# tanishqkumar/ssd

Hardware: NVIDIA H100
Metric: decode tokens/sec (sync speculative decoding, accept-len reported) (higher is better)
Workload: dtype bf16

## Files before the change

### include/ssdk.h

```cpp
#ifndef SSDK_H_
#define SSDK_H_

#include <stdint.h>

#ifdef __cplusplus
extern "C" {
#endif

#define SSDK_ABI_VERSION 1

typedef struct ssdk_engine* ssdk_handle;

enum { SSDK_TARGET = 0, SSDK_DRAFT = 1 };

enum {
  SSDK_W_EMBED      = 0,
  SSDK_W_LM_HEAD    = 1,
  SSDK_W_FINAL_NORM = 2,
  SSDK_W_INPUT_NORM = 3,
  SSDK_W_QKV        = 4,
  SSDK_W_Q_NORM     = 5,
  SSDK_W_K_NORM     = 6,
  SSDK_W_O          = 7,
  SSDK_W_POST_NORM  = 8,
  SSDK_W_GATE_UP    = 9,
  SSDK_W_DOWN       = 10,
  SSDK_W_ROPE_TABLE = 11,
  SSDK_W_KIND_COUNT = 12
};

typedef struct ssdk_model_cfg {
  int32_t hidden;
  int32_t layers;
  int32_t heads;
  int32_t kv_heads;
  int32_t head_dim;
  int32_t ffn;
  int32_t vocab;
  int32_t qk_norm;
  float   rms_eps;
  int32_t max_pos;
  int32_t tp_size;
  int32_t tp_rank;
} ssdk_model_cfg;

typedef struct ssdk_runtime_cfg {
  int32_t spec_k;
  int32_t max_batch;
  int32_t block_size;
  int32_t max_blocks_per_seq;
  int32_t use_graph;
  int32_t use_pdl;
  int32_t jit_speculate;
  int32_t reserved;
} ssdk_runtime_cfg;

int  ssdk_abi_version(void);
const char* ssdk_last_error(void);

int ssdk_create(const ssdk_model_cfg* target, const ssdk_model_cfg* draft,
                const ssdk_runtime_cfg* rt, ssdk_handle* out);
int ssdk_destroy(ssdk_handle h);

int ssdk_bind_weight(ssdk_handle h, int which, int kind, int layer,
                     const void* dev_ptr, int64_t rows, int64_t cols);

int ssdk_bind_kv_cache(ssdk_handle h, int which, void* kv_base, int64_t num_blocks);

int64_t ssdk_workspace_bytes(ssdk_handle h);
int ssdk_bind_workspace(ssdk_handle h, void* dev_ptr, int64_t bytes);

int ssdk_set_nccl_comm(ssdk_handle h, void* nccl_comm);
int64_t ssdk_symm_bytes(ssdk_handle h);
int ssdk_bind_symm(ssdk_handle h, void* const* peer_ptrs, int n_peers);

int ssdk_finalize(ssdk_handle h, void* stream);


int ssdk_spec_step(ssdk_handle h, int batch,
                   const int32_t* ctx_len, const int64_t* recovery,
                   const int32_t* block_tables_target, const int32_t* block_tables_draft,
                   const float* temp_t, const float* temp_q,
                   uint64_t seed, uint64_t step_id,
                   int64_t* out_tokens, int32_t* out_n_accept, int64_t* out_recovery,
                   void* stream);

int ssdk_spec_step_stage(ssdk_handle h, int batch,
                         const int32_t* ctx_len, const int64_t* recovery,
                         const int32_t* block_tables_target, const int32_t* block_tables_draft,
                         const float* temp_t, const float* temp_q,
                         uint64_t seed, uint64_t step_id, void* stream);
int ssdk_spec_step_resident(ssdk_handle h, int batch, void* stream);
int ssdk_spec_step_fetch(ssdk_handle h, int batch, int64_t* out_tokens,
                         int32_t* out_n_accept, int64_t* out_recovery, void* stream);
int ssdk_spec_step_log(ssdk_handle h, int seq, int64_t* out_tokens, int cap, void* stream);

int ssdk_forward_tokens(ssdk_handle h, int which, int batch, int q_len,
                        const int64_t* ids, const int32_t* ctx_len,
                        const int32_t* block_tables, int want_sample,
                        const float* temps, uint64_t seed, uint64_t step_id,
                        int64_t* out_tokens, void* stream);

int ssdk_forward_varlen(ssdk_handle h, int which, int n_seqs, const int32_t* q_lens,
                        const int64_t* ids, const int32_t* ctx_len,
                        const int32_t* block_tables, int want_sample,
                        const float* temps, uint64_t seed, uint64_t step_id,
                        int64_t* out_tokens, void* stream);

const void* ssdk_logits_p(ssdk_handle h);
const void* ssdk_logits_q(ssdk_handle h);
const void* ssdk_logits_last(ssdk_handle h);
int ssdk_debug_trace(void* dev_buf, int cap);
int64_t ssdk_launch_count(ssdk_handle h);


int ssdk_gemm_small_m(const void* x, const void* w, void* y, float* partials,
                      int M, int N, int K, int ldy, int split_k, void* stream);

int ssdk_gemm_gate_up_silu(const void* x, const void* w_gate_up, void* h,
                           int M, int ffn, int K, void* stream);

int ssdk_rmsnorm(const void* x, const void* residual_in, const void* w, float eps,
                 void* y, void* residual_out, int M, int d, void* stream);

int ssdk_rope_store_kv(const void* qkv, const int64_t* positions, const int32_t* slot_mapping,
                       const float* rope_table, const void* q_norm_w, const void* k_norm_w,
                       float norm_eps, void* q_out, void* k_cache, void* v_cache,
                       int M, int heads, int kv_heads, int head_dim, void* stream);

int ssdk_silu_mul(const void* gate_up, void* out, int M, int ffn, void* stream);

int64_t ssdk_paged_attn_scratch_bytes(int batch, int q_len, int heads, int head_dim, int max_ctx);
int ssdk_paged_attn(const void* q, const void* k_cache, const void* v_cache,
                    const int32_t* block_tables, const int32_t* context_lens,
                    void* out, void* scratch,
                    int batch, int q_len, int heads, int kv_heads, int head_dim,
                    int block_size, int max_blocks_per_seq, float scale, void* stream);
int ssdk_paged_attn_plan(int heads, int kv_heads, int batch, int q_len, int max_ctx, int* out4);
int ssdk_paged_attn_varlen(const void* q, const void* k_cache, const void* v_cache,
                           const int32_t* block_tables, const int32_t* context_lens,
                           const int32_t* q_lens, void* out, void* scratch,
                           int batch, int heads, int kv_heads, int head_dim,
                           int block_size, int max_blocks_per_seq, float scale, void* stream);
int ssdk_paged_attn_varlen_plan(int heads, int kv_heads, int batch, const int32_t* q_lens, int max_ctx, int* out5);

int ssdk_sample(const void* logits, int64_t ld, const float* temps, int B, int V,
                uint64_t seed, uint64_t step_id, int64_t* out_tokens, void* stream);

int64_t ssdk_verify_scratch_bytes(int B, int K);
int ssdk_verify(const void* logits_p, const void* logits_q, const int64_t* speculations,
                const float* temps_t, const float* temps_q, const int32_t* cache_hits,
                int jit_speculate, int B, int K, int V, uint64_t seed, uint64_t step_id,
                int32_t* n_accept, int64_t* recovery, void* scratch, void* stream);

#ifdef __cplusplus
}
#endif
#endif
```

### ssd_b200/csrc/draft_stream.cuh

```cuda
#pragma once
#include "common.cuh"
#include "sampling.cuh"

namespace ssdk {

constexpr int kDsConsumers = 256;
constexpr int kDsWarps = kDsConsumers / 32;
constexpr int kDsThreads = kDsConsumers + 32;
constexpr int kDsMaxLayers = 32;
constexpr int kDsSplits = 16;
constexpr int kDsShortSplits = 8;
constexpr int kDsLongCtx = 256;
constexpr int kDsSlotBytes = 32768;
constexpr int kDsMaxSlots = 6;
constexpr int kDsMaxSteps = 8;
constexpr int kDsBtSmem = 32;

struct DsLayer {
  const __nv_bfloat16 *qkv, *o, *gate_up, *down, *in_norm, *post_norm, *q_norm, *k_norm;
};

struct DsParams {
  int d, L, H, KV, ffn, vocab, qk_norm;
  float eps, scale_log2;
  const __nv_bfloat16 *embed, *final_norm, *lm_head;
  const float* rope;
  __nv_bfloat16 *k_cache, *v_cache;
  long long cache_layer_stride;
  int block_size, max_blocks;
  int64_t* tok_buf;
  int n_fwd;
  int skip_last_head;
  const int32_t* ctx0;
  const int32_t* block_table;
  __nv_bfloat16 *vec_qkv, *vec_attn, *vec_o, *vec_act, *vec_down, *resid0, *resid1;
  float* attn_part;
  __nv_bfloat16* logits;
  long long logits_ld;
  const float* temp;
  const uint64_t* dyn;
  uint64_t seed, call_base;
  ArgMax* samp_partial;
  unsigned* bar_state;
  unsigned* attn_ticket;
  int n_slots;
  DsLayer layers[kDsMaxLayers];
};

SSDK_DEVINL void ds_sync() {
#ifdef SSDK_HOST_EMU
  ::emu::named_barrier(1, kDsConsumers);
#else
  asm volatile("bar.sync 1, 256;" ::: "memory");
#endif
}

struct DsGridBar {
  unsigned long long* counter;
  unsigned long long target;
  __device__ void init() {
    if (threadIdx.x == 0) {
      const unsigned long long c = ld_relaxed_gpu_u64(counter);
      target = c - c % (unsigned long long)gridDim.x;
    }
  }
  __device__ void sync() {
    ds_sync();
    if (threadIdx.x == 0) {
      target += (unsigned long long)gridDim.x;
      red_add_release_gpu_u64(counter, 1ull);
      const long long t0 = clock64();
      while (ld_relaxed_gpu_u64(counter) < target) {
        if (clock64() - t0 > 4000000000LL) __trap();
      }
      fence_acq_rel_gpu();
    }
    ds_sync();
  }
};

SSDK_DEVINL uint4 ds_ldcg16(const void* p) { return __ldcg(reinterpret_cast<const uint4*>(p)); }
SSDK_DEVINL float2 ds_bf2(uint32_t w) { return __bfloat1622float2(*reinterpret_cast<const __nv_bfloat162*>(&w)); }

SSDK_DEVINL void ds_mark(int f, int point) {
  if (f == 1 && threadIdx.x == 0) trace_mark(64 + point);
}

enum { DS_QKV = 0, DS_O = 1, DS_GU = 2, DS_DOWN = 3, DS_HEAD = 4 };
enum { DS_PLAIN = 0, DS_PAIR = 1, DS_SPLIT = 2 };
struct DsGeom {
  int K;
  int rows;
  int kind;
  int rpj;
  int segs;
  int nj;
};
__host__ SSDK_DEVINL bool ds_geometry(int K, int rows, bool pair, DsGeom* g) {
  g->K = K; g->rows = rows; g->segs = 1;
  if (K < 256 || K > 8192 || (K % 256) != 0) return false;
  if (pair) {
    if (K > 2048) return false;
    g->kind = DS_PAIR; g->rpj = 8;
  } else if (K <= 2048) {
    g->kind = DS_PLAIN; g->rpj = 8;
  } else {
    g->kind = DS_SPLIT; g->rpj = K <= 4096 ? 4 : 2; g->segs = kDsWarps / g->rpj;
    if ((K % (256 * g->segs)) != 0) return false;
  }
  g->nj = (rows + g->rpj - 1) / g->rpj;
  return true;
}
SSDK_DEVINL bool ds_has_head(const DsParams& p, int f) { return !(p.skip_last_head && f == p.n_fwd - 1); }
SSDK_DEVINL const __nv_bfloat16* ds_weight(const DsParams& p, int l, int m) {
  const DsLayer& lw = p.layers[l < p.L ? l : 0];
  return m == DS_QKV ? lw.qkv : (m == DS_O ? lw.o : (m == DS_GU ? lw.gate_up : (m == DS_DOWN ? lw.down : p.lm_head)));
}

struct DsCursor {
  int f, l, m, s;
  bool valid;
};
SSDK_DEVINL void ds_cursor_settle(const DsParams& p, const DsGeom* geom, DsCursor& c) {
  while (c.valid && c.s >= geom[c.m].nj) {
    c.s = (int)blockIdx.x;
    if (c.m == DS_HEAD) {
      c.f++; c.l = 0; c.m = DS_QKV;
    } else if (c.m == DS_DOWN) {
      c.l++; c.m = DS_QKV;
      if (c.l == p.L) {
        if (ds_has_head(p, c.f)) c.m = DS_HEAD;
        else { c.f++; c.l = 0; }
      }
    } else {
      c.m++;
    }
    if (c.f >= p.n_fwd) c.valid = false;
  }
}

SSDK_DEVINL void ds_cursor_next(const DsParams& p, const DsGeom* geom, DsCursor& c) {
  c.s += (int)gridDim.x;
  if (c.s >= geom[c.m].nj) ds_cursor_settle(p, geom, c);
}
SSDK_DEVINL void ds_producer(const DsParams& p, const DsGeom* geom, uint8_t* ring, uint64_t* full, uint64_t* empty) {
  DsCursor c;
  c.f = 0; c.l = 0; c.m = DS_QKV; c.s = (int)blockIdx.x; c.valid = p.n_fwd > 0;
  ds_cursor_settle(p, geom, c);
  unsigned n = 0;
  const unsigned S = (unsigned)p.n_slots;
  while (c.valid) {
    const DsGeom g = geom[c.m];
    const __nv_bfloat16* w = ds_weight(p, c.l, c.m);
    const int rows = min(g.rpj, g.rows - c.s * g.rpj);
    const unsigned bytes = (unsigned)rows * (unsigned)g.K * 2u;
    const int parts = g.kind == DS_PAIR ? 2 : 1;
    for (int q = 0; q < parts; ++q) {
      const unsigned slot = n % S, round = n / S;
      mbar_wait(&empty[slot], (round & 1u) ^ 1u);
      mbar_arrive_expect_tx(&full[slot], bytes);
      const __nv_bfloat16* src = w + ((size_t)(q ? g.rows : 0) + (size_t)c.s * g.rpj) * g.K;
      bulk_load_g2s(ring + (size_t)slot * kDsSlotBytes, src, bytes, &full[slot]);
      ++n;
    }
    ds_cursor_next(p, geom, c);
  }
}

struct DsRing {
  uint8_t* base;
  uint64_t *full, *empty;
  unsigned n_slots;
  unsigned taken;
};
SSDK_DEVINL const uint8_t* ds_acquire(DsRing& r, unsigned k) {
  const unsigned n = r.taken + k, slot = n % r.n_slots;
  mbar_wait(&r.full[slot], (n / r.n_slots) & 1u);
  return r.base + (size_t)slot * kDsSlotBytes;
}
SSDK_DEVINL void ds_release(DsRing& r, unsigned k, int lane) {
  __syncwarp();
  if (lane == 0) mbar_arrive(&r.empty[(r.taken + k) % r.n_slots]);
}

SSDK_DEVINL void ds_load_x(const float* xseg, int steps, int lane, float (&xr)[kDsMaxSteps][8]) {
#pragma unroll
  for (int j = 0; j < kDsMaxSteps; ++j) {
    if (j < steps) {
      const float4 a = *reinterpret_cast<const float4*>(xseg + j * 256 + lane * 8);
      const float4 b = *reinterpret_cast<const float4*>(xseg + j * 256 + lane * 8 + 4);
      xr[j][0] = a.x; xr[j][1] = a.y; xr[j][2] = a.z; xr[j][3] = a.w;
      xr[j][4] = b.x; xr[j][5] = b.y; xr[j][6] = b.z; xr[j][7] = b.w;
    } else {
#pragma unroll
      for (int e = 0; e < 8; ++e) xr[j][e] = 0.f;
    }
  }
}
SSDK_DEVINL float ds_dot_seg(const uint8_t* wseg, int steps, int lane, const float (&xr)[kDsMaxSteps][8]) {
  const uint4* wp = reinterpret_cast<const uint4*>(wseg) + lane;
  float a0 = 0.f, a1 = 0.f, a2 = 0.f, a3 = 0.f;
#pragma unroll
  for (int j = 0; j < kDsMaxSteps; ++j) {
    if (j < steps) {
      const uint4 w = wp[j * 32];
      float2 f = ds_bf2(w.x);
      a0 = fmaf(f.x, xr[j][0], a0); a1 = fmaf(f.y, xr[j][1], a1);
      f = ds_bf2(w.y);
      a2 = fmaf(f.x, xr[j][2], a2); a3 = fmaf(f.y, xr[j][3], a3);
      f = ds_bf2(w.z);
      a0 = fmaf(f.x, xr[j][4], a0); a1 = fmaf(f.y, xr[j][5], a1);
      f = ds_bf2(w.w);
      a2 = fmaf(f.x, xr[j][6], a2); a3 = fmaf(f.y, xr[j][7], a3);
    }
  }
  return warp_sum((a0 + a1) + (a2 + a3));
}

struct DsSample {
  bool greedy;
  float invT;
  uint64_t seed, call_id;
  ArgMax best;
};
SSDK_DEVINL float ds_score(const DsSample& s, float logit, int idx) {
  if (s.greedy) return logit;
  const uint4 rnd = philox_draw((uint32_t)(idx >> 2), 0u, s.call_id, TAG_SAMPLE, s.seed);
  const float e = u32_to_exp1(u4_word(rnd, idx & 3)) + 1e-10f;
  return logit * s.invT - __logf(e);
}

template <bool HEAD>
SSDK_DEVINL void ds_consume_plain(DsRing& ring, const DsGeom& g, const float* xs, __nv_bfloat16* y, DsSample* smp) {
  if ((int)blockIdx.x >= g.nj) return;
  const int warp = threadIdx.x >> 5, lane = threadIdx.x & 31;
  const int steps = g.K >> 8;
  float xr[kDsMaxSteps][8];
  ds_load_x(xs, steps, lane, xr);
  for (int s = (int)blockIdx.x; s < g.nj; s += (int)gridDim.x) {
    const uint8_t* st = ds_acquire(ring, 0);
    const float acc = ds_dot_seg(st + (size_t)warp * g.K * 2, steps, lane, xr);
    ds_release(ring, 0, lane);
    ring.taken += 1u;
    const int row = s * 8 + warp;
    if (lane == 0 && row < g.rows) {
      const __nv_bfloat16 o = f2bf(acc);
      if (!HEAD) {
        y[row] = o;
      } else {
        if (y) y[row] = o;
        smp->best = argmax_better(smp->best, ArgMax{ds_score(*smp, bf2f(o), row), row});
      }
    }
  }
}
SSDK_DEVINL void ds_consume_pair(DsRing& ring, const DsGeom& g, const float* xs, __nv_bfloat16* act) {
  if ((int)blockIdx.x >= g.nj) return;
  const int warp = threadIdx.x >> 5, lane = threadIdx.x & 31;
  const int steps = g.K >> 8;
  float xr[kDsMaxSteps][8];
  ds_load_x(xs, steps, lane, xr);
  for (int s = (int)blockIdx.x; s < g.nj; s += (int)gridDim.x) {
    const uint8_t* sg = ds_acquire(ring, 0);
    float gate = ds_dot_seg(sg + (size_t)warp * g.K * 2, steps, lane, xr);
    ds_release(ring, 0, lane);
    const uint8_t* su = ds_acquire(ring, 1);
    float up = ds_dot_seg(su + (size_t)warp * g.K * 2, steps, lane, xr);
    ds_release(ring, 1, lane);
    ring.taken += 2u;
    const int i = s * 8 + warp;
    if (lane == 0 && i < g.rows) {
      gate = bf16_round(gate);
      up = bf16_round(up);
      act[i] = f2bf((gate / (1.0f + __expf(-gate))) * up);
    }
  }
}
SSDK_DEVINL void ds_consume_split(DsRing& ring, const DsGeom& g, const float* xs, float* res, __nv_bfloat16* y) {
  if ((int)blockIdx.x >= g.nj) return;
  const int warp = threadIdx.x >> 5, lane = threadIdx.x & 31;
  const int row_in_job = warp / g.segs, seg = warp - row_in_job * g.segs;
  const int seg_len = g.K / g.segs, steps = seg_len >> 8;
  float xr[kDsMaxSteps][8];
  ds_load_x(xs + seg * seg_len, steps, lane, xr);
  const size_t w_off = ((size_t)row_in_job * g.K + (size_t)seg * seg_len) * 2;
  unsigned it = 0;
  for (int s = (int)blockIdx.x; s < g.nj; s += (int)gridDim.x, ++it) {
    const uint8_t* st = ds_acquire(ring, 0);
    const float acc = ds_dot_seg(st + w_off, steps, lane, xr);
    ds_release(ring, 0, lane);
    ring.taken += 1u;
    float* rb = res + (it & 1u) * kDsWarps;
    if (lane == 0) rb[warp] = acc;
    ds_sync();
    if ((int)threadIdx.x < g.rpj) {
      const int row = s * g.rpj + (int)threadIdx.x;
      if (row < g.rows) {
        float v = 0.f;
        for (int q = 0; q < g.segs; ++q) v += rb[(int)threadIdx.x * g.segs + q];
        y[row] = f2bf(v);
      }
    }
  }
}
SSDK_DEVINL void ds_consume(DsRing& ring, const DsGeom& g, const float* xs, float* res, __nv_bfloat16* y) {
  if (g.kind == DS_PLAIN) ds_consume_plain<false>(ring, g, xs, y, nullptr);
  else ds_consume_split(ring, g, xs, res, y);
}

SSDK_DEVINL float ds_block_sum(float v, float* red) {
  const int lane = threadIdx.x & 31, wid = threadIdx.x >> 5;
  v = warp_sum(v);
  ds_sync();
  if (lane == 0) red[wid] = v;
  ds_sync();
  float t = (lane < kDsWarps) ? red[lane] : 0.f;
  return warp_sum(t);
}

struct DsPre {
  uint4 w, b;
};
SSDK_DEVINL DsPre ds_preload(const __nv_bfloat16* b, const __nv_bfloat16* w, int d) {
  DsPre r;
  const int i = threadIdx.x * 8;
  r.w = r.b = make_uint4(0u, 0u, 0u, 0u);
  if (i < d) {
    r.w = *reinterpret_cast<const uint4*>(w + i);
    if (b) r.b = ds_ldcg16(b + i);
  }
  return r;
}
SSDK_DEVINL void ds_norm_prologue(const __nv_bfloat16* a, const __nv_bfloat16* b, __nv_bfloat16* resid_out,
                                  const __nv_bfloat16* w, float eps, int d, float* xs, float* red, const DsPre* pre) {
  float ss = 0.f;
  const int i0 = threadIdx.x * 8;
  for (int i = i0; i < d; i += kDsConsumers * 8) {
    float x[8];
    unpack_bf16x8(ds_ldcg16(a + i), x);
    if (b) {
      float y[8];
      unpack_bf16x8((pre && i == i0) ? pre->b : ds_ldcg16(b + i), y);
#pragma unroll
      for (int j = 0; j < 8; ++j) x[j] += y[j];
    }
    if (resid_out && blockIdx.x == 0) *reinterpret_cast<uint4*>(resid_out + i) = pack_bf16x8(x);
#pragma unroll
    for (int j = 0; j < 8; ++j) {
      xs[i + j] = x[j];
      ss += x[j] * x[j];
    }
  }
  ss = ds_block_sum(ss, red);
  const float rstd = rsqrtf(ss / (float)d + eps);
  for (int i = i0; i < d; i += kDsConsumers * 8) {
    float wv[8];
    unpack_bf16x8((pre && i == i0) ? pre->w : *reinterpret_cast<const uint4*>(w + i), wv);
#pragma unroll
    for (int j = 0; j < 8; ++j) xs[i + j] = bf16_round(xs[i + j] * rstd * wv[j]);
  }
  ds_sync();
}
SSDK_DEVINL void ds_load_vec(const __nv_bfloat16* v, int n, float* xs) {
  for (int i = threadIdx.x * 8; i < n; i += kDsConsumers * 8) {
    float x[8];
    unpack_bf16x8(ds_ldcg16(v + i), x);
#pragma unroll
    for (int j = 0; j < 8; ++j) xs[i + j] = x[j];
  }
  ds_sync();
}

SSDK_DEVINL int ds_num_splits(int ctx) {
  return ctx > kDsLongCtx ? kDsSplits : min(kDsShortSplits, max(1, (ctx + 7) >> 3));
}
SSDK_DEVINL int ds_page_of(const DsParams& p, const int* bt_s, int t) {
  const int i = t / p.block_size;
  return p.max_blocks <= kDsBtSmem ? bt_s[i] : p.block_table[i];
}
template <int HD, int TB>
SSDK_DEVINL void ds_load_kv(const DsParams& p, const int* bt_s, const __nv_bfloat16* kbase, const __nv_bfloat16* vbase, int h,
                            int tb, int t1, int pos, int lane, float (&kv)[TB][HD / 32], float (&vv)[TB][HD / 32]) {
  constexpr int EPL = HD / 32;
  static_assert(EPL == 2 || EPL == 4, "head_dim 64 or 128");
#pragma unroll
  for (int u = 0; u < TB; ++u) {
    const int t = tb + u * kDsWarps;
#pragma unroll
    for (int e = 0; e < EPL; ++e) kv[u][e] = vv[u][e] = 0.f;
    if (t < t1 && t != pos) {
      const int blk = ds_page_of(p, bt_s, t);
      const size_t off = (((size_t)blk * p.block_size + t % p.block_size) * p.KV + h) * HD + lane * EPL;
      if constexpr (EPL == 2) {
        const float2 a = ds_bf2(__ldcg(reinterpret_cast<const uint32_t*>(kbase + off)));
        const float2 b = ds_bf2(__ldcg(reinterpret_cast<const uint32_t*>(vbase + off)));
        kv[u][0] = a.x; kv[u][1] = a.y; vv[u][0] = b.x; vv[u][1] = b.y;
      } else {
        const uint2 a = __ldcg(reinterpret_cast<const uint2*>(kbase + off));
        const uint2 b = __ldcg(reinterpret_cast<const uint2*>(vbase + off));
        float2 f = ds_bf2(a.x); kv[u][0] = f.x; kv[u][1] = f.y;
        f = ds_bf2(a.y); kv[u][EPL - 2] = f.x; kv[u][EPL - 1] = f.y;
        f = ds_bf2(b.x); vv[u][0] = f.x; vv[u][1] = f.y;
        f = ds_bf2(b.y); vv[u][EPL - 2] = f.x; vv[u][EPL - 1] = f.y;
      }
    }
  }
}
template <int HD, int GMAX, int TB>
SSDK_DEVINL void ds_attention_unit(const DsParams& p, int layer, int h, int s, int ns, int ctx, float* sm, int* flag,
                                   const int* bt_s) {
  constexpr int HALF = HD / 2;
  constexpr int EPL = HD / 32;
  const int warp = threadIdx.x >> 5, lane = threadIdx.x & 31;
  const int G = p.H / p.KV;
  const int pos = ctx - 1;
  float* sq = sm;
  float* sk = sq + GMAX * HD;
  float* sv = sk + HD;
  float* sred = sv + HD;

  const int per = (ctx + ns - 1) / ns;
  const int t0 = s * per, t1 = min(ctx, t0 + per);
  const __nv_bfloat16* kbase = p.k_cache + (size_t)layer * p.cache_layer_stride;
  const __nv_bfloat16* vbase = p.v_cache + (size_t)layer * p.cache_layer_stride;
  float kv[TB][EPL], vv[TB][EPL];
  ds_load_kv<HD, TB>(p, bt_s, kbase, vbase, h, t0 + warp, t1, pos, lane, kv, vv);

  const float* cs = p.rope + (size_t)pos * HD;
  for (int row = warp; row < G + 2; row += kDsWarps) {
    const int kind = row < G ? 0 : (row == G ? 1 : 2);
    const int col0 = (kind == 0 ? (h * G + row) : (kind == 1 ? p.H + h : p.H + p.KV + h)) * HD;
    float x1[(HALF + 31) / 32], x2[(HALF + 31) / 32];
    float ss = 0.f;
#pragma unroll
    for (int t = 0; t < (HALF + 31) / 32; ++t) {
      const int i = lane + 32 * t;
      x1[t] = x2[t] = 0.f;
      if (i < HALF) {
        const unsigned short a = __ldcg(reinterpret_cast<const unsigned short*>(p.vec_qkv + col0 + i));
        const unsigned short b = __ldcg(reinterpret_cast<const unsigned short*>(p.vec_qkv + col0 + HALF + i));
        x1[t] = __bfloat162float(__ushort_as_bfloat16(a));
        x2[t] = __bfloat162float(__ushort_as_bfloat16(b));
        ss += x1[t] * x1[t] + x2[t] * x2[t];
      }
    }
    float* dst = kind == 0 ? sq + row * HD : (kind == 1 ? sk : sv);
    if (kind == 2) {
#pragma unroll
      for (int t = 0; t < (HALF + 31) / 32; ++t) {
        const int i = lane + 32 * t;
        if (i < HALF) {
          dst[i] = x1[t];
          dst[HALF + i] = x2[t];
        }
      }
      continue;
    }
    const __nv_bfloat16* nw = p.qk_norm ? (kind == 0 ? p.layers[layer].q_norm : p.layers[layer].k_norm) : nullptr;
    if (nw) {
      ss = warp_sum(ss);
      const float rstd = rsqrtf(ss / (float)HD + p.eps);
#pragma unroll
      for (int t = 0; t < (HALF + 31) / 32; ++t) {
        const int i = lane + 32 * t;
        if (i < HALF) {
          x1[t] = bf16_round(x1[t] * rstd * bf2f(nw[i]));
          x2[t] = bf16_round(x2[t] * rstd * bf2f(nw[HALF + i]));
        }
      }
    }
#pragma unroll
    for (int t = 0; t < (HALF + 31) / 32; ++t) {
      const int i = lane + 32 * t;
      if (i < HALF) {
        const float c = cs[i], sn = cs[HALF + i];
        dst[i] = bf16_round(x1[t] * c - x2[t] * sn);
        dst[HALF + i] = bf16_round(x2[t] * c + x1[t] * sn);
      }
    }
  }
  ds_sync();

  const int blk_new = ds_page_of(p, bt_s, pos);
  if (s == 0 && blk_new >= 0) {
    const size_t slot = (size_t)blk_new * p.block_size + pos % p.block_size;
    __nv_bfloat16* kc = p.k_cache + (size_t)layer * p.cache_layer_stride + (slot * p.KV + h) * HD;
    __nv_bfloat16* vc = p.v_cache + (size_t)layer * p.cache_layer_stride + (slot * p.KV + h) * HD;
    for (int i = threadIdx.x; i < HD; i += kDsConsumers) {
      kc[i] = f2bf(sk[i]);
      vc[i] = f2bf(sv[i]);
    }
  }

  float qreg[GMAX][EPL];
#pragma unroll
  for (int g = 0; g < GMAX; ++g)
#pragma unroll
    for (int e = 0; e < EPL; ++e) qreg[g][e] = (g < G) ? sq[g * HD + lane * EPL + e] : 0.f;
  float m[GMAX], l[GMAX], acc[GMAX][EPL];
#pragma unroll
  for (int g = 0; g < GMAX; ++g) {
    m[g] = -INFINITY;
    l[g] = 0.f;
#pragma unroll
    for (int e = 0; e < EPL; ++e) acc[g][e] = 0.f;
  }
  for (int tb = t0 + warp; tb < t1; tb += TB * kDsWarps) {
    if (tb != t0 + warp) ds_load_kv<HD, TB>(p, bt_s, kbase, vbase, h, tb, t1, pos, lane, kv, vv);
#pragma unroll
    for (int u = 0; u < TB; ++u) {
      const int t = tb + u * kDsWarps;
      if (t < t1) {
        if (t == pos) {
#pragma unroll
          for (int e = 0; e < EPL; ++e) {
            kv[u][e] = sk[lane * EPL + e];
            vv[u][e] = sv[lane * EPL + e];
          }
        }
#pragma unroll
        for (int g = 0; g < GMAX; ++g) {
          if (g < G) {
            float sc = 0.f;
#pragma unroll
            for (int e = 0; e < EPL; ++e) sc = fmaf(qreg[g][e], kv[u][e], sc);
            sc = warp_sum(sc) * p.scale_log2;
            const float mn = fmaxf(m[g], sc);
            const float corr = exp2f(m[g] - mn);
            const float pr = exp2f(sc - mn);
            l[g] = l[g] * corr + pr;
#pragma unroll
            for (int e = 0; e < EPL; ++e) acc[g][e] = acc[g][e] * corr + pr * vv[u][e];
            m[g] = mn;
          }
        }
      }
    }
  }
  constexpr int LDR = HD + 2;
#pragma unroll
  for (int g = 0; g < GMAX; ++g) {
    if (g < G) {
      float* w = sred + ((size_t)warp * G + g) * LDR;
#pragma unroll
      for (int e = 0; e < EPL; ++e) w[lane * EPL + e] = acc[g][e];
      if (lane == 0) {
        w[HD] = m[g];
        w[HD + 1] = l[g];
      }
    }
  }
  ds_sync();
  for (int idx = threadIdx.x; idx < G * HD; idx += kDsConsumers) {
    const int g = idx / HD, dim = idx - g * HD;
    float mx = -INFINITY;
    for (int w = 0; w < kDsWarps; ++w) mx = fmaxf(mx, sred[((size_t)w * G + g) * LDR + HD]);
    float o = 0.f, ll = 0.f;
    if (mx != -INFINITY) {
      for (int w = 0; w < kDsWarps; ++w) {
        const float* r = sred + ((size_t)w * G + g) * LDR;
        const float wt = exp2f(r[HD] - mx);
        o += r[dim] * wt;
        ll += r[HD + 1] * wt;
      }
    }
    if (ns == 1) {
      p.vec_attn[(size_t)(h * G + g) * HD + dim] = f2bf(ll > 0.f ? o / ll : 0.f);
    } else {
      float* out = p.attn_part + ((size_t)(h * G + g) * kDsSplits + s) * LDR;
      out[dim] = o;
      if (dim == 0) {
        out[HD] = mx;
        out[HD + 1] = ll;
      }
    }
  }
  if (ns == 1) {
    ds_sync();
    return;
  }
  ds_sync();
  if (threadIdx.x == 0) *flag = (atom_add_acq_rel_gpu(p.attn_ticket + h, 1u) == (unsigned)ns - 1u) ? 1 : 0;
  ds_sync();
  if (*flag) {
    if (threadIdx.x == 0) st_relaxed_gpu_u32(p.attn_ticket + h, 0u);
    for (int idx = threadIdx.x; idx < G * HD; idx += kDsConsumers) {
      const int g = idx / HD, dim = idx - g * HD;
      const float* base = p.attn_part + (size_t)(h * G + g) * kDsSplits * LDR;
      float ms[kDsSplits], ls[kDsSplits], os[kDsSplits];
      float mx = -INFINITY;
#pragma unroll
      for (int q = 0; q < kDsSplits; ++q) {
        const bool on = q < ns;
        ms[q] = on ? __ldcg(base + q * LDR + HD) : -INFINITY;
        ls[q] = on ? __ldcg(base + q * LDR + HD + 1) : 0.f;
        os[q] = on ? __ldcg(base + q * LDR + dim) : 0.f;
        mx = fmaxf(mx, ms[q]);
      }
      float o = 0.f, l = 0.f;
#pragma unroll
      for (int q = 0; q < kDsSplits; ++q) {
        const float wt = (ms[q] == -INFINITY) ? 0.f : exp2f(ms[q] - mx);
        o += os[q] * wt;
        l += ls[q] * wt;
      }
      p.vec_attn[(size_t)(h * G + g) * HD + dim] = f2bf(l > 0.f ? o / l : 0.f);
    }
  }
  ds_sync();
}


template <int HD, int GMAX>
__global__ void __launch_bounds__(kDsThreads, 1) draft_stream_kernel(const __grid_constant__ DsParams p) {
  SSDK_DYN_SMEM(uint8_t, ds_smem);
  SSDK_STATIC_SMEM(uint64_t, full_bar, kDsMaxSlots);
  SSDK_STATIC_SMEM(uint64_t, empty_bar, kDsMaxSlots);
  SSDK_STATIC_SMEM(DsGeom, geom, 5);
  SSDK_STATIC_SMEM(float, red, 32);
  SSDK_STATIC_SMEM(float, res, 2 * kDsWarps);
  SSDK_STATIC_SMEM(ArgMax, ared, 32);
  SSDK_SHARED_VAR(int, tok_s);
  SSDK_SHARED_VAR(int, flag_s);
  SSDK_STATIC_SMEM(int, bt_s, kDsBtSmem);
  float* xs = reinterpret_cast<float*>(ds_smem + (size_t)p.n_slots * kDsSlotBytes);
  float* scratch = xs + max(max(p.d, p.ffn), p.H * HD);
  if (threadIdx.x < kDsBtSmem && (int)threadIdx.x < p.max_blocks) bt_s[threadIdx.x] = p.block_table[threadIdx.x];
  if (threadIdx.x == 0) {
    trace_mark(TR_MISC);
    ds_geometry(p.d, (p.H + 2 * p.KV) * HD, false, &geom[DS_QKV]);
    ds_geometry(p.H * HD, p.d, false, &geom[DS_O]);
    ds_geometry(p.d, p.ffn, true, &geom[DS_GU]);
    ds_geometry(p.ffn, p.d, false, &geom[DS_DOWN]);
    ds_geometry(p.d, p.vocab, false, &geom[DS_HEAD]);
    for (int s = 0; s < p.n_slots; ++s) {
      mbar_init(&full_bar[s], 1);
      mbar_init(&empty_bar[s], kDsWarps);
    }
    fence_mbar_init();
  }
  __syncthreads();

  if (threadIdx.x >= kDsConsumers) {
    if (threadIdx.x == kDsConsumers) ds_producer(p, geom, ds_smem, full_bar, empty_bar);
    return;
  }

  DsRing ring;
  ring.base = ds_smem;
  ring.full = full_bar;
  ring.empty = empty_bar;
  ring.n_slots = (unsigned)p.n_slots;
  ring.taken = 0u;
  DsGridBar bar;
  bar.counter = reinterpret_cast<unsigned long long*>(p.bar_state);
  bar.target = 0;
  bar.init();

  const int ctx_base = p.ctx0[0];
  const float T = p.temp ? p.temp[0] : 0.f;
  const uint64_t seed = p.dyn ? p.dyn[0] : p.seed;
  const uint64_t call0 = p.dyn ? p.dyn[1] * 16ull : p.call_base;
  __nv_bfloat16* resid[2] = {p.resid0, p.resid1};
  long long tok = p.tok_buf[0];

  for (int f = 0; f < p.n_fwd; ++f) {
    if (threadIdx.x == 0 && f > 0) trace_mark(TR_MISC);
    const int ctx = ctx_base + f + 1;
    const __nv_bfloat16* emb = p.embed + (size_t)tok * p.d;
    int cur = 0;
    DsPre pre;
    for (int l = 0; l < p.L; ++l) {
      const DsLayer& lw = p.layers[l];
      if (l == 0) {
        ds_norm_prologue(emb, nullptr, resid[cur ^ 1], lw.in_norm, p.eps, p.d, xs, red, nullptr);
      } else {
        ds_norm_prologue(p.vec_down, resid[cur], resid[cur ^ 1], lw.in_norm, p.eps, p.d, xs, red, &pre);
      }
      cur ^= 1;
      ds_mark(f, 0);
      ds_consume(ring, geom[DS_QKV], xs, res, p.vec_qkv);
      ds_mark(f, 1);
      bar.sync();
      ds_mark(f, 2);
#ifdef SSDK_TRACE_FINE
      bar.sync();
      ds_mark(f, 12);
#endif
      const int ns = ds_num_splits(ctx);
      for (int u = blockIdx.x; u < p.KV * ns; u += gridDim.x) {
        if (ns == kDsSplits) ds_attention_unit<HD, GMAX, 8>(p, l, u / ns, u % ns, ns, ctx, scratch, &flag_s, bt_s);
        else ds_attention_unit<HD, GMAX, 4>(p, l, u / ns, u % ns, ns, ctx, scratch, &flag_s, bt_s);
      }
      ds_mark(f, 3);
      bar.sync();
      ds_mark(f, 4);
      ds_load_vec(p.vec_attn, p.H * HD, xs);
      ds_consume(ring, geom[DS_O], xs, res, p.vec_o);
      ds_mark(f, 5);
      pre = ds_preload(resid[cur], lw.post_norm, p.d);
      bar.sync();
      ds_mark(f, 6);
      ds_norm_prologue(p.vec_o, resid[cur], resid[cur ^ 1], lw.post_norm, p.eps, p.d, xs, red, &pre);
      cur ^= 1;
      ds_mark(f, 7);
      ds_consume_pair(ring, geom[DS_GU], xs, p.vec_act);
      ds_mark(f, 8);
      bar.sync();
      ds_mark(f, 9);
      ds_load_vec(p.vec_act, p.ffn, xs);
      ds_consume(ring, geom[DS_DOWN], xs, res, p.vec_down);
      ds_mark(f, 10);
      pre = ds_preload(resid[cur], l + 1 < p.L ? p.layers[l + 1].in_norm : p.final_norm, p.d);
      bar.sync();
      ds_mark(f, 11);
    }
    if (!ds_has_head(p, f)) break;
    ds_norm_prologue(p.vec_down, resid[cur], nullptr, p.final_norm, p.eps, p.d, xs, red, &pre);
    DsSample smp;
    smp.greedy = (T == 0.f);
    smp.invT = smp.greedy ? 1.f : 1.f / T;
    smp.seed = seed;
    smp.call_id = call0 + (uint64_t)f;
    smp.best = ArgMax{-INFINITY, 0x7fffffff};
    ds_consume_plain<true>(ring, geom[DS_HEAD], xs, p.logits ? p.logits + (size_t)f * p.logits_ld : nullptr, &smp);
    if ((threadIdx.x & 31) == 0) ared[threadIdx.x >> 5] = smp.best;
    ds_sync();
    if (threadIdx.x == 0) {
      ArgMax b = ared[0];
      for (int w = 1; w < kDsWarps; ++w) b = argmax_better(b, ared[w]);
      p.samp_partial[blockIdx.x] = b;
    }
    bar.sync();
    {
      ArgMax a{-INFINITY, 0x7fffffff};
      for (int i = threadIdx.x; i < (int)gridDim.x; i += kDsConsumers) {
        ArgMax q;
        q.v = __ldcg(&p.samp_partial[i].v);
        q.i = __ldcg(&p.samp_partial[i].i);
        a = argmax_better(a, q);
      }
      a = warp_argmax(a);
      ds_sync();
      if ((threadIdx.x & 31) == 0) ared[threadIdx.x >> 5] = a;
      ds_sync();
      if (threadIdx.x == 0) {
        ArgMax b = ared[0];
        for (int w = 1; w < kDsWarps; ++w) b = argmax_better(b, ared[w]);
        tok_s = b.i;
      }
      ds_sync();
      tok = tok_s;
      if (blockIdx.x == 0 && threadIdx.x == 0) p.tok_buf[f + 1] = tok;
    }
  }
}

}
```

### ssd_b200/csrc/elementwise.cuh

```cuda
#pragma once
#include "common.cuh"

namespace ssdk {

struct GemmOut {
  const __nv_bfloat16* dense;
  const float* partial;
  int S;
  int M;
  int N;
};

SSDK_DEVINL float gemm_out_at(const GemmOut& g, int m, int n) {
  if (g.S == 0) return bf2f(g.dense[(size_t)m * g.N + n]);
  const float* base = g.partial + (size_t)m * g.N + n;
  const size_t stride = (size_t)g.M * g.N;
  float acc = 0.f;
  for (int s0 = 0; s0 < g.S; s0 += 8) {
    float v[8];
#pragma unroll
    for (int u = 0; u < 8; ++u) v[u] = (s0 + u < g.S) ? __ldcg(base + (size_t)(s0 + u) * stride) : 0.f;
#pragma unroll
    for (int u = 0; u < 8; ++u) acc += v[u];
  }
  return bf16_round(acc);
}
template <int NB = 8>
SSDK_DEVINL void gemm_out_at8(const GemmOut& g, int m, int n, float* f) {
  if (g.S == 0) {
    uint4 v = *reinterpret_cast<const uint4*>(g.dense + (size_t)m * g.N + n);
    unpack_bf16x8(v, f);
    return;
  }
#pragma unroll
  for (int i = 0; i < 8; ++i) f[i] = 0.f;
  const float* base = g.partial + (size_t)m * g.N + n;
  const size_t stride = (size_t)g.M * g.N;
  for (int s0 = 0; s0 < g.S; s0 += NB) {
    float4 a[NB], b[NB];
#pragma unroll
    for (int u = 0; u < NB; ++u) {
      if (s0 + u < g.S) {
        const float4* p = reinterpret_cast<const float4*>(base + (size_t)(s0 + u) * stride);
        a[u] = __ldcg(p);
        b[u] = __ldcg(p + 1);
      } else {
        a[u] = make_float4(0.f, 0.f, 0.f, 0.f);
        b[u] = a[u];
      }
    }
#pragma unroll
    for (int u = 0; u < NB; ++u) {
      f[0] += a[u].x; f[1] += a[u].y; f[2] += a[u].z; f[3] += a[u].w;
      f[4] += b[u].x; f[5] += b[u].y; f[6] += b[u].z; f[7] += b[u].w;
    }
  }
#pragma unroll
  for (int i = 0; i < 8; ++i) f[i] = bf16_round(f[i]);
}

SSDK_DEVINL void gemm_out_at2x2(const GemmOut& g, int m, int a, int b, float* fa, float* fb) {
  if (g.S == 0) {
    const float2 va = __bfloat1622float2(*reinterpret_cast<const __nv_bfloat162*>(g.dense + (size_t)m * g.N + a));
    const float2 vb = __bfloat1622float2(*reinterpret_cast<const __nv_bfloat162*>(g.dense + (size_t)m * g.N + b));
    fa[0] = va.x; fa[1] = va.y; fb[0] = vb.x; fb[1] = vb.y;
    return;
  }
  fa[0] = fa[1] = fb[0] = fb[1] = 0.f;
  const float* base = g.partial + (size_t)m * g.N;
  const size_t stride = (size_t)g.M * g.N;
  for (int s0 = 0; s0 < g.S; s0 += 8) {
    float2 va[8], vb[8];
#pragma unroll
    for (int u = 0; u < 8; ++u) {
      const float* row = base + (size_t)min(s0 + u, g.S - 1) * stride;
      va[u] = __ldcg(reinterpret_cast<const float2*>(row + a));
      vb[u] = __ldcg(reinterpret_cast<const float2*>(row + b));
    }
#pragma unroll
    for (int u = 0; u < 8; ++u) {
      const bool in = s0 + u < g.S;
      fa[0] += in ? va[u].x : 0.f; fa[1] += in ? va[u].y : 0.f;
      fb[0] += in ? vb[u].x : 0.f; fb[1] += in ? vb[u].y : 0.f;
    }
  }
  fa[0] = bf16_round(fa[0]); fa[1] = bf16_round(fa[1]); fb[0] = bf16_round(fb[0]); fb[1] = bf16_round(fb[1]);
}

__global__ void prep_kernel(const int32_t* __restrict__ ctx0, const int32_t* __restrict__ block_tables,
                            int max_blocks, int block_size, int batch, int q_len, int pos_offset,
                            int64_t* __restrict__ positions, int32_t* __restrict__ slot_mapping,
                            int32_t* __restrict__ context_lens, unsigned* __restrict__ fwd_seq) {
  pdl_launch_dependents();
  pdl_wait();
  if (threadIdx.x == 0) trace_mark(TR_PREP);
  const int i = blockIdx.x * blockDim.x + threadIdx.x;
  if (i < batch * q_len) {
    const int b = i / q_len, j = i - b * q_len;
    const int pos = ctx0[b] + pos_offset + j;
    positions[i] = pos;
    const int blk = block_tables[(size_t)b * max_blocks + pos / block_size];
    slot_mapping[i] = (blk < 0) ? -1 : blk * block_size + pos % block_size;
  }
  if (i < batch) context_lens[i] = ctx0[i] + pos_offset + q_len;
  if (fwd_seq && i == 0) *fwd_seq += 1u;
}

__global__ void prep_varlen_kernel(const int32_t* __restrict__ ctx0, const int32_t* __restrict__ cu_q,
                                   const int32_t* __restrict__ block_tables, int max_blocks, int block_size, int batch,
                                   int64_t* __restrict__ positions, int32_t* __restrict__ slot_mapping,
                                   int32_t* __restrict__ context_lens, unsigned* __restrict__ fwd_seq) {
  pdl_launch_dependents();
  pdl_wait();
  if (threadIdx.x == 0) trace_mark(TR_PREP);
  const int i = blockIdx.x * blockDim.x + threadIdx.x;
  if (i < cu_q[batch]) {
    int b = 0;
    while (cu_q[b + 1] <= i) ++b;
    const int pos = ctx0[b] + i - cu_q[b];
    positions[i] = pos;
    const int blk = block_tables[(size_t)b * max_blocks + pos / block_size];
    slot_mapping[i] = (blk < 0) ? -1 : blk * block_size + pos % block_size;
  }
  if (i < batch) context_lens[i] = ctx0[i] + cu_q[i + 1] - cu_q[i];
  if (fwd_seq && i == 0) *fwd_seq += 1u;
}

struct SymmIn {
  const uint8_t* base;
  const unsigned* fwd_seq;
  int no_dep_wait;
  int call_idx;
  int n_calls;
  int n_ranks;
  unsigned slot_bytes;
};
constexpr int kSymmMaxRanks = 8;
SSDK_DEVINL size_t symm_slot_off(unsigned parity, int rank, unsigned slot_bytes) {
  return ((size_t)parity * kSymmMaxRanks + rank) * slot_bytes;
}

struct NormParams {
  GemmOut x;
  SymmIn symm;
  const int64_t* ids;
  int ids_stride;
  const __nv_bfloat16* embed;
  int vocab_start, vocab_rows;
  const __nv_bfloat16* residual_in;
  const __nv_bfloat16* w;
  float eps;
  __nv_bfloat16* y;
  __nv_bfloat16* residual_out;
  int d;
};

template <int NB>
SSDK_DEVINL void norm_slice(const NormParams& p, int m, int i, const uint8_t* symm_slots, unsigned symm_e,
                            const __nv_bfloat16* erow, bool zero_row, float* x) {
  const int d = p.d;
  uint4 res = make_uint4(0, 0, 0, 0);
  if (p.residual_in && !symm_slots) res = *reinterpret_cast<const uint4*>(p.residual_in + (size_t)m * d + i);
  if (symm_slots) {
#pragma unroll
    for (int j = 0; j < 8; ++j) x[j] = 0.f;
    const size_t word0 = ((size_t)m * d + i) / 2;
    uint4 lo[kSymmMaxRanks], hi[kSymmMaxRanks];
    const long long t0 = clock64();
    bool ready = false;
    while (!ready) {
#pragma unroll
      for (int r = 0; r < kSymmMaxRanks; ++r) {
        if (r < p.symm.n_ranks) {
          const uint4* src = reinterpret_cast<const uint4*>(symm_slots + (size_t)r * p.symm.slot_bytes) + word0 / 2;
          lo[r] = ld_volatile_v4(src);
          hi[r] = ld_volatile_v4(src + 1);
        }
      }
      ready = true;
#pragma unroll
      for (int r = 0; r < kSymmMaxRanks; ++r)
        if (r < p.symm.n_ranks)
          ready = ready && lo[r].y == symm_e && lo[r].w == symm_e && hi[r].y == symm_e && hi[r].w == symm_e;
      if (!ready && clock64() - t0 > 8000000000LL) __trap();
    }
#pragma unroll
    for (int r = 0; r < kSymmMaxRanks; ++r) {
      if (r < p.symm.n_ranks) {
        const uint32_t w4[4] = {lo[r].x, lo[r].z, hi[r].x, hi[r].z};
#pragma unroll
        for (int q = 0; q < 4; ++q) {
          const float2 c = __bfloat1622float2(*reinterpret_cast<const __nv_bfloat162*>(&w4[q]));
          x[2 * q] += c.x;
          x[2 * q + 1] += c.y;
        }
      }
    }
#pragma unroll
    for (int j = 0; j < 8; ++j) x[j] = bf16_round(x[j]);
    asm volatile("" ::: "memory");
    if (p.residual_in) res = *reinterpret_cast<const uint4*>(p.residual_in + (size_t)m * d + i);
  } else if (p.ids) {
    if (zero_row) {
#pragma unroll
      for (int j = 0; j < 8; ++j) x[j] = 0.f;
    } else {
      unpack_bf16x8(*reinterpret_cast<const uint4*>(erow + i), x);
    }
  } else {
    gemm_out_at8<NB>(p.x, m, i, x);
  }
  if (p.residual_in) {
    float r[8];
    unpack_bf16x8(res, r);
#pragma unroll
    for (int j = 0; j < 8; ++j) x[j] += r[j];
  }
  if (p.residual_out) *reinterpret_cast<uint4*>(p.residual_out + (size_t)m * d + i) = pack_bf16x8(x);
}

template <int SLICES>
__global__ void __launch_bounds__(512) add_rmsnorm_kernel(NormParams p) {
  SSDK_DYN_SMEM(float, rbuf);
  SSDK_STATIC_SMEM(float, red, 32);
  pdl_launch_dependents();
  if (!(p.symm.base && p.symm.no_dep_wait)) pdl_wait();
  if (threadIdx.x == 0) trace_mark(TR_NORM);
  const int m = blockIdx.x;
  const int d = p.d;
  const uint8_t* symm_slots = nullptr;
  unsigned symm_e = 0;
  if (p.symm.base) {
    const unsigned seq = __ldcg(p.symm.fwd_seq);
    symm_e = symm_epoch_of(seq, p.symm.call_idx);
    symm_slots = p.symm.base + symm_slot_off(symm_parity_of(seq, p.symm.call_idx, p.symm.n_calls), 0, p.symm.slot_bytes);
  }
  const __nv_bfloat16* erow = nullptr;
  bool zero_row = false;
  if (p.ids) {
    const long long id = p.ids[(size_t)m * p.ids_stride] - p.vocab_start;
    if (id < 0 || id >= p.vocab_rows) zero_row = true;
    else erow = p.embed + (size_t)id * d;
  }
  float ss = 0.f;
  if constexpr (SLICES > 0) {
    constexpr int NB = (SLICES == 1) ? 8 : 4;
    float xreg[SLICES][8];
    uint4 wpk[SLICES];
#pragma unroll
    for (int c = 0; c < SLICES; ++c) {
      const int i = (c * blockDim.x + threadIdx.x) * 8;
      if (i < d && p.y) wpk[c] = *reinterpret_cast<const uint4*>(p.w + i);
    }
#pragma unroll
    for (int c = 0; c < SLICES; ++c) {
      const int i = (c * blockDim.x + threadIdx.x) * 8;
      if (i < d) {
        norm_slice<NB>(p, m, i, symm_slots, symm_e, erow, zero_row, xreg[c]);
#pragma unroll
        for (int j = 0; j < 8; ++j) ss += xreg[c][j] * xreg[c][j];
      }
    }
    if (threadIdx.x == 0) trace_fine(TRF_NORM + 0);
    ss = block_sum(ss, red);
    if (threadIdx.x == 0) trace_fine(TRF_NORM + 1);
    const float rstd = rsqrtf(ss / (float)d + p.eps);
    if (p.y) {
#pragma unroll
      for (int c = 0; c < SLICES; ++c) {
        const int i = (c * blockDim.x + threadIdx.x) * 8;
        if (i < d) {
          float w[8], o[8];
          unpack_bf16x8(wpk[c], w);
#pragma unroll
          for (int j = 0; j < 8; ++j) o[j] = xreg[c][j] * rstd * w[j];
          *reinterpret_cast<uint4*>(p.y + (size_t)m * d + i) = pack_bf16x8(o);
        }
      }
    }
  } else {
    for (int i = threadIdx.x * 8; i < d; i += blockDim.x * 8) {
      float x[8];
      norm_slice<4>(p, m, i, symm_slots, symm_e, erow, zero_row, x);
#pragma unroll
      for (int j = 0; j < 8; ++j) {
        rbuf[i + j] = x[j];
        ss += x[j] * x[j];
      }
    }
    ss = block_sum(ss, red);
    const float rstd = rsqrtf(ss / (float)d + p.eps);
    if (p.y) {
      for (int i = threadIdx.x * 8; i < d; i += blockDim.x * 8) {
        float w[8], o[8];
        unpack_bf16x8(*reinterpret_cast<const uint4*>(p.w + i), w);
#pragma unroll
        for (int j = 0; j < 8; ++j) o[j] = rbuf[i + j] * rstd * w[j];
        *reinterpret_cast<uint4*>(p.y + (size_t)m * d + i) = pack_bf16x8(o);
      }
    }
  }
  if (threadIdx.x == 0) trace_fine(TRF_NORM + 2);
}

struct ArPublishParams {
  GemmOut x;
  const int64_t* ids;
  int ids_stride;
  const __nv_bfloat16* embed;
  int vocab_start, vocab_rows;
  int M, d, n_ranks, rank;
  uint8_t* peer[kSymmMaxRanks];
  unsigned slot_bytes;
  const unsigned* fwd_seq;
  int call_idx, n_calls;
};

__global__ void __launch_bounds__(256) ar_publish_kernel(ArPublishParams p) {
  pdl_launch_dependents();
  pdl_wait();
  if (threadIdx.x == 0) trace_mark(TR_MISC);
  const unsigned seq = __ldcg(p.fwd_seq);
  const unsigned e = symm_epoch_of(seq, p.call_idx);
  const size_t slot_off = symm_slot_off(symm_parity_of(seq, p.call_idx, p.n_calls), p.rank, p.slot_bytes);
  const int total = p.M * p.d;
  for (int idx = (blockIdx.x * blockDim.x + threadIdx.x) * 8; idx < total; idx += gridDim.x * blockDim.x * 8) {
    const int m = idx / p.d, i = idx - m * p.d;
    float x[8];
    if (p.ids) {
      const long long id = p.ids[(size_t)m * p.ids_stride] - p.vocab_start;
      if (id < 0 || id >= p.vocab_rows) {
#pragma unroll
        for (int j = 0; j < 8; ++j) x[j] = 0.f;
      } else {
        unpack_bf16x8(*reinterpret_cast<const uint4*>(p.embed + (size_t)id * p.d + i), x);
      }
    } else {
      gemm_out_at8(p.x, m, i, x);
    }
    const uint4 v = pack_bf16x8(x);
    const uint4 lo = make_uint4(v.x, e, v.y, e), hi = make_uint4(v.z, e, v.w, e);
    const int r_lo = gridDim.y > 1 ? (int)blockIdx.y : 0, r_hi = gridDim.y > 1 ? (int)blockIdx.y + 1 : p.n_ranks;
#pragma unroll
    for (int r = 0; r < kSymmMaxRanks; ++r) {
      if (r >= r_lo && r < r_hi) {
        uint4* dst = reinterpret_cast<uint4*>(p.peer[r] + slot_off) + idx / 4;
        dst[0] = lo;
        dst[1] = hi;
      }
    }
  }
}

struct RopeParams {
  GemmOut qkv;
  const int64_t* positions;
  const int32_t* slot_mapping;
  const float* rope_table;
  const __nv_bfloat16* q_norm_w;
  const __nv_bfloat16* k_norm_w;
  float norm_eps;
  __nv_bfloat16* q_out;
  __nv_bfloat16* k_cache;
  __nv_bfloat16* v_cache;
  int heads, kv_heads, head_dim;
};

template <int HD>
__global__ void __launch_bounds__(128) rope_store_kernel(RopeParams p) {
  constexpr int HALF = HD / 2;
  constexpr int NP = (HALF + 63) / 64;
  pdl_launch_dependents();
  pdl_wait();
  if (threadIdx.x == 0) trace_mark(TR_ROPE);
  const int m = blockIdx.x;
  const int head = blockIdx.y * 4 + (threadIdx.x >> 5);
  const int lane = threadIdx.x & 31;
  const int H = p.heads, KV = p.kv_heads;
  if (head >= H + 2 * KV) return;
  const int kind = head < H ? 0 : (head < H + KV ? 1 : 2);
  const int col0 = head * HD;
  const int slot = p.slot_mapping[m];
  const long long pos = p.positions[m];

  float x1[NP][2], x2[NP][2];
  float ss = 0.f;
#pragma unroll
  for (int t = 0; t < NP; ++t) {
    const int i = 2 * lane + 64 * t;
    if (i < HALF) {
      gemm_out_at2x2(p.qkv, m, col0 + i, col0 + HALF + i, x1[t], x2[t]);
      ss += x1[t][0] * x1[t][0] + x1[t][1] * x1[t][1] + x2[t][0] * x2[t][0] + x2[t][1] * x2[t][1];
    } else {
      x1[t][0] = x1[t][1] = x2[t][0] = x2[t][1] = 0.f;
    }
  }
  if (kind != 0 && slot < 0) return;
  if (kind == 2) {
    __nv_bfloat16* dst = p.v_cache + ((size_t)slot * KV + (head - H - KV)) * HD;
#pragma unroll
    for (int t = 0; t < NP; ++t) {
      const int i = 2 * lane + 64 * t;
      if (i < HALF) {
        *reinterpret_cast<__nv_bfloat162*>(dst + i) = __floats2bfloat162_rn(x1[t][0], x1[t][1]);
        *reinterpret_cast<__nv_bfloat162*>(dst + HALF + i) = __floats2bfloat162_rn(x2[t][0], x2[t][1]);
// ... 77 lines not shown
```

### ssd_b200/csrc/engine.cu

```cuda
#include <cuda.h>
#include <cuda_runtime.h>
#include <cudaTypedefs.h>
#include <nccl.h>

#include <algorithm>
#include <cstdarg>
#include <cstdio>
#include <cstdlib>
#include <cstring>
#include <map>
#include <string>
#include <tuple>
#include <vector>

#include "../../include/ssdk.h"
#include "attention.cuh"
#include "common.cuh"
#include "elementwise.cuh"
#include "gemm.cuh"
#include "sampling.cuh"
#include "draft_stream.cuh"

using namespace ssdk;
typedef __nv_bfloat16 bf16;

static thread_local std::string g_err;
static int fail(const char* fmt, ...) {
  char buf[1024];
  va_list ap;
  va_start(ap, fmt);
  vsnprintf(buf, sizeof(buf), fmt, ap);
  va_end(ap);
  g_err = buf;
  return -1;
}
#define CK(expr)                                                                              \
  do {                                                                                        \
    cudaError_t _e = (expr);                                                                  \
    if (_e != cudaSuccess) return fail("%s:%d %s -> %s", __FILE__, __LINE__, #expr, cudaGetErrorString(_e)); \
  } while (0)
#define CKN(expr)                                                                             \
  do {                                                                                        \
    ncclResult_t _e = (expr);                                                                 \
    if (_e != ncclSuccess) return fail("%s:%d %s -> nccl error %d", __FILE__, __LINE__, #expr, (int)_e); \
  } while (0)
#define CKI(expr)                 \
  do {                            \
    int _r = (expr);              \
    if (_r != 0) return _r;       \
  } while (0)

static int env_int(const char* name, int dflt) {
  const char* s = getenv(name);
  return (s && *s) ? atoi(s) : dflt;
}

struct Launcher {
  cudaStream_t st = nullptr;
  bool pdl = false;
  bool prev_kernel = false;
  int64_t count = 0;

  template <typename... KArgs, typename... Args>
  int go(void (*kernel)(KArgs...), dim3 grid, dim3 block, size_t smem, Args... args) {
    cudaLaunchConfig_t cfg = {};
    cfg.gridDim = grid;
    cfg.blockDim = block;
    cfg.dynamicSmemBytes = smem;
    cfg.stream = st;
    cudaLaunchAttribute attr[1];
    attr[0].id = cudaLaunchAttributeProgrammaticStreamSerialization;
    attr[0].val.programmaticStreamSerializationAllowed = 1;
    cfg.attrs = attr;
    cfg.numAttrs = (pdl && prev_kernel) ? 1 : 0;
    cudaError_t e = cudaLaunchKernelEx(&cfg, kernel, KArgs(args)...);
    if (e != cudaSuccess) return fail("kernel launch failed: %s", cudaGetErrorString(e));
    prev_kernel = true;
    ++count;
    return 0;
  }
  void barrier_op() { prev_kernel = false; }
};

static PFN_cuTensorMapEncodeTiled_v12000 g_encode = nullptr;
static int get_encode() {
  if (g_encode) return 0;
  void* fn = nullptr;
  cudaDriverEntryPointQueryResult qres;
  cudaError_t e = cudaGetDriverEntryPoint("cuTensorMapEncodeTiled", &fn, cudaEnableDefault, &qres);
  if (e != cudaSuccess || qres != cudaDriverEntryPointSuccess || !fn)
    return fail("cuTensorMapEncodeTiled unavailable (%s)", cudaGetErrorString(e));
  g_encode = reinterpret_cast<PFN_cuTensorMapEncodeTiled_v12000>(fn);
  return 0;
}
static int make_tmap(CUtensorMap* tm, const void* ptr, int64_t rows, int64_t cols, int box_rows) {
  CKI(get_encode());
  if (cols % 8 != 0) return fail("TMA: row length %lld not a multiple of 8 elements", (long long)cols);
  if (((uintptr_t)ptr & 15) != 0) return fail("TMA: base pointer not 16-byte aligned");
  cuuint64_t gdim[2] = {(cuuint64_t)cols, (cuuint64_t)rows};
  cuuint64_t gstride[1] = {(cuuint64_t)cols * 2};
  cuuint32_t box[2] = {(cuuint32_t)kBlockK, (cuuint32_t)box_rows};
  cuuint32_t estr[2] = {1, 1};
  CUresult r = g_encode(tm, CU_TENSOR_MAP_DATA_TYPE_BFLOAT16, 2, const_cast<void*>(ptr), gdim, gstride, box, estr,
                        CU_TENSOR_MAP_INTERLEAVE_NONE, CU_TENSOR_MAP_SWIZZLE_128B, CU_TENSOR_MAP_L2_PROMOTION_L2_256B,
                        CU_TENSOR_MAP_FLOAT_OOB_FILL_NONE);
  if (r != CUDA_SUCCESS) return fail("cuTensorMapEncodeTiled failed (%d) rows=%lld cols=%lld box_rows=%d", (int)r,
                                     (long long)rows, (long long)cols, box_rows);
  return 0;
}

static int g_num_sms = 0;
static int num_sms() {
  if (!g_num_sms) {
    int dev = 0;
    cudaGetDevice(&dev);
    cudaDeviceGetAttribute(&g_num_sms, cudaDevAttrMultiProcessorCount, dev);
    if (g_num_sms <= 0) g_num_sms = 132;
  }
  return g_num_sms;
}
static int norm_threads(int d) { return std::max(32, std::min(512, ((d / 8 + 31) / 32) * 32)); }
static int launch_norm(Launcher& L, int M, int d, const NormParams& np) {
  const int threads = norm_threads(d);
  const int slices = (d + 8 * threads - 1) / (8 * threads);
  if (slices == 1) return L.go(add_rmsnorm_kernel<1>, dim3(M), dim3(threads), 0, np);
  if (slices == 2) return L.go(add_rmsnorm_kernel<2>, dim3(M), dim3(threads), 0, np);
  return L.go(add_rmsnorm_kernel<0>, dim3(M), dim3(threads), (size_t)d * 4, np);
}
static int launch_rope(Launcher& L, int M, const RopeParams& rp) {
  const dim3 grid(M, (rp.heads + 2 * rp.kv_heads + 3) / 4), block(128);
  switch (rp.head_dim) {
    case 64: return L.go(rope_store_kernel<64>, grid, block, 0, rp);
    case 128: return L.go(rope_store_kernel<128>, grid, block, 0, rp);
    case 256: return L.go(rope_store_kernel<256>, grid, block, 0, rp);
    default: return fail("unsupported head_dim %d for RoPE (64, 128 and 256 are built)", rp.head_dim);
  }
}
static int umma_n_for(int M) { return M <= 16 ? 16 : (M <= 32 ? 32 : (M <= 64 ? 64 : (M <= 128 ? 128 : 256))); }

static int auto_splits(int tiles, int num_kb, int ctas_per_sm = 2) {
  const int slots = ctas_per_sm * num_sms();
  int S = std::max(1, slots / tiles);
  S = std::min(S, std::max(1, num_kb / 4));
  S = std::min(S, 8);
  const int per = (num_kb + S - 1) / S;
  return (num_kb + per - 1) / per;
}

template <int UN, int EPI>
static int launch_gemm_inst(Launcher& L, const CUtensorMap& tmW, const CUtensorMap& tmX, const GemmParams& p, int tiles,
                            int splits) {
  using Cfg = GemmCfg<UN>;
  static bool attr_set = false;
  if (!attr_set) {
    CK(cudaFuncSetAttribute(gemm_ws_kernel<UN, EPI>, cudaFuncAttributeMaxDynamicSharedMemorySize, Cfg::kSmemBytes));
    attr_set = true;
  }
  return L.go(gemm_ws_kernel<UN, EPI>, dim3(tiles, splits), dim3(kGemmThreads), (size_t)Cfg::kSmemBytes, tmW, tmX, p);
}
static int launch_gemm(Launcher& L, int umma_n, int epi, const CUtensorMap& tmW, const CUtensorMap& tmX,
                       const GemmParams& p, int tiles, int splits) {
#define SSDK_GEMM_CASE(UN, EP) \
  if (umma_n == UN && epi == EP) return launch_gemm_inst<UN, EP>(L, tmW, tmX, p, tiles, splits);
  SSDK_GEMM_CASE(16, EPI_BF16) SSDK_GEMM_CASE(16, EPI_PARTIAL) SSDK_GEMM_CASE(16, EPI_SILU) SSDK_GEMM_CASE(16, EPI_PUBLISH)
  SSDK_GEMM_CASE(32, EPI_BF16) SSDK_GEMM_CASE(32, EPI_PARTIAL) SSDK_GEMM_CASE(32, EPI_SILU) SSDK_GEMM_CASE(32, EPI_PUBLISH)
  SSDK_GEMM_CASE(64, EPI_BF16) SSDK_GEMM_CASE(64, EPI_PARTIAL) SSDK_GEMM_CASE(64, EPI_SILU) SSDK_GEMM_CASE(64, EPI_PUBLISH)
  SSDK_GEMM_CASE(128, EPI_BF16) SSDK_GEMM_CASE(128, EPI_PARTIAL) SSDK_GEMM_CASE(128, EPI_SILU)
  SSDK_GEMM_CASE(256, EPI_BF16) SSDK_GEMM_CASE(256, EPI_PARTIAL) SSDK_GEMM_CASE(256, EPI_SILU)
#undef SSDK_GEMM_CASE
  return fail("no GEMM instance for umma_n=%d epi=%d", umma_n, epi);
}

struct WeightMat {
  const bf16* ptr = nullptr;
  int64_t rows = 0, cols = 0;
  CUtensorMap tm;
  bool has_tm = false;
};
static int weight_tmap(WeightMat& w) {
  if (w.has_tm) return 0;
  if (!w.ptr) return fail("weight not bound");
  CKI(make_tmap(&w.tm, w.ptr, w.rows, w.cols, 64));
  w.has_tm = true;
  return 0;
}

constexpr int kMaxTokens = 256;
struct XMapCache {
  std::map<std::tuple<const void*, int, int>, CUtensorMap> maps;
  int get(const void* ptr, int K, int umma_n, const CUtensorMap** out) {
    auto key = std::make_tuple(ptr, K, umma_n);
    auto it = maps.find(key);
    if (it == maps.end()) {
      CUtensorMap tm;
      CKI(make_tmap(&tm, ptr, kMaxTokens, K, umma_n));
      it = maps.emplace(key, tm).first;
    }
    *out = &it->second;
    return 0;
  }
};

struct LayerW {
  const bf16* input_norm = nullptr;
  const bf16* post_norm = nullptr;
  const bf16* q_norm = nullptr;
  const bf16* k_norm = nullptr;
  WeightMat qkv, o, gate_up, down;
};
struct Model {
  ssdk_model_cfg cfg;
  bool present = false;
  WeightMat embed, lm_head;
  const bf16* final_norm = nullptr;
  const float* rope = nullptr;
  int64_t rope_rows = 0;
  std::vector<LayerW> layers;
  bf16* k_cache = nullptr;
  bf16* v_cache = nullptr;
  int64_t num_blocks = 0;
  int H, KV, hd, d, ffn, qkv_dim, vocab_local;
};

struct Workspace {
  bf16 *hidden, *residual, *q, *attn_out, *act, *last_hidden, *dense_tmp;
  float* partials;
  float *att_o, *att_lse;
  unsigned* att_counters;
  unsigned* ar_state;
  unsigned* pub_counters;
  int64_t* positions;
  int32_t *slot_mapping, *context_lens;
  uint8_t* out_dev;
  int64_t* tok_buf;
  int64_t* ids_in;
  int32_t* var_cu_q;
  AttnTile* var_tiles;
  int64_t* out_tok;
  bf16 *logits_q, *logits_p, *logits_last;
  bf16 *logits_shard, *logits_gather;
  uint8_t* step_dev;
  int32_t* n_accept;
  int64_t* recovery;
  int64_t* log_tokens;
  int32_t* log_len;
  ArgMax* samp_partial;
  unsigned* samp_counters;
  RowPart* ver_rows;
  RecPart* ver_rec;
  unsigned* ver_counters;
  size_t partial_floats = 0;
  bf16* ds_vec;
  float* ds_attn;
  unsigned* ds_sync;
};

constexpr int kSampleChunks = 64;
constexpr size_t kFwInCuOff = (size_t)kMaxTokens * 8;
constexpr size_t kFwInTileOff = kFwInCuOff + ((size_t)(kMaxTokens + 1) * 4 + 15) / 16 * 16;
constexpr size_t kFwInBytes = kFwInTileOff + (size_t)kMaxTokens * sizeof(AttnTile);
constexpr int kLogCap = 16384;
constexpr int kVerifyCtas = 128;

struct ssdk_engine {
  ssdk_runtime_cfg rt;
  Model model[2];
  Workspace ws;
  void* ws_base = nullptr;
  int64_t ws_bytes = 0;
  XMapCache xmaps;
  ncclComm_t comm = nullptr;
  bool finalized = false;
  int64_t launches = 0;
  uint8_t* pin_in = nullptr;
  uint8_t* pin_out = nullptr;
  static constexpr int kFwSlots = 4;
  uint8_t* pin_fw = nullptr;
  size_t fw_slot_bytes = 0;
  cudaEvent_t fw_ev[kFwSlots] = {nullptr};
  bool fw_ev_pending[kFwSlots] = {false};
  unsigned fw_next = 0;
  size_t step_bytes = 0;
  size_t out_bytes = 0;
  size_t off_ctx, off_rec, off_tt, off_tq, off_seed, off_btt, off_btd;
  size_t off_out_nacc, off_out_rec;
  std::map<int, cudaGraphExec_t> spec_graphs;
  std::map<int, int64_t> spec_graph_launches;
  std::map<int, cudaGraphExec_t> spec_graphs_resident;
  int resident_ctx_bound = 0;
  int max_ctx_hint = 0;
  cudaStream_t cap_stream = nullptr;
  int symm_n = 0;
  uint8_t* symm_peer[kSymmMaxRanks] = {nullptr};
  unsigned symm_slot_bytes = 0;
};

static size_t align_up(size_t x, size_t a) { return (x + a - 1) / a * a; }

static void derive(Model& m) {
  const auto& c = m.cfg;
  m.H = c.heads / c.tp_size;
  m.KV = c.kv_heads / c.tp_size;
  m.hd = c.head_dim;
  m.d = c.hidden;
  m.ffn = c.ffn / c.tp_size;
  m.qkv_dim = (m.H + 2 * m.KV) * m.hd;
  m.vocab_local = c.vocab / c.tp_size;
}

static int64_t carve(ssdk_engine* e, uint8_t* base) {
  size_t off = 0;
  auto take = [&](size_t bytes) -> uint8_t* {
    off = align_up(off, 1024);
    uint8_t* p = base ? base + off : nullptr;
    off += bytes;
    return p;
  };
  int dmax = 0, qmax = 0, fmax = 0, vmax = 0, Hmax = 0, hdmax = 0;
  size_t part = 0;
  for (int w = 0; w < 2; ++w) {
    Model& m = e->model[w];
    if (!m.present) continue;
    dmax = std::max(dmax, m.d);
    qmax = std::max(qmax, m.qkv_dim);
    fmax = std::max(fmax, m.ffn);
    vmax = std::max(vmax, m.cfg.vocab);
    Hmax = std::max(Hmax, m.H);
    hdmax = std::max(hdmax, m.hd);
    auto need = [&](int N, int K) {
      const int tiles = (N + kTileRows - 1) / kTileRows;
      const int S = auto_splits(tiles, K / kBlockK);
      return (size_t)S * kMaxTokens * N;
    };
    part = std::max(part, need(m.qkv_dim, m.d));
    part = std::max(part, need(m.d, m.H * m.hd));
    part = std::max(part, need(2 * m.ffn, m.d));
    part = std::max(part, need(m.d, m.ffn));
  }
  Workspace scratch_ws;
  Workspace& w = base ? e->ws : scratch_ws;
  const int K = e->rt.spec_k, MB = e->rt.max_batch;
  w.hidden = (bf16*)take((size_t)kMaxTokens * dmax * 2);
  w.residual = (bf16*)take((size_t)kMaxTokens * dmax * 2);
  w.q = (bf16*)take((size_t)kMaxTokens * Hmax * hdmax * 2);
  w.attn_out = (bf16*)take((size_t)kMaxTokens * Hmax * hdmax * 2);
  w.act = (bf16*)take((size_t)kMaxTokens * fmax * 2);
  w.last_hidden = (bf16*)take((size_t)kMaxTokens * dmax * 2);
  w.dense_tmp = (bf16*)take((size_t)kMaxTokens * std::max(dmax, qmax) * 2);
  w.partials = (float*)take(part * 4);
  w.partial_floats = part;
  w.att_o = (float*)take((size_t)kMaxTokens * Hmax * kAttnMaxSplit * hdmax * 4);
  w.att_lse = (float*)take((size_t)kMaxTokens * Hmax * kAttnMaxSplit * 4);
  w.att_counters = (unsigned*)take((size_t)kMaxTokens * 64 * 4);
  w.ar_state = (unsigned*)take(64);
  w.pub_counters = (unsigned*)take(512 * 4);
  w.positions = (int64_t*)take(kMaxTokens * 8);
  w.slot_mapping = (int32_t*)take(kMaxTokens * 4);
  w.context_lens = (int32_t*)take(kMaxTokens * 4);
  w.out_dev = take(e->out_bytes);
  w.tok_buf = (int64_t*)w.out_dev;
  w.n_accept = (int32_t*)(w.out_dev ? w.out_dev + e->off_out_nacc : nullptr);
  w.recovery = (int64_t*)(w.out_dev ? w.out_dev + e->off_out_rec : nullptr);
  w.log_tokens = (int64_t*)take((size_t)MB * kLogCap * 8);
  w.log_len = (int32_t*)take((size_t)MB * 4);
  w.ids_in = (int64_t*)take(kFwInBytes);
  w.var_cu_q = (int32_t*)(w.ids_in ? (uint8_t*)w.ids_in + kFwInCuOff : nullptr);
  w.var_tiles = (AttnTile*)(w.ids_in ? (uint8_t*)w.ids_in + kFwInTileOff : nullptr);
  w.out_tok = (int64_t*)take(kMaxTokens * 8);
  w.logits_q = (bf16*)take((size_t)MB * std::max(K, 1) * vmax * 2);
  w.logits_p = (bf16*)take((size_t)MB * (K + 1) * vmax * 2);
  w.logits_last = (bf16*)take((size_t)kMaxTokens * vmax * 2);
  w.logits_shard = (bf16*)take((size_t)kMaxTokens * vmax * 2);
  w.logits_gather = (bf16*)take((size_t)kMaxTokens * vmax * 2);
  w.step_dev = take(e->step_bytes);
  w.samp_partial = (ArgMax*)take((size_t)kMaxTokens * kSampleChunks * sizeof(ArgMax));
  w.samp_counters = (unsigned*)take(kMaxTokens * 4);
  w.ver_rows = (RowPart*)take((size_t)kVerifyMaxRows * kVerifyCtas * sizeof(RowPart));
  w.ver_rec = (RecPart*)take((size_t)kVerifyMaxBatch * kVerifyCtas * sizeof(RecPart));
  w.ver_counters = (unsigned*)take(64);
  w.ds_vec = (bf16*)take((size_t)(qmax + 4 * dmax + fmax + Hmax * hdmax + 64) * 2);
  w.ds_attn = (float*)take((size_t)Hmax * kDsSplits * (hdmax + 2) * 4);
  w.ds_sync = (unsigned*)take(256);
  return (int64_t)align_up(off, 1024);
}

struct VarlenFwd {
  AttnVarlen attn;
  AttnPlan plan;
  int n_tiles;
  int M;
};
struct Fwd {
  int which;
  int B, Q;
  const int64_t* ids;
  int ids_stride;
  const int32_t* ctx0;
  const int32_t* block_tables;
  int pos_offset;
  int logits_mode;
  bf16* logits_out;
  int64_t logits_ld;
  const VarlenFwd* var = nullptr;
};

static int attn_plan_raw(int H, int KV, int B, int Q, int max_ctx, int* TQ, int* MT, int* nqt, int* nsplit) {
  AttnPlan pl;
  const int rc = attn_make_plan(H, KV, B, Q, max_ctx, num_sms(), &pl);
  if (rc == 1) return fail("unsupported GQA ratio %d/%d", H, KV);
  if (rc != 0) return fail("attention tile too large");
  *TQ = pl.TQ;
  *MT = pl.MT;
  *nqt = pl.n_qtiles;
  *nsplit = pl.n_split;
  return 0;
}
static int attn_plan(const Model& m, int B, int Q, int* TQ, int* MT, int* nqt, int* nsplit, int max_ctx) {
  return attn_plan_raw(m.H, m.KV, B, Q, max_ctx, TQ, MT, nqt, nsplit);
}

template <int HD, int MT>
static int launch_attn_inst(Launcher& L, const AttnParams& p, const AttnVarlen* var, dim3 grid) {
  const size_t smem = (size_t)2 * 2 * kAttChunk * (HD + 8) * 2;
  static bool attr_set = false;
  if (!attr_set) {
    CK(cudaFuncSetAttribute(paged_attn_kernel<HD, MT>, cudaFuncAttributeMaxDynamicSharedMemorySize, (int)smem));
    CK(cudaFuncSetAttribute(paged_attn_varlen_kernel<HD, MT>, cudaFuncAttributeMaxDynamicSharedMemorySize, (int)smem));
    attr_set = true;
  }
  if (var) return L.go(paged_attn_varlen_kernel<HD, MT>, grid, dim3(attn_warps(MT) * 32), smem, p, *var);
  return L.go(paged_attn_kernel<HD, MT>, grid, dim3(attn_warps(MT) * 32), smem, p);
}
static int launch_attn(Launcher& L, const AttnParams& p, const AttnVarlen* var, int hd, int MT, dim3 grid) {
  if (hd == 128 && MT == 1) return launch_attn_inst<128, 1>(L, p, var, grid);
  if (hd == 128 && MT == 2) return launch_attn_inst<128, 2>(L, p, var, grid);
  if (hd == 128 && MT == 4) return launch_attn_inst<128, 4>(L, p, var, grid);
  if (hd == 64 && MT == 1) return launch_attn_inst<64, 1>(L, p, var, grid);
  if (hd == 64 && MT == 2) return launch_attn_inst<64, 2>(L, p, var, grid);
  if (hd == 64 && MT == 4) return launch_attn_inst<64, 4>(L, p, var, grid);
  return fail("unsupported head_dim %d (64 and 128 are built)", hd);
}

static int enqueue_attention(Launcher& L, const bf16* q, const bf16* kc, const bf16* vc, const int32_t* bt,
                             const int32_t* ctx_lens, bf16* out, float* part_o, float* part_lse, unsigned* counters,
                             int B, int Q, int H,
                             int KV, int hd, int block_size, int max_blocks, float scale, int TQ, int MT, int nqt,
                             int nsplit, const VarlenFwd* var = nullptr) {
  AttnParams a;
  a.q = q; a.k_cache = kc; a.v_cache = vc; a.block_tables = bt; a.context_lens = ctx_lens; a.out = out;
  a.part_o = part_o; a.part_lse = part_lse;
  (void)counters;
  a.B = B; a.Q = Q; a.H = H; a.KV = KV; a.block_size = block_size; a.max_blocks = max_blocks;
  a.n_split = nsplit; a.TQ = TQ; a.n_qtiles = nqt;
  a.g_shift = attn_g_shift(H, KV);
  a.scale_log2 = scale * 1.4426950408889634f;
  if (var) {
    CKI(launch_attn(L, a, &var->attn, hd, MT, dim3(KV, nsplit, var->n_tiles)));
    if (nsplit > 1) CKI(L.go(attn_combine_kernel<true>, dim3(var->M * H), dim3(32), 0, a, hd, var->attn));
    return 0;
  }
  CKI(launch_attn(L, a, nullptr, hd, MT, dim3(KV, nsplit, B * nqt)));
  if (nsplit > 1) CKI(L.go(attn_combine_kernel<false>, dim3(B * Q * H), dim3(32), 0, a, hd, AttnVarlen{}));
  return 0;
}

static int enqueue_gemm(ssdk_engine* e, Launcher& L, const bf16* x, WeightMat& w, int M, int epi, void* out, int ldo,
                        int N_out, int* splits_out, const PublishParams* pub = nullptr) {
  CKI(weight_tmap(w));
  const int K = (int)w.cols;
  if (K % kBlockK) return fail("GEMM K=%d not a multiple of 64", K);
  const int un = umma_n_for(M);
  const CUtensorMap* tmX;
  CKI(e->xmaps.get(x, K, un, &tmX));
  GemmParams p;
  p.out = out; p.M = M; p.N = N_out; p.ldo = ldo; p.num_kb = K / kBlockK;
  int tiles, splits;
  p.sk_partials = nullptr; p.sk_counters = nullptr; p.sk_width = 0;
  if (epi == EPI_SILU) {
    tiles = (N_out + 63) / 64;
    splits = (un <= 64 && tiles < num_sms() && out != nullptr && e->ws.partials) ? auto_splits(tiles, p.num_kb) : 1;
    if (splits > 1 && (tiles > 512 || (size_t)splits * M * 2 * N_out > e->ws.partial_floats)) splits = 1;
    p.tile_rows = 64;
    p.hi_row_offset = N_out;
    if (splits > 1) {
      p.sk_partials = e->ws.partials; p.sk_counters = e->ws.pub_counters; p.sk_width = 2 * N_out;
    }
  } else {
    tiles = (N_out + kTileRows - 1) / kTileRows;
    splits = (epi == EPI_PARTIAL || epi == EPI_PUBLISH) ? auto_splits(tiles, p.num_kb, un <= 64 ? 2 : 1) : 1;
    p.tile_rows = kTileRows;
    p.hi_row_offset = 64;
  }
  if (epi == EPI_PUBLISH) {
    if (!pub) return fail("EPI_PUBLISH without publish parameters");
    if (un > 64) return fail("EPI_PUBLISH is planned for <= 64 tokens");
    if (tiles > 512) return fail("EPI_PUBLISH: %d tiles > 512 ticket counters", tiles);
    if ((size_t)splits * M * N_out > e->ws.partial_floats) return fail("split-K partial buffer too small");
    p.pub = *pub;
    p.sk_partials = e->ws.partials; p.sk_counters = e->ws.pub_counters; p.sk_width = N_out;
  }
  p.kb_per_split = (p.num_kb + splits - 1) / splits;
  if (epi == EPI_PARTIAL && (size_t)splits * M * N_out > e->ws.partial_floats && out == e->ws.partials)
    return fail("split-K partial buffer too small");
  if (splits_out) *splits_out = splits;
  return launch_gemm(L, un, epi, w.tm, *tmX, p, tiles, splits);
}

static SymmIn symm_in(ssdk_engine* e, int call_idx, bool no_dep_wait = false) {
  SymmIn s;
  s.no_dep_wait = no_dep_wait ? 1 : 0;
  s.base = e->symm_peer[e->model[SSDK_TARGET].cfg.tp_rank];
  s.fwd_seq = e->ws.ar_state;
  s.call_idx = call_idx;
  s.n_calls = 2 * e->model[SSDK_TARGET].cfg.layers + 1;
  s.n_ranks = e->symm_n;
  s.slot_bytes = e->symm_slot_bytes;
  return s;
}
static int enqueue_ar_publish(ssdk_engine* e, Launcher& L, const GemmOut* x, const NormParams* embed_src, int M, int d,
                              int call_idx) {
  Model& m = e->model[SSDK_TARGET];
  ArPublishParams ap;
  memset(&ap, 0, sizeof(ap));
  if (x) ap.x = *x;
  if (embed_src) {
    ap.ids = embed_src->ids; ap.ids_stride = embed_src->ids_stride; ap.embed = embed_src->embed;
    ap.vocab_start = embed_src->vocab_start; ap.vocab_rows = embed_src->vocab_rows;
  }
  ap.M = M; ap.d = d; ap.n_ranks = e->symm_n; ap.rank = m.cfg.tp_rank;
  for (int r = 0; r < e->symm_n; ++r) ap.peer[r] = e->symm_peer[r];
  ap.slot_bytes = e->symm_slot_bytes;
  ap.fwd_seq = e->ws.ar_state; ap.call_idx = call_idx; ap.n_calls = 2 * m.cfg.layers + 1;
  const int n8 = M * d / 8;
  static int per_peer = -1;
  if (per_peer < 0) per_peer = env_int("SSDK_PUBLISH_PER_PEER", e->symm_n >= 8 ? 1 : 0) != 0 ? 1 : 0;
  const int gx = std::max(1, std::min((n8 + 255) / 256, num_sms()));
  return L.go(ar_publish_kernel, dim3(gx, per_peer ? e->symm_n : 1), dim3(256), 0, ap);
}

static PublishParams publish_params(ssdk_engine* e, int call_idx) {
  Model& m = e->model[SSDK_TARGET];
  PublishParams pb;
  memset(&pb, 0, sizeof(pb));
  for (int r = 0; r < e->symm_n; ++r) pb.peer[r] = e->symm_peer[r];
  pb.fwd_seq = e->ws.ar_state;
  pb.slot_bytes = e->symm_slot_bytes;
  pb.call_idx = call_idx;
  pb.n_calls = 2 * m.cfg.layers + 1;
  pb.n_ranks = e->symm_n;
  pb.rank = m.cfg.tp_rank;
  return pb;
}
static bool fused_publish_enabled() {
  static int v = -1;
  if (v < 0) {
    const char* s = getenv("SSDK_FUSED_PUBLISH");
    v = (s && *s) ? (atoi(s) != 0 ? 1 : 0) : 0;
  }
  return v == 1;
}

static int enqueue_tp_allreduce(ssdk_engine* e, Launcher& L, int S, int M, int N, GemmOut* out) {
  Workspace& w = e->ws;
  const int n = M * N;
  CKI(L.go(splitk_reduce_kernel, dim3((n + 255) / 256), dim3(256), 0, (const float*)w.partials, w.dense_tmp, S, M, N, N));
  CKN(ncclAllReduce(w.dense_tmp, w.dense_tmp, (size_t)n, ncclBfloat16, ncclSum, e->comm, L.st));
  L.barrier_op();
  out->dense = w.dense_tmp; out->partial = nullptr; out->S = 0; out->M = M; out->N = N;
  return 0;
}

__global__ void unshard_logits_kernel(const bf16* __restrict__ gathered, bf16* __restrict__ out, int tp, int rows, int Vs,
                                      int64_t ld) {
  pdl_launch_dependents();
  pdl_wait();
  const int64_t n8 = (int64_t)tp * rows * (Vs / 8);
  for (int64_t i = (int64_t)blockIdx.x * blockDim.x + threadIdx.x; i < n8; i += (int64_t)gridDim.x * blockDim.x) {
    const int v8 = (int)(i % (Vs / 8));
    const int64_t t = i / (Vs / 8);
    const int m = (int)(t % rows), r = (int)(t / rows);
    const uint4 val = *reinterpret_cast<const uint4*>(gathered + ((size_t)r * rows + m) * Vs + (size_t)v8 * 8);
    *reinterpret_cast<uint4*>(out + (size_t)m * ld + (size_t)r * Vs + (size_t)v8 * 8) = val;
  }
}

static int enqueue_forward(ssdk_engine* e, Launcher& L, const Fwd& f) {
  Model& m = e->model[f.which];
  Workspace& w = e->ws;
  const int M = f.var ? f.var->M : f.B * f.Q;
  if (M < 1 || M > kMaxTokens) return fail("forward: %d tokens (max %d)", M, kMaxTokens);
  const int tp = m.cfg.tp_size;
  if (tp > 1 && !e->comm) return fail("tensor parallel forward without a NCCL communicator");
  const int bs = e->rt.block_size, mb = e->rt.max_blocks_per_seq;
  const int64_t cache_layer_stride = m.num_blocks * bs * m.KV * m.hd;

  unsigned* fwd_seq = (f.which == SSDK_TARGET && tp > 1 && e->symm_n == tp) ? w.ar_state : (unsigned*)nullptr;
  int TQ = 1, MT = 1, nqt = 1, nsplit = 1;
  if (f.var) {
    CKI(L.go(prep_varlen_kernel, dim3(1), dim3(kMaxTokens), 0, f.ctx0, f.var->attn.cu_q, f.block_tables, mb, bs, f.B,
             w.positions, w.slot_mapping, w.context_lens, fwd_seq));
    TQ = f.var->plan.TQ; MT = f.var->plan.MT; nqt = f.var->plan.n_qtiles; nsplit = f.var->plan.n_split;
  } else {
    CKI(L.go(prep_kernel, dim3(1), dim3(kMaxTokens), 0, f.ctx0, f.block_tables, mb, bs, f.B, f.Q, f.pos_offset,
             w.positions, w.slot_mapping, w.context_lens, fwd_seq));
    CKI(attn_plan(m, f.B, f.Q, &TQ, &MT, &nqt, &nsplit, e->max_ctx_hint));
  }
  const float scale = 1.0f / sqrtf((float)m.hd);

  const bool use_symm = tp > 1 && e->symm_n == tp;
  bool prev_symm = false;
  int ar_idx = 0, prev_idx = 0;
  GemmOut prev;
  prev.dense = nullptr; prev.partial = nullptr; prev.S = 0; prev.M = M; prev.N = m.d;

  for (int l = 0; l < m.cfg.layers; ++l) {
    LayerW& lw = m.layers[l];
    NormParams np;
    memset(&np, 0, sizeof(np));
    np.eps = m.cfg.rms_eps; np.d = m.d; np.w = lw.input_norm; np.y = w.hidden; np.residual_out = w.residual;
    if (l == 0) {
      if (tp == 1) {
        np.ids = f.ids; np.ids_stride = f.ids_stride; np.embed = m.embed.ptr;
        np.vocab_start = 0; np.vocab_rows = m.vocab_local;
      } else {
        NormParams ep;
        memset(&ep, 0, sizeof(ep));
        ep.ids = f.ids; ep.ids_stride = f.ids_stride; ep.embed = m.embed.ptr;
        ep.vocab_start = m.cfg.tp_rank * m.vocab_local; ep.vocab_rows = m.vocab_local;
        if (use_symm) {
          CKI(enqueue_ar_publish(e, L, nullptr, &ep, M, m.d, ar_idx));
          np.symm = symm_in(e, ar_idx++);
        } else {
          ep.eps = m.cfg.rms_eps; ep.d = m.d; ep.residual_out = w.dense_tmp;
          CKI(launch_norm(L, M, m.d, ep));
          CKN(ncclAllReduce(w.dense_tmp, w.dense_tmp, (size_t)M * m.d, ncclBfloat16, ncclSum, e->comm, L.st));
          L.barrier_op();
          np.x.dense = w.dense_tmp; np.x.S = 0; np.x.M = M; np.x.N = m.d;
        }
      }
    } else {
      np.x = prev;
      if (prev_symm) np.symm = symm_in(e, prev_idx, true);
      np.residual_in = w.residual;
    }
    CKI(launch_norm(L, M, m.d, np));

    int S = 1;
    CKI(enqueue_gemm(e, L, w.hidden, lw.qkv, M, EPI_PARTIAL, w.partials, 0, m.qkv_dim, &S));
    RopeParams rp;
    rp.qkv.dense = nullptr; rp.qkv.partial = w.partials; rp.qkv.S = S; rp.qkv.M = M; rp.qkv.N = m.qkv_dim;
    rp.positions = w.positions; rp.slot_mapping = w.slot_mapping; rp.rope_table = m.rope;
    rp.q_norm_w = m.cfg.qk_norm ? lw.q_norm : nullptr;
    rp.k_norm_w = m.cfg.qk_norm ? lw.k_norm : nullptr;
    rp.norm_eps = m.cfg.rms_eps;
    rp.q_out = w.q;
    rp.k_cache = m.k_cache + (size_t)l * cache_layer_stride;
    rp.v_cache = m.v_cache + (size_t)l * cache_layer_stride;
    rp.heads = m.H; rp.kv_heads = m.KV; rp.head_dim = m.hd;
    CKI(launch_rope(L, M, rp));

    CKI(enqueue_attention(L, w.q, rp.k_cache, rp.v_cache, f.block_tables, w.context_lens, w.attn_out, w.att_o,
                          w.att_lse, w.att_counters, f.B, f.Q, m.H, m.KV, m.hd, bs, mb, scale, TQ, MT, nqt, nsplit,
                          f.var));

    const bool fuse_pub = use_symm && fused_publish_enabled() && M <= 64;
    GemmOut oproj;
    bool oproj_symm = false;
    int oproj_idx = 0;
    if (fuse_pub) {
      const PublishParams pb = publish_params(e, ar_idx);
      CKI(enqueue_gemm(e, L, w.attn_out, lw.o, M, EPI_PUBLISH, w.partials, 0, m.d, &S, &pb));
      oproj_idx = ar_idx++;
      oproj_symm = true;
    } else {
      CKI(enqueue_gemm(e, L, w.attn_out, lw.o, M, EPI_PARTIAL, w.partials, 0, m.d, &S));
    }
    oproj.dense = nullptr; oproj.partial = w.partials; oproj.S = S; oproj.M = M; oproj.N = m.d;
    if (tp > 1 && !fuse_pub) {
      if (use_symm) {
        CKI(enqueue_ar_publish(e, L, &oproj, nullptr, M, m.d, ar_idx));
        oproj_idx = ar_idx++;
        oproj_symm = true;
      } else {
        CKI(enqueue_tp_allreduce(e, L, S, M, m.d, &oproj));
      }
    }

    NormParams pn;
    memset(&pn, 0, sizeof(pn));
    pn.x = oproj; pn.residual_in = w.residual; pn.w = lw.post_norm; pn.eps = m.cfg.rms_eps;
    if (oproj_symm) pn.symm = symm_in(e, oproj_idx, true);
    pn.y = w.hidden; pn.residual_out = w.residual; pn.d = m.d;
    CKI(launch_norm(L, M, m.d, pn));

    CKI(enqueue_gemm(e, L, w.hidden, lw.gate_up, M, EPI_SILU, w.act, m.ffn, m.ffn, nullptr));
    if (fuse_pub) {
      const PublishParams pb = publish_params(e, ar_idx);
      CKI(enqueue_gemm(e, L, w.act, lw.down, M, EPI_PUBLISH, w.partials, 0, m.d, &S, &pb));
      prev_idx = ar_idx++;
      prev_symm = true;
    } else {
      CKI(enqueue_gemm(e, L, w.act, lw.down, M, EPI_PARTIAL, w.partials, 0, m.d, &S));
    }
    prev.dense = nullptr; prev.partial = w.partials; prev.S = S; prev.M = M; prev.N = m.d;
    if (tp > 1 && !fuse_pub) {
      if (use_symm) {
        CKI(enqueue_ar_publish(e, L, &prev, nullptr, M, m.d, ar_idx));
        prev_idx = ar_idx++;
        prev_symm = true;
      } else {
        CKI(enqueue_tp_allreduce(e, L, S, M, m.d, &prev));
      }
    }
  }
  NormParams fn;
  memset(&fn, 0, sizeof(fn));
  fn.x = prev; fn.residual_in = w.residual; fn.w = m.final_norm; fn.eps = m.cfg.rms_eps; fn.y = w.hidden;
  if (prev_symm) fn.symm = symm_in(e, prev_idx, true);
  fn.residual_out = nullptr; fn.d = m.d;
  CKI(launch_norm(L, M, m.d, fn));

  if (f.logits_mode != 0) {
    const bf16* x = w.hidden;
    int rows = M;
    if (f.logits_mode == 2 && f.var) {
      if (M > f.B) {
        CKI(L.go(gather_last_rows_varlen_kernel, dim3(f.B), dim3(256), 0, (const bf16*)w.hidden, w.last_hidden,
                 f.var->attn.cu_q, m.d));
        x = w.last_hidden;
      }
      rows = f.B;
    } else if (f.logits_mode == 2 && f.Q > 1) {
      CKI(L.go(gather_last_rows_kernel, dim3(f.B), dim3(256), 0, (const bf16*)w.hidden, w.last_hidden, f.B, f.Q, m.d));
      x = w.last_hidden;
      rows = f.B;
    } else if (f.logits_mode == 2) {
      rows = f.B;
    }
    if (tp == 1) {
      CKI(enqueue_gemm(e, L, x, m.lm_head, rows, EPI_BF16, f.logits_out, (int)f.logits_ld, m.vocab_local, nullptr));
    } else {
      const int Vs = m.vocab_local;
      if (Vs % 8) return fail("tensor-parallel lm_head: vocab shard %d not a multiple of 8", Vs);
      CKI(enqueue_gemm(e, L, x, m.lm_head, rows, EPI_BF16, w.logits_shard, Vs, Vs, nullptr));
      CKN(ncclAllGather(w.logits_shard, w.logits_gather, (size_t)rows * Vs, ncclBfloat16, e->comm, L.st));
      L.barrier_op();
      if (m.cfg.tp_rank == 0 && f.logits_out)
        CKI(L.go(unshard_logits_kernel, dim3(num_sms()), dim3(256), 0, (const bf16*)w.logits_gather, f.logits_out, tp, rows,
                 Vs, f.logits_ld));
    }
  }
  return 0;
}

static void layout_step(ssdk_engine* e) {
  const int MB = e->rt.max_batch, mbk = e->rt.max_blocks_per_seq;
  size_t off = 0;
  auto take = [&](size_t n) { size_t o = off; off = align_up(off + n, 16); return o; };
  e->off_ctx = take((size_t)MB * 4);
  e->off_rec = take((size_t)MB * 8);
  e->off_tt = take((size_t)MB * 4);
  e->off_tq = take((size_t)MB * 4);
  e->off_seed = take(16);
  e->off_btt = take((size_t)MB * mbk * 4);
  e->off_btd = take((size_t)MB * mbk * 4);
  e->step_bytes = off;
  e->off_out_nacc = align_up((size_t)MB * (e->rt.spec_k + 1) * 8, 16);
  e->off_out_rec = e->off_out_nacc + align_up((size_t)MB * 4, 16);
  e->out_bytes = align_up(e->off_out_rec + (size_t)MB * 8, 16);
}



__global__ void init_tokens_kernel(const int64_t* __restrict__ recovery, int64_t* __restrict__ tok_buf, int B, int Kp1) {
  pdl_launch_dependents();
  pdl_wait();
  const int b = threadIdx.x;
  if (b < B) tok_buf[(size_t)b * Kp1] = recovery[b];
}

__global__ void advance_kernel(int32_t* __restrict__ ctx, int64_t* __restrict__ recovery_in, uint64_t* __restrict__ seed_step,
                               const int64_t* __restrict__ tok_buf, const int32_t* __restrict__ n_accept,
                               const int64_t* __restrict__ recovery_out, int64_t* __restrict__ log_tokens,
                               int32_t* __restrict__ log_len, int B, int Kp1, int log_cap) {
  pdl_launch_dependents();
  pdl_wait();
  const int b = threadIdx.x;
  if (b < B) {
    const int n = n_accept[b] + 1;
    int len = log_len[b];
    for (int j = 0; j < n && len < log_cap; ++j) log_tokens[(size_t)b * log_cap + len++] = tok_buf[(size_t)b * Kp1 + j];
    log_len[b] = len;
    ctx[b] += n;
    recovery_in[b] = recovery_out[b];
  }
  if (threadIdx.x == 0) seed_step[1] += 1;
}

static bool draft_stream_enabled() {
  static int v = -1;
  if (v < 0) v = env_int("SSDK_DRAFT_STREAM", 1) != 0 ? 1 : 0;
  return v == 1;
}
constexpr int kMaxDynSmem = 227 * 1024 - 2048;
static size_t ds_fixed_smem(const Model& m) {
  const int G = m.H / m.KV, gmax = G <= 4 ? 4 : 8;
  const size_t xs = (size_t)std::max(std::max(m.d, m.ffn), m.H * m.hd);
  const size_t scratch = (size_t)gmax * m.hd + 2 * m.hd + (size_t)kDsWarps * gmax * (m.hd + 2);
  return (xs + scratch) * 4 + 256;
}
static int ds_ring_slots(const Model& m) {
  const size_t fixed = ds_fixed_smem(m);
  if (fixed + 3 * (size_t)kDsSlotBytes > (size_t)kMaxDynSmem) return 0;
  return (int)std::min<size_t>(kDsMaxSlots, ((size_t)kMaxDynSmem - fixed) / kDsSlotBytes);
}
static bool draft_stream_supported(const Model& m, int B) {
  const int G = m.KV ? m.H / m.KV : 0;
  DsGeom g;
  return B == 1 && m.cfg.tp_size == 1 && m.cfg.layers <= kDsMaxLayers && (m.hd == 64 || m.hd == 128) && G >= 1 && G <= 8 &&
         m.H % m.KV == 0 && m.KV <= 32 && m.d % 8 == 0 && (m.H * m.hd) % 8 == 0 && m.ffn % 8 == 0 &&
         ds_geometry(m.d, m.qkv_dim, false, &g) && ds_geometry(m.H * m.hd, m.d, false, &g) &&
         ds_geometry(m.d, m.ffn, true, &g) && ds_geometry(m.ffn, m.d, false, &g) && ds_geometry(m.d, m.cfg.vocab, false, &g) &&
         ds_ring_slots(m) >= 3;
}
static int draft_stream_max_ctx() {
  static int v = -1;
  if (v < 0) v = std::max(0, env_int("SSDK_DRAFT_STREAM_MAX_CTX", 1024));
  return v;
}
static bool use_draft_stream(ssdk_engine* e, int B, int ctx_bound) {
  const Model& drf = e->model[SSDK_DRAFT];
  return drf.present && draft_stream_enabled() && draft_stream_supported(drf, B) &&
         ctx_bound + e->rt.spec_k + 1 <= draft_stream_max_ctx();
}
template <int HD, int GMAX>
static int launch_draft_stream(Launcher& L, const DsParams& p, size_t smem) {
  static bool attr_set = false;
  if (!attr_set) {
    CK(cudaFuncSetAttribute(draft_stream_kernel<HD, GMAX>, cudaFuncAttributeMaxDynamicSharedMemorySize, (int)smem));
    attr_set = true;
  }
  cudaLaunchConfig_t cfg = {};
  cfg.gridDim = dim3(num_sms());
  cfg.blockDim = dim3(kDsThreads);
  cfg.dynamicSmemBytes = smem;
  cfg.stream = L.st;
  cudaLaunchAttribute attr[1];
  attr[0].id = cudaLaunchAttributeCooperative;
  attr[0].val.cooperative = 1;
  cfg.attrs = attr;
  cfg.numAttrs = 1;
  cudaError_t err = cudaLaunchKernelEx(&cfg, draft_stream_kernel<HD, GMAX>, p);
  if (err != cudaSuccess) return fail("draft stream launch failed: %s", cudaGetErrorString(err));
  L.barrier_op();
  ++L.count;
  return 0;
}
static int enqueue_draft_stream(ssdk_engine* e, Launcher& L, int64_t* tok_buf, int n_fwd, bool skip_last_head,
                                const int32_t* ctx0, const int32_t* block_table, const float* temp, const uint64_t* dyn,
                                bf16* logits, int64_t logits_ld) {
  Model& m = e->model[SSDK_DRAFT];
  Workspace& w = e->ws;
  DsParams p;
  memset(&p, 0, sizeof(p));
  p.d = m.d; p.L = m.cfg.layers; p.H = m.H; p.KV = m.KV; p.ffn = m.ffn; p.vocab = m.cfg.vocab; p.qk_norm = m.cfg.qk_norm;
  p.eps = m.cfg.rms_eps;
  p.scale_log2 = (1.0f / sqrtf((float)m.hd)) * 1.4426950408889634f;
  p.embed = m.embed.ptr; p.final_norm = m.final_norm; p.lm_head = m.lm_head.ptr; p.rope = m.rope;
  p.k_cache = m.k_cache; p.v_cache = m.v_cache;
  p.cache_layer_stride = (long long)m.num_blocks * e->rt.block_size * m.KV * m.hd;
  p.block_size = e->rt.block_size; p.max_blocks = e->rt.max_blocks_per_seq;
  p.tok_buf = tok_buf; p.n_fwd = n_fwd; p.skip_last_head = skip_last_head ? 1 : 0;
  p.ctx0 = ctx0; p.block_table = block_table;
  bf16* v = w.ds_vec;
  p.vec_qkv = v; v += align_up((size_t)m.qkv_dim, 8);
  p.vec_attn = v; v += (size_t)m.H * m.hd;
  p.vec_o = v; v += m.d;
  p.vec_down = v; v += m.d;
  p.resid0 = v; v += m.d;
  p.resid1 = v; v += m.d;
  p.vec_act = v;
  p.attn_part = w.ds_attn;
  p.logits = logits; p.logits_ld = logits_ld;
  p.temp = temp; p.dyn = dyn;
  p.samp_partial = w.samp_partial;
  p.bar_state = w.ds_sync;
  p.attn_ticket = w.ds_sync + 8;
  p.n_slots = ds_ring_slots(m);
  for (int l = 0; l < p.L; ++l) {
    const LayerW& lw = m.layers[l];
    p.layers[l] = DsLayer{lw.qkv.ptr, lw.o.ptr, lw.gate_up.ptr, lw.down.ptr, lw.input_norm, lw.post_norm, lw.q_norm, lw.k_norm};
  }
  const int G = m.H / m.KV, gmax = G <= 4 ? 4 : 8;
  const size_t smem = ds_fixed_smem(m) + (size_t)p.n_slots * kDsSlotBytes;
  if (m.hd == 64 && gmax == 4) return launch_draft_stream<64, 4>(L, p, smem);
  if (m.hd == 64 && gmax == 8) return launch_draft_stream<64, 8>(L, p, smem);
  if (m.hd == 128 && gmax == 4) return launch_draft_stream<128, 4>(L, p, smem);
  return launch_draft_stream<128, 8>(L, p, smem);
}

static int enqueue_spec_step(ssdk_engine* e, Launcher& L, int B, bool host_io, bool advance, bool stream_draft) {
  Workspace& w = e->ws;
  const int K = e->rt.spec_k;
  Model& tgt = e->model[SSDK_TARGET];
  Model& drf = e->model[SSDK_DRAFT];
  const int V = tgt.cfg.vocab;
  if (host_io) {
    CK(cudaMemcpyAsync(w.step_dev, e->pin_in, e->step_bytes, cudaMemcpyHostToDevice, L.st));
    L.barrier_op();
  }
  int32_t* ctx = (int32_t*)(w.step_dev + e->off_ctx);
  int64_t* rec_in = (int64_t*)(w.step_dev + e->off_rec);
  const float* tt = (const float*)(w.step_dev + e->off_tt);
  const float* tq = (const float*)(w.step_dev + e->off_tq);
  uint64_t* seed_step = (uint64_t*)(w.step_dev + e->off_seed);
  const int32_t* btt = (const int32_t*)(w.step_dev + e->off_btt);
  const int32_t* btd = (const int32_t*)(w.step_dev + e->off_btd);

  const int tp = tgt.cfg.tp_size, tp_rank = tgt.cfg.tp_rank;
  if (tp > 1 && !e->comm) return fail("tensor parallel spec step without a NCCL communicator");
  if (tp_rank == 0 && !drf.present) return fail("rank 0 needs the draft model");
  if (drf.present) CKI(L.go(init_tokens_kernel, dim3(1), dim3(64), 0, (const int64_t*)rec_in, w.tok_buf, B, K + 1));
  if (stream_draft)
    CKI(enqueue_draft_stream(e, L, w.tok_buf, K + 1, true, ctx, btd, tq, seed_step, w.logits_q, (int64_t)V));
  for (int k = 0; k <= K && drf.present && !stream_draft; ++k) {
    Fwd f;
    f.which = SSDK_DRAFT; f.B = B; f.Q = 1; f.ids = w.tok_buf + k; f.ids_stride = K + 1;
    f.ctx0 = ctx; f.block_tables = btd; f.pos_offset = k;
    f.logits_mode = (k < K) ? 1 : 0;
    f.logits_out = w.logits_q + (size_t)k * V;
    f.logits_ld = (int64_t)K * V;
    CKI(enqueue_forward(e, L, f));
    if (k < K) {
      SampleParams sp;
      sp.logits = w.logits_q + (size_t)k * V; sp.ld = (int64_t)K * V; sp.temps = tq; sp.V = drf.cfg.vocab;
      sp.seed = 0; sp.call_id = 0; sp.out = w.tok_buf + k + 1; sp.out_stride = K + 1;
      sp.partial = w.samp_partial; sp.counters = w.samp_counters; sp.dyn = seed_step; sp.sub = k;
      CKI(L.go(sample_kernel, dim3(kSampleChunks, B), dim3(256), 0, sp));
    }
  }
  if (tp > 1) {
    CKN(ncclBroadcast(w.tok_buf, w.tok_buf, (size_t)B * (K + 1), ncclInt64, 0, e->comm, L.st));
    L.barrier_op();
  }
  {
    Fwd f;
    f.which = SSDK_TARGET; f.B = B; f.Q = K + 1; f.ids = w.tok_buf; f.ids_stride = 1;
    f.ctx0 = ctx; f.block_tables = btt; f.pos_offset = 0; f.logits_mode = 1;
    f.logits_out = w.logits_p; f.logits_ld = V;
    CKI(enqueue_forward(e, L, f));
  }
  if (tp_rank == 0) {
    VerifyParams vp;
    vp.lp = w.logits_p; vp.lq = w.logits_q; vp.spec = w.tok_buf; vp.temps_t = tt; vp.temps_q = tq;
    vp.cache_hits = nullptr; vp.jit = e->rt.jit_speculate; vp.B = B; vp.K = K; vp.V = V;
    vp.seed = 0; vp.call_id = 0; vp.n_accept = w.n_accept; vp.recovery = w.recovery;
    vp.row_part = w.ver_rows; vp.rec_part = w.ver_rec; vp.counters = w.ver_counters;
    vp.dyn = seed_step; vp.sub = 15;
    CKI(L.go(verify_kernel, dim3(kVerifyCtas), dim3(kVerifyThreads), 0, vp));
  }
  if (tp > 1) {
    CKN(ncclBroadcast(w.out_dev, w.out_dev, e->out_bytes, ncclChar, 0, e->comm, L.st));
    L.barrier_op();
  }
  if (advance) {
    CKI(L.go(advance_kernel, dim3(1), dim3(64), 0, ctx, rec_in, seed_step, (const int64_t*)w.tok_buf,
             (const int32_t*)w.n_accept, (const int64_t*)w.recovery, w.log_tokens, w.log_len, B, K + 1, kLogCap));
  }
  if (host_io) {
    CK(cudaMemcpyAsync(e->pin_out, w.out_dev, e->out_bytes, cudaMemcpyDeviceToHost, L.st));
    L.barrier_op();
  }
  return 0;
}

static int get_spec_graph(ssdk_engine* e, int B, bool host_io, bool stream_draft, cudaStream_t st, cudaGraphExec_t* out,
                          int64_t* nlaunch) {
  auto& cache = host_io ? e->spec_graphs : e->spec_graphs_resident;
  const int key = B * 2 + (stream_draft ? 1 : 0);
  auto it = cache.find(key);
  if (it != cache.end()) {
    *out = it->second;
    *nlaunch = e->spec_graph_launches[key];
    return 0;
  }
  (void)st;
  if (!e->cap_stream) CK(cudaStreamCreateWithFlags(&e->cap_stream, cudaStreamNonBlocking));
  Launcher L;
  L.st = e->cap_stream;
  L.pdl = e->rt.use_pdl != 0;
  cudaGraph_t graph = nullptr;
  CK(cudaStreamBeginCapture(e->cap_stream, cudaStreamCaptureModeThreadLocal));
  const int rc = enqueue_spec_step(e, L, B, host_io, !host_io, stream_draft);
  cudaError_t ce = cudaStreamEndCapture(e->cap_stream, &graph);
  if (rc != 0) {
    if (graph) cudaGraphDestroy(graph);
    return rc;
  }
  if (ce != cudaSuccess) return fail("graph capture failed: %s", cudaGetErrorString(ce));
  cudaGraphExec_t exec = nullptr;
  ce = cudaGraphInstantiate(&exec, graph, 0);
  cudaGraphDestroy(graph);
  if (ce != cudaSuccess) return fail("graph instantiate failed: %s", cudaGetErrorString(ce));
  cache[key] = exec;
  e->spec_graph_launches[key] = L.count;
  *out = exec;
  *nlaunch = L.count;
  return 0;
}

static int init_kernel_attrs() {
#define SSDK_ATTR_G(UN, EP) \
  CK(cudaFuncSetAttribute(gemm_ws_kernel<UN, EP>, cudaFuncAttributeMaxDynamicSharedMemorySize, GemmCfg<UN>::kSmemBytes));
  SSDK_ATTR_G(16, EPI_BF16) SSDK_ATTR_G(16, EPI_PARTIAL) SSDK_ATTR_G(16, EPI_SILU) SSDK_ATTR_G(16, EPI_PUBLISH)
  SSDK_ATTR_G(32, EPI_BF16) SSDK_ATTR_G(32, EPI_PARTIAL) SSDK_ATTR_G(32, EPI_SILU) SSDK_ATTR_G(32, EPI_PUBLISH)
  SSDK_ATTR_G(64, EPI_BF16) SSDK_ATTR_G(64, EPI_PARTIAL) SSDK_ATTR_G(64, EPI_SILU) SSDK_ATTR_G(64, EPI_PUBLISH)
  SSDK_ATTR_G(128, EPI_BF16) SSDK_ATTR_G(128, EPI_PARTIAL) SSDK_ATTR_G(128, EPI_SILU)
  SSDK_ATTR_G(256, EPI_BF16) SSDK_ATTR_G(256, EPI_PARTIAL) SSDK_ATTR_G(256, EPI_SILU)
#undef SSDK_ATTR_G
#define SSDK_ATTR_A(HD, MT) \
  CK(cudaFuncSetAttribute(paged_attn_kernel<HD, MT>, cudaFuncAttributeMaxDynamicSharedMemorySize, 2 * 2 * kAttChunk * (HD + 8) * 2));
  SSDK_ATTR_A(128, 1) SSDK_ATTR_A(128, 2) SSDK_ATTR_A(128, 4) SSDK_ATTR_A(64, 1) SSDK_ATTR_A(64, 2) SSDK_ATTR_A(64, 4)
#undef SSDK_ATTR_A
#define SSDK_ATTR_AV(HD, MT) \
  CK(cudaFuncSetAttribute(paged_attn_varlen_kernel<HD, MT>, cudaFuncAttributeMaxDynamicSharedMemorySize, 2 * 2 * kAttChunk * (HD + 8) * 2));
  SSDK_ATTR_AV(128, 1) SSDK_ATTR_AV(128, 2) SSDK_ATTR_AV(128, 4) SSDK_ATTR_AV(64, 1) SSDK_ATTR_AV(64, 2) SSDK_ATTR_AV(64, 4)
#undef SSDK_ATTR_AV
  CK(cudaFuncSetAttribute(add_rmsnorm_kernel<0>, cudaFuncAttributeMaxDynamicSharedMemorySize, 64 * 1024));
  return 0;
}

static void* g_op_scratch = nullptr;
static int op_scratch(void** out, cudaStream_t st) {
  if (!g_op_scratch) {
    CK(cudaMalloc(&g_op_scratch, 1 << 20));
    CK(cudaMemsetAsync(g_op_scratch, 0, 1 << 20, st));
  }
  *out = g_op_scratch;
  return 0;
}

extern "C" {

int ssdk_abi_version(void) { return SSDK_ABI_VERSION; }
const char* ssdk_last_error(void) { return g_err.c_str(); }

int ssdk_create(const ssdk_model_cfg* target, const ssdk_model_cfg* draft, const ssdk_runtime_cfg* rt, ssdk_handle* out) {
  if (!target || !rt || !out) return fail("ssdk_create: null argument");
  int ndev = 0;
  if (cudaGetDeviceCount(&ndev) != cudaSuccess || ndev == 0) return fail("ssdk_create: no CUDA device");
  if (rt->spec_k < 0 || rt->spec_k > 7) return fail("spec_k=%d out of range [0,7]", rt->spec_k);
  if (rt->max_batch < 1 || rt->max_batch * (rt->spec_k + 1) > kMaxTokens || rt->max_batch > kVerifyMaxBatch)
    return fail("max_batch=%d: need max_batch*(K+1) <= %d and max_batch <= %d", rt->max_batch, kMaxTokens, kVerifyMaxBatch);
  if (rt->spec_k > 0 && !draft && target->tp_rank == 0) return fail("spec_k>0 needs a draft model on rank 0");
  ssdk_engine* e = new ssdk_engine();
  e->rt = *rt;
  const ssdk_model_cfg* cfgs[2] = {target, draft};
  for (int w = 0; w < 2; ++w) {
    if (!cfgs[w]) continue;
    Model& m = e->model[w];
    m.cfg = *cfgs[w];
    m.present = true;
    const ssdk_model_cfg c = m.cfg;
    if (c.tp_size < 1 || c.heads % c.tp_size || c.kv_heads % c.tp_size || c.ffn % c.tp_size || c.vocab % c.tp_size) {
      delete e;
      return fail("model %d: tp_size %d does not divide heads/kv_heads/ffn/vocab", w, c.tp_size);
    }
    if (c.head_dim != 64 && c.head_dim != 128) {
      delete e;
      return fail("model %d: head_dim %d unsupported", w, c.head_dim);
    }
    if (c.hidden % 64 || (c.ffn / c.tp_size) % 64) {
      delete e;
      return fail("model %d: hidden/ffn must be multiples of 64", w);
    }
    derive(m);
    m.layers.resize(c.layers);
  }
  if (draft && draft->vocab != target->vocab) {
    delete e;
    return fail("draft and target vocab differ (model_runner.py:49)");
  }
  layout_step(e);
  e->max_ctx_hint = rt->max_blocks_per_seq * rt->block_size;
  if (cudaHostAlloc((void**)&e->pin_in, e->step_bytes, cudaHostAllocDefault) != cudaSuccess ||
      cudaHostAlloc((void**)&e->pin_out, e->out_bytes + 64 * 8, cudaHostAllocDefault) != cudaSuccess) {
    delete e;
    return fail("pinned staging allocation failed");
  }
  memset(e->pin_in, 0, e->step_bytes);
  e->fw_slot_bytes = align_up(e->step_bytes, 64) + kFwInBytes;
  if (cudaHostAlloc((void**)&e->pin_fw, e->fw_slot_bytes * ssdk_engine::kFwSlots, cudaHostAllocDefault) != cudaSuccess) {
    cudaFreeHost(e->pin_in);
    cudaFreeHost(e->pin_out);
    delete e;
    return fail("pinned staging allocation failed");
  }
  memset(e->pin_fw, 0, e->fw_slot_bytes * ssdk_engine::kFwSlots);
  for (int i = 0; i < ssdk_engine::kFwSlots; ++i) {
    if (cudaEventCreateWithFlags(&e->fw_ev[i], cudaEventDisableTiming) != cudaSuccess) {
      delete e;
      return fail("event creation failed");
    }
  }
  *out = e;
  return 0;
}

int ssdk_destroy(ssdk_handle h) {
  if (!h) return 0;
  for (auto& kv : h->spec_graphs) cudaGraphExecDestroy(kv.second);
  for (auto& kv : h->spec_graphs_resident) cudaGraphExecDestroy(kv.second);
  if (h->cap_stream) cudaStreamDestroy(h->cap_stream);
  if (h->pin_in) cudaFreeHost(h->pin_in);
  if (h->pin_out) cudaFreeHost(h->pin_out);
  if (h->pin_fw) cudaFreeHost(h->pin_fw);
  for (int i = 0; i < ssdk_engine::kFwSlots; ++i)
    if (h->fw_ev[i]) cudaEventDestroy(h->fw_ev[i]);
  delete h;
  return 0;
}

int ssdk_bind_weight(ssdk_handle h, int which, int kind, int layer, const void* dev_ptr, int64_t rows, int64_t cols) {
  if (!h || which < 0 || which > 1 || !h->model[which].present) return fail("bind_weight: bad handle/model");
  Model& m = h->model[which];
  if (!dev_ptr) return fail("bind_weight: null pointer");
  auto mat = [&](WeightMat& w, int64_t er, int64_t ec) -> int {
    if (rows != er || cols != ec)
      return fail("bind_weight kind %d layer %d: shape [%lld,%lld], expected [%lld,%lld]", kind, layer, (long long)rows,
                  (long long)cols, (long long)er, (long long)ec);
    w.ptr = (const bf16*)dev_ptr; w.rows = rows; w.cols = cols; w.has_tm = false;
    return 0;
  };
  auto vec = [&](const bf16** dst, int64_t n) -> int {
    if (rows * std::max<int64_t>(cols, 1) != n) return fail("bind_weight kind %d: %lld elements, expected %lld", kind,
                                                            (long long)(rows * std::max<int64_t>(cols, 1)), (long long)n);
    *dst = (const bf16*)dev_ptr;
    return 0;
  };
  const bool per_layer = kind >= SSDK_W_INPUT_NORM && kind <= SSDK_W_DOWN;
  if (per_layer && (layer < 0 || layer >= m.cfg.layers)) return fail("bind_weight: layer %d out of range", layer);
  switch (kind) {
    case SSDK_W_EMBED: return mat(m.embed, m.vocab_local, m.d);
    case SSDK_W_LM_HEAD: return mat(m.lm_head, m.vocab_local, m.d);
    case SSDK_W_FINAL_NORM: return vec(&m.final_norm, m.d);
    case SSDK_W_INPUT_NORM: return vec(&m.layers[layer].input_norm, m.d);
    case SSDK_W_QKV: return mat(m.layers[layer].qkv, m.qkv_dim, m.d);
    case SSDK_W_Q_NORM: return vec(&m.layers[layer].q_norm, m.hd);
    case SSDK_W_K_NORM: return vec(&m.layers[layer].k_norm, m.hd);
    case SSDK_W_O: return mat(m.layers[layer].o, m.d, (int64_t)m.H * m.hd);
    case SSDK_W_POST_NORM: return vec(&m.layers[layer].post_norm, m.d);
    case SSDK_W_GATE_UP: return mat(m.layers[layer].gate_up, 2 * (int64_t)m.ffn, m.d);
    case SSDK_W_DOWN: return mat(m.layers[layer].down, m.d, m.ffn);
    case SSDK_W_ROPE_TABLE:
      if (cols != m.hd) return fail("rope table width %lld != head_dim %d", (long long)cols, m.hd);
      m.rope = (const float*)dev_ptr;
      m.rope_rows = rows;
      return 0;
    default: return fail("bind_weight: unknown kind %d", kind);
  }
}

int ssdk_bind_kv_cache(ssdk_handle h, int which, void* kv_base, int64_t num_blocks) {
  if (!h || which < 0 || which > 1 || !h->model[which].present) return fail("bind_kv_cache: bad handle/model");
  Model& m = h->model[which];
  if (!kv_base || num_blocks < 1) return fail("bind_kv_cache: bad arguments");
  m.num_blocks = num_blocks;
  m.k_cache = (bf16*)kv_base;
  m.v_cache = m.k_cache + (size_t)m.cfg.layers * num_blocks * h->rt.block_size * m.KV * m.hd;
  return 0;
}

int64_t ssdk_workspace_bytes(ssdk_handle h) {
  if (!h) return fail("null handle");
  return carve(h, nullptr);
}
int ssdk_bind_workspace(ssdk_handle h, void* dev_ptr, int64_t bytes) {
  if (!h || !dev_ptr) return fail("bind_workspace: null");
  const int64_t need = carve(h, nullptr);
  if (bytes < need) return fail("workspace too small: %lld < %lld", (long long)bytes, (long long)need);
  if (((uintptr_t)dev_ptr & 1023) != 0) return fail("workspace must be 1024-byte aligned");
  carve(h, (uint8_t*)dev_ptr);
  h->ws_base = dev_ptr;
  h->ws_bytes = bytes;
  h->xmaps.maps.clear();
  return 0;
}

int ssdk_set_nccl_comm(ssdk_handle h, void* nccl_comm) {
  if (!h) return fail("null handle");
  h->comm = (ncclComm_t)nccl_comm;
  return 0;
}
int64_t ssdk_symm_bytes(ssdk_handle h) {
  if (!h) return fail("null handle");
  const Model& m = h->model[SSDK_TARGET];
  if (m.cfg.tp_size <= 1) return 0;
  const int64_t slot = (int64_t)kMaxTokens * m.d * 4;
  return 2 * kSymmMaxRanks * slot;
}
int ssdk_bind_symm(ssdk_handle h, void* const* peer_ptrs, int n_peers) {
  if (!h || !peer_ptrs) return fail("bind_symm: null argument");
  const Model& m = h->model[SSDK_TARGET];
  if (n_peers != m.cfg.tp_size || n_peers > kSymmMaxRanks) return fail("bind_symm: %d peers, tp_size %d", n_peers, m.cfg.tp_size);
  for (int r = 0; r < n_peers; ++r) {
    if (!peer_ptrs[r]) return fail("bind_symm: null peer pointer %d", r);
    h->symm_peer[r] = (uint8_t*)peer_ptrs[r];
  }
  h->symm_n = n_peers;
  h->symm_slot_bytes = (unsigned)((size_t)kMaxTokens * m.d * 4);
  return 0;
}

int ssdk_finalize(ssdk_handle h, void* stream) {
  if (!h) return fail("null handle");
  if (!h->ws_base) return fail("finalize: workspace not bound");
  cudaStream_t st = (cudaStream_t)stream;
  for (int w = 0; w < 2; ++w) {
    Model& m = h->model[w];
    if (!m.present) continue;
    if (!m.embed.ptr || !m.lm_head.ptr || !m.final_norm || !m.rope) return fail("model %d: embed/lm_head/final_norm/rope not bound", w);
    if (!m.k_cache) return fail("model %d: KV cache not bound", w);
    if (m.rope_rows < h->max_ctx_hint) return fail("model %d: rope table has %lld rows < max context %d", w, (long long)m.rope_rows, h->max_ctx_hint);
    for (int l = 0; l < m.cfg.layers; ++l) {
      LayerW& lw = m.layers[l];
      if (!lw.input_norm || !lw.post_norm || !lw.qkv.ptr || !lw.o.ptr || !lw.gate_up.ptr || !lw.down.ptr)
        return fail("model %d layer %d: weights missing", w, l);
      if (m.cfg.qk_norm && (!lw.q_norm || !lw.k_norm)) return fail("model %d layer %d: q/k norm missing", w, l);
      CKI(weight_tmap(lw.qkv));
      CKI(weight_tmap(lw.o));
      CKI(weight_tmap(lw.gate_up));
      CKI(weight_tmap(lw.down));
    }
    CKI(weight_tmap(m.lm_head));
  }
  CKI(init_kernel_attrs());
  CK(cudaMemsetAsync(h->ws_base, 0, (size_t)carve(h, nullptr), st));
  CK(cudaStreamSynchronize(st));
  h->finalized = true;
  return 0;
}

static int fill_step(ssdk_handle h, int batch, const int32_t* ctx_len, const int64_t* recovery, const int32_t* btt,
                     const int32_t* btd, const float* tt, const float* tq, uint64_t seed, uint64_t step_id) {
  if (batch < 1 || batch > h->rt.max_batch) return fail("batch %d out of range", batch);
  const int mbk = h->rt.max_blocks_per_seq;
  memcpy(h->pin_in + h->off_ctx, ctx_len, (size_t)batch * 4);
  memcpy(h->pin_in + h->off_rec, recovery, (size_t)batch * 8);
  memcpy(h->pin_in + h->off_tt, tt, (size_t)batch * 4);
  memcpy(h->pin_in + h->off_tq, tq, (size_t)batch * 4);
  uint64_t ss[2] = {seed, step_id};
  memcpy(h->pin_in + h->off_seed, ss, 16);
  memcpy(h->pin_in + h->off_btt, btt, (size_t)batch * mbk * 4);
  memcpy(h->pin_in + h->off_btd, btd, (size_t)batch * mbk * 4);
  return 0;
}
static void read_step(ssdk_handle h, int batch, int64_t* out_tokens, int32_t* out_n_accept, int64_t* out_recovery) {
  const int K = h->rt.spec_k;
  if (out_tokens) memcpy(out_tokens, h->pin_out, (size_t)batch * (K + 1) * 8);
  if (out_n_accept) memcpy(out_n_accept, h->pin_out + h->off_out_nacc, (size_t)batch * 4);
  if (out_recovery) memcpy(out_recovery, h->pin_out + h->off_out_rec, (size_t)batch * 8);
}

int ssdk_spec_step(ssdk_handle h, int batch, const int32_t* ctx_len, const int64_t* recovery,
                   const int32_t* block_tables_target, const int32_t* block_tables_draft, const float* temp_t,
                   const float* temp_q, uint64_t seed, uint64_t step_id, int64_t* out_tokens, int32_t* out_n_accept,
                   int64_t* out_recovery, void* stream) {
  if (!h || !h->finalized) return fail("spec_step: engine not finalized");
  if (h->rt.spec_k < 1) return fail("spec_step: engine built without speculation");
  cudaStream_t st = (cudaStream_t)stream;
  CKI(fill_step(h, batch, ctx_len, recovery, block_tables_target, block_tables_draft, temp_t, temp_q, seed, step_id));
  const bool stream_draft = use_draft_stream(h, batch, *std::max_element(ctx_len, ctx_len + batch));
  if (h->rt.use_graph) {
    cudaGraphExec_t g;
    int64_t n;
    CKI(get_spec_graph(h, batch, true, stream_draft, st, &g, &n));
    CK(cudaGraphLaunch(g, st));
    h->launches += n;
  } else {
    Launcher L;
    L.st = st;
    L.pdl = h->rt.use_pdl != 0;
    CKI(enqueue_spec_step(h, L, batch, true, false, stream_draft));
    h->launches += L.count;
  }
  CK(cudaStreamSynchronize(st));
  read_step(h, batch, out_tokens, out_n_accept, out_recovery);
  return 0;
}

int ssdk_spec_step_stage(ssdk_handle h, int batch, const int32_t* ctx_len, const int64_t* recovery,
                         const int32_t* block_tables_target, const int32_t* block_tables_draft, const float* temp_t,
                         const float* temp_q, uint64_t seed, uint64_t step_id, void* stream) {
  if (!h || !h->finalized) return fail("spec_step_stage: engine not finalized");
  cudaStream_t st = (cudaStream_t)stream;
  CKI(fill_step(h, batch, ctx_len, recovery, block_tables_target, block_tables_draft, temp_t, temp_q, seed, step_id));
  h->resident_ctx_bound = *std::max_element(ctx_len, ctx_len + batch);
  CK(cudaMemcpyAsync(h->ws.step_dev, h->pin_in, h->step_bytes, cudaMemcpyHostToDevice, st));
  CK(cudaMemsetAsync(h->ws.log_len, 0, (size_t)h->rt.max_batch * 4, st));
  CK(cudaStreamSynchronize(st));
  return 0;
}

int ssdk_spec_step_resident(ssdk_handle h, int batch, void* stream) {
  if (!h || !h->finalized) return fail("spec_step_resident: engine not finalized");
  if (h->rt.spec_k < 1) return fail("spec_step: engine built without speculation");
  cudaStream_t st = (cudaStream_t)stream;
  const bool stream_draft = use_draft_stream(h, batch, h->resident_ctx_bound);
  h->resident_ctx_bound += h->rt.spec_k + 1;
  if (h->rt.use_graph) {
    cudaGraphExec_t g;
    int64_t n;
    CKI(get_spec_graph(h, batch, false, stream_draft, st, &g, &n));
    CK(cudaGraphLaunch(g, st));
    h->launches += n;
  } else {
    Launcher L;
    L.st = st;
    L.pdl = h->rt.use_pdl != 0;
    CKI(enqueue_spec_step(h, L, batch, false, true, stream_draft));
    h->launches += L.count;
  }
  return 0;
}

int ssdk_spec_step_fetch(ssdk_handle h, int batch, int64_t* out_tokens, int32_t* out_n_accept, int64_t* out_recovery,
                         void* stream) {
  if (!h || !h->finalized) return fail("spec_step_fetch: engine not finalized");
  cudaStream_t st = (cudaStream_t)stream;
  CK(cudaMemcpyAsync(h->pin_out, h->ws.out_dev, h->out_bytes, cudaMemcpyDeviceToHost, st));
  int32_t* lens = (int32_t*)(h->pin_out + h->out_bytes);
  CK(cudaMemcpyAsync(lens, h->ws.log_len, (size_t)batch * 4, cudaMemcpyDeviceToHost, st));
  CK(cudaStreamSynchronize(st));
  read_step(h, batch, out_tokens, nullptr, out_recovery);
  if (out_n_accept) memcpy(out_n_accept, lens, (size_t)batch * 4);
  return 0;
}

int ssdk_spec_step_log(ssdk_handle h, int seq, int64_t* out_tokens, int cap, void* stream) {
  if (!h || !h->finalized) return fail("spec_step_log: engine not finalized");
  if (seq < 0 || seq >= h->rt.max_batch || !out_tokens || cap < 0) return fail("spec_step_log: bad arguments");
  cudaStream_t st = (cudaStream_t)stream;
  int32_t len = 0;
  CK(cudaMemcpyAsync(&len, h->ws.log_len + seq, 4, cudaMemcpyDeviceToHost, st));
  CK(cudaStreamSynchronize(st));
  const int n = std::min(std::min((int)len, cap), kLogCap);
  if (n > 0) {
    CK(cudaMemcpyAsync(out_tokens, h->ws.log_tokens + (size_t)seq * kLogCap, (size_t)n * 8, cudaMemcpyDeviceToHost, st));
    CK(cudaStreamSynchronize(st));
  }
  return n;
}

static int forward_call(ssdk_handle h, int which, int batch, int q_len, const int32_t* q_lens, const int64_t* ids,
                        const int32_t* ctx_len, const int32_t* block_tables, int want_sample, const float* temps,
                        uint64_t seed, uint64_t step_id, int64_t* out_tokens, void* stream) {
  cudaStream_t st = (cudaStream_t)stream;
  Workspace& w = h->ws;
  Model& m = h->model[which];
  const int mbk = h->rt.max_blocks_per_seq;
  VarlenFwd var;
  int M = batch * q_len;
  if (q_lens) {
    int32_t n_tiles = 0;
    const int rc = attn_make_plan_varlen(m.H, m.KV, batch, q_lens, h->max_ctx_hint, num_sms(), &var.plan, &n_tiles);
    if (rc == 1) return fail("unsupported GQA ratio %d/%d", m.H, m.KV);
    if (rc != 0) return fail("attention tile too large");
    var.n_tiles = n_tiles;
    M = 0;
    for (int b = 0; b < batch; ++b) M += q_lens[b];
    var.M = M;
    var.attn.cu_q = w.var_cu_q;
    var.attn.tiles = w.var_tiles;
  }
  const int slot = (int)(h->fw_next++ % ssdk_engine::kFwSlots);
  if (h->fw_ev_pending[slot]) {
    CK(cudaEventSynchronize(h->fw_ev[slot]));
    h->fw_ev_pending[slot] = false;
  }
  uint8_t* pin = h->pin_fw + (size_t)slot * h->fw_slot_bytes;
  memcpy(pin + h->off_ctx, ctx_len, (size_t)batch * 4);
  float zero[kVerifyMaxBatch] = {0};
  memcpy(pin + h->off_tt, temps ? temps : zero, (size_t)batch * 4);
  uint64_t ss[2] = {seed, step_id};
  memcpy(pin + h->off_seed, ss, 16);
  memcpy(pin + (which == SSDK_TARGET ? h->off_btt : h->off_btd), block_tables, (size_t)batch * mbk * 4);
  CK(cudaMemcpyAsync(w.step_dev, pin, h->step_bytes, cudaMemcpyHostToDevice, st));
  uint8_t* pin_in = pin + align_up(h->step_bytes, 64);
  memcpy(pin_in, ids, (size_t)M * 8);
  size_t in_bytes = (size_t)M * 8;
  if (q_lens) {
    attn_varlen_tiles(batch, q_lens, var.plan.TQ, (AttnTile*)(pin_in + kFwInTileOff), (int32_t*)(pin_in + kFwInCuOff));
    in_bytes = kFwInTileOff + (size_t)var.n_tiles * sizeof(AttnTile);
  }
  CK(cudaMemcpyAsync(w.ids_in, pin_in, in_bytes, cudaMemcpyHostToDevice, st));
  CK(cudaEventRecord(h->fw_ev[slot], st));
  h->fw_ev_pending[slot] = true;
  int64_t* pin_ids = (int64_t*)(h->pin_out + h->out_bytes);

  Launcher L;
  L.st = st;
  L.pdl = h->rt.use_pdl != 0;
  Fwd f;
  f.which = which; f.B = batch; f.Q = q_len; f.ids = w.ids_in; f.ids_stride = 1;
  f.ctx0 = (const int32_t*)(w.step_dev + h->off_ctx);
  f.block_tables = (const int32_t*)(w.step_dev + (which == SSDK_TARGET ? h->off_btt : h->off_btd));
  f.pos_offset = 0;
  f.logits_mode = want_sample ? 2 : 0;
  f.logits_out = w.logits_last;
  f.logits_ld = m.cfg.vocab;
  f.var = q_lens ? &var : nullptr;
  CKI(enqueue_forward(h, L, f));
  const bool do_sample = want_sample && m.cfg.tp_rank == 0;
  if (do_sample) {
    SampleParams sp;
    sp.logits = w.logits_last; sp.ld = m.cfg.vocab; sp.temps = (const float*)(w.step_dev + h->off_tt);
    sp.V = m.cfg.vocab; sp.seed = seed; sp.call_id = step_id * 16ull + 14ull; sp.out = w.out_tok; sp.out_stride = 1;
    sp.partial = w.samp_partial; sp.counters = w.samp_counters; sp.dyn = nullptr; sp.sub = 0;
    CKI(L.go(sample_kernel, dim3(kSampleChunks, batch), dim3(256), 0, sp));
  }
  if (want_sample) {
    if (m.cfg.tp_size > 1) CKN(ncclBroadcast(w.out_tok, w.out_tok, (size_t)batch, ncclInt64, 0, h->comm, st));
    CK(cudaMemcpyAsync(pin_ids, w.out_tok, (size_t)batch * 8, cudaMemcpyDeviceToHost, st));
    CK(cudaStreamSynchronize(st));
    if (out_tokens) memcpy(out_tokens, pin_ids, (size_t)batch * 8);
  }
  h->launches += L.count;
  return 0;
}

int ssdk_forward_tokens(ssdk_handle h, int which, int batch, int q_len, const int64_t* ids, const int32_t* ctx_len,
                        const int32_t* block_tables, int want_sample, const float* temps, uint64_t seed,
                        uint64_t step_id, int64_t* out_tokens, void* stream) {
  if (!h || !h->finalized) return fail("forward_tokens: engine not finalized");
  if (which < 0 || which > 1 || !h->model[which].present) return fail("forward_tokens: model %d absent", which);
  if (batch < 1 || batch > h->rt.max_batch || q_len < 1 || batch * q_len > kMaxTokens)
    return fail("forward_tokens: batch=%d q_len=%d out of range", batch, q_len);
  return forward_call(h, which, batch, q_len, nullptr, ids, ctx_len, block_tables, want_sample, temps, seed, step_id,
                      out_tokens, stream);
}

int ssdk_forward_varlen(ssdk_handle h, int which, int n_seqs, const int32_t* q_lens, const int64_t* ids,
                        const int32_t* ctx_len, const int32_t* block_tables, int want_sample, const float* temps,
                        uint64_t seed, uint64_t step_id, int64_t* out_tokens, void* stream) {
  if (!h || !h->finalized) return fail("forward_varlen: engine not finalized");
  if (which < 0 || which > 1 || !h->model[which].present) return fail("forward_varlen: model %d absent", which);
  if (n_seqs < 1 || n_seqs > h->rt.max_batch)
    return fail("forward_varlen: n_seqs=%d out of range [1, %d]", n_seqs, h->rt.max_batch);
  if (!q_lens || !ids || !ctx_len || !block_tables) return fail("forward_varlen: null argument");
  int total = 0;
  for (int b = 0; b < n_seqs; ++b) {
    if (q_lens[b] < 1) return fail("forward_varlen: q_lens[%d]=%d < 1", b, q_lens[b]);
    total += q_lens[b];
    if (total > kMaxTokens) return fail("forward_varlen: more than %d tokens in one call", kMaxTokens);
  }
  return forward_call(h, which, n_seqs, 0, q_lens, ids, ctx_len, block_tables, want_sample, temps, seed, step_id,
                      out_tokens, stream);
}

int ssdk_debug_trace(void* dev_buf, int cap) {
  unsigned long long* p = (unsigned long long*)dev_buf;
  unsigned c = (unsigned)cap, zero = 0;
  CK(cudaMemcpyToSymbol(g_trace_buf, &p, sizeof(p)));
  CK(cudaMemcpyToSymbol(g_trace_cap, &c, sizeof(c)));
  CK(cudaMemcpyToSymbol(g_trace_n, &zero, sizeof(zero)));
  return 0;
}

const void* ssdk_logits_p(ssdk_handle h) { return h ? h->ws.logits_p : nullptr; }
const void* ssdk_logits_q(ssdk_handle h) { return h ? h->ws.logits_q : nullptr; }
const void* ssdk_logits_last(ssdk_handle h) { return h ? h->ws.logits_last : nullptr; }
int64_t ssdk_launch_count(ssdk_handle h) { return h ? h->launches : 0; }

int ssdk_gemm_small_m(const void* x, const void* w, void* y, float* partials, int M, int N, int K, int ldy, int split_k,
                      void* stream) {
  if (M < 1 || M > kMaxTokens) return fail("gemm_small_m: M=%d out of [1,%d]", M, kMaxTokens);
  if (K % kBlockK) return fail("gemm_small_m: K must be a multiple of 64");
  Launcher L;
  L.st = (cudaStream_t)stream;
  CUtensorMap tmW, tmX;
  CKI(make_tmap(&tmW, w, N, K, 64));
  const int un = umma_n_for(M);
  CKI(make_tmap(&tmX, x, M, K, un));
  const int tiles = (N + kTileRows - 1) / kTileRows;
  const int num_kb = K / kBlockK;
  int S = split_k > 0 ? std::min(split_k, num_kb) : auto_splits(tiles, num_kb, un <= 64 ? 2 : 1);
  if (S > 1 && !partials) return fail("gemm_small_m: split_k=%d needs a partials buffer", S);
  GemmParams p;
  p.M = M; p.N = N; p.ldo = ldy; p.num_kb = num_kb; p.tile_rows = kTileRows; p.hi_row_offset = 64;
  p.kb_per_split = (num_kb + S - 1) / S;
  S = (num_kb + p.kb_per_split - 1) / p.kb_per_split;
  if (S == 1) {
    p.out = y;
    return launch_gemm(L, un, EPI_BF16, tmW, tmX, p, tiles, 1);
  }
  p.out = partials;
  CKI(launch_gemm(L, un, EPI_PARTIAL, tmW, tmX, p, tiles, S));
  const int n = M * N;
  return L.go(splitk_reduce_kernel, dim3((n + 255) / 256), dim3(256), 0, (const float*)partials, (bf16*)y, S, M, N, ldy);
}

int ssdk_gemm_gate_up_silu(const void* x, const void* w_gate_up, void* hout, int M, int ffn, int K, void* stream) {
  if (M < 1 || M > kMaxTokens) return fail("gemm_gate_up_silu: M=%d out of range", M);
  if (K % kBlockK || ffn % 8) return fail("gemm_gate_up_silu: K %% 64 or ffn %% 8 violated");
  Launcher L;
  L.st = (cudaStream_t)stream;
  CUtensorMap tmW, tmX;
  CKI(make_tmap(&tmW, w_gate_up, 2 * (int64_t)ffn, K, 64));
  const int un = umma_n_for(M);
  CKI(make_tmap(&tmX, x, M, K, un));
  GemmParams p;
  p.out = hout; p.M = M; p.N = ffn; p.ldo = ffn; p.num_kb = K / kBlockK; p.kb_per_split = p.num_kb;
  p.tile_rows = 64; p.hi_row_offset = ffn;
  return launch_gemm(L, un, EPI_SILU, tmW, tmX, p, (ffn + 63) / 64, 1);
}

int ssdk_rmsnorm(const void* x, const void* residual_in, const void* w, float eps, void* y, void* residual_out, int M,
                 int d, void* stream) {
  if (d % 8 || d > 16384) return fail("rmsnorm: d=%d unsupported", d);
  Launcher L;
  L.st = (cudaStream_t)stream;
  CKI(init_kernel_attrs());
  NormParams np;
  memset(&np, 0, sizeof(np));
  np.x.dense = (const bf16*)x; np.x.S = 0; np.x.M = M; np.x.N = d;
  np.residual_in = (const bf16*)residual_in; np.w = (const bf16*)w; np.eps = eps;
  np.y = (bf16*)y; np.residual_out = (bf16*)residual_out; np.d = d;
  return launch_norm(L, M, d, np);
}

int ssdk_rope_store_kv(const void* qkv, const int64_t* positions, const int32_t* slot_mapping, const float* rope_table,
                       const void* q_norm_w, const void* k_norm_w, float norm_eps, void* q_out, void* k_cache,
                       void* v_cache, int M, int heads, int kv_heads, int head_dim, void* stream) {
  if (head_dim > 256 || head_dim % 2) return fail("rope: head_dim %d unsupported", head_dim);
  Launcher L;
  L.st = (cudaStream_t)stream;
  RopeParams rp;
  rp.qkv.dense = (const bf16*)qkv; rp.qkv.partial = nullptr; rp.qkv.S = 0; rp.qkv.M = M;
  rp.qkv.N = (heads + 2 * kv_heads) * head_dim;
  rp.positions = positions; rp.slot_mapping = slot_mapping; rp.rope_table = rope_table;
  rp.q_norm_w = (const bf16*)q_norm_w; rp.k_norm_w = (const bf16*)k_norm_w; rp.norm_eps = norm_eps;
  rp.q_out = (bf16*)q_out; rp.k_cache = (bf16*)k_cache; rp.v_cache = (bf16*)v_cache;
  rp.heads = heads; rp.kv_heads = kv_heads; rp.head_dim = head_dim;
  return launch_rope(L, M, rp);
}

int ssdk_silu_mul(const void* gate_up, void* out, int M, int ffn, void* stream) {
  if (ffn % 8) return fail("silu_mul: ffn %% 8 != 0");
  Launcher L;
  L.st = (cudaStream_t)stream;
  GemmOut g;
  g.dense = (const bf16*)gate_up; g.partial = nullptr; g.S = 0; g.M = M; g.N = 2 * ffn;
  return L.go(silu_mul_kernel, dim3((M * ffn / 8 + 255) / 256), dim3(256), 0, g, (bf16*)out, M, ffn);
}

int ssdk_paged_attn_plan(int heads, int kv_heads, int batch, int q_len, int max_ctx, int* out4) {
  if (batch < 1 || q_len < 1 || kv_heads < 1 || out4 == nullptr) return fail("paged_attn_plan: bad arguments");
  return attn_plan_raw(heads, kv_heads, batch, q_len, max_ctx, &out4[0], &out4[1], &out4[2], &out4[3]);
}

int64_t ssdk_paged_attn_scratch_bytes(int batch, int q_len, int heads, int head_dim, int max_ctx) {
  (void)max_ctx;
  return (int64_t)batch * q_len * heads * kAttnMaxSplit * (head_dim + 1) * 4 + 1024 + 16384;
}

int ssdk_paged_attn(const void* q, const void* k_cache, const void* v_cache, const int32_t* block_tables,
                    const int32_t* context_lens, void* out, void* scratch, int batch, int q_len, int heads, int kv_heads,
                    int head_dim, int block_size, int max_blocks_per_seq, float scale, void* stream) {
  if (batch * q_len > kMaxTokens) return fail("paged_attn: too many query tokens");
  Launcher L;
  L.st = (cudaStream_t)stream;
  CKI(init_kernel_attrs());
  int TQ, MT, nqt, nsplit;
  CKI(attn_plan_raw(heads, kv_heads, batch, q_len, block_size * max_blocks_per_seq, &TQ, &MT, &nqt, &nsplit));
  CK(cudaMemsetAsync(scratch, 0, 16384, L.st));
  float* part_o = (float*)((uint8_t*)scratch + 16384);
  float* part_lse = part_o + (size_t)batch * q_len * heads * kAttnMaxSplit * head_dim;
  return enqueue_attention(L, (const bf16*)q, (const bf16*)k_cache, (const bf16*)v_cache, block_tables, context_lens,
                           (bf16*)out, part_o, part_lse, (unsigned*)scratch, batch, q_len, heads, kv_heads, head_dim, block_size,
                           max_blocks_per_seq, scale, TQ, MT, nqt, nsplit);
}

int ssdk_paged_attn_varlen_plan(int heads, int kv_heads, int batch, const int32_t* q_lens, int max_ctx, int* out5) {
  if (batch < 1 || batch > kMaxTokens || !q_lens || kv_heads < 1 || out5 == nullptr)
    return fail("paged_attn_varlen_plan: bad arguments");
  int total = 0;
  for (int b = 0; b < batch; ++b) {
    if (q_lens[b] < 1) return fail("paged_attn_varlen_plan: q_lens[%d]=%d < 1", b, q_lens[b]);
    total += q_lens[b];
  }
  if (total > kMaxTokens) return fail("paged_attn_varlen_plan: %d query tokens (max %d)", total, kMaxTokens);
  AttnPlan pl;
  const int rc = attn_make_plan_varlen(heads, kv_heads, batch, q_lens, max_ctx, num_sms(), &pl, &out5[4]);
  if (rc == 1) return fail("unsupported GQA ratio %d/%d", heads, kv_heads);
  if (rc != 0) return fail("attention tile too large");
  out5[0] = pl.TQ; out5[1] = pl.MT; out5[2] = pl.n_qtiles; out5[3] = pl.n_split;
  return 0;
}

// ... 68 lines not shown
```

### ssd_b200/lib.py

```python
from __future__ import annotations

import ctypes as C
import os
from pathlib import Path

_LIB_PATH = Path(__file__).resolve().parent / "_lib" / "libssdk.so"

c_i32p = C.POINTER(C.c_int32)
c_i64p = C.POINTER(C.c_int64)
c_f32p = C.POINTER(C.c_float)
VP = C.c_void_p


class ModelCfg(C.Structure):

    _fields_ = [
        ("hidden", C.c_int32), ("layers", C.c_int32), ("heads", C.c_int32), ("kv_heads", C.c_int32),
        ("head_dim", C.c_int32), ("ffn", C.c_int32), ("vocab", C.c_int32), ("qk_norm", C.c_int32),
        ("rms_eps", C.c_float), ("max_pos", C.c_int32), ("tp_size", C.c_int32), ("tp_rank", C.c_int32),
    ]


class RuntimeCfg(C.Structure):

    _fields_ = [
        ("spec_k", C.c_int32), ("max_batch", C.c_int32), ("block_size", C.c_int32),
        ("max_blocks_per_seq", C.c_int32), ("use_graph", C.c_int32), ("use_pdl", C.c_int32),
        ("jit_speculate", C.c_int32), ("reserved", C.c_int32),
    ]


W_EMBED, W_LM_HEAD, W_FINAL_NORM, W_INPUT_NORM, W_QKV, W_Q_NORM, W_K_NORM, W_O, W_POST_NORM, W_GATE_UP, W_DOWN, W_ROPE_TABLE = range(12)
TARGET, DRAFT = 0, 1

SIGNATURES: dict[str, tuple] = {
    "ssdk_abi_version": (C.c_int, []),
    "ssdk_last_error": (C.c_char_p, []),
    "ssdk_create": (C.c_int, [C.POINTER(ModelCfg), C.POINTER(ModelCfg), C.POINTER(RuntimeCfg), C.POINTER(VP)]),
    "ssdk_destroy": (C.c_int, [VP]),
    "ssdk_bind_weight": (C.c_int, [VP, C.c_int, C.c_int, C.c_int, VP, C.c_int64, C.c_int64]),
    "ssdk_bind_kv_cache": (C.c_int, [VP, C.c_int, VP, C.c_int64]),
    "ssdk_workspace_bytes": (C.c_int64, [VP]),
    "ssdk_bind_workspace": (C.c_int, [VP, VP, C.c_int64]),
    "ssdk_set_nccl_comm": (C.c_int, [VP, VP]),
    "ssdk_symm_bytes": (C.c_int64, [VP]),
    "ssdk_bind_symm": (C.c_int, [VP, C.POINTER(VP), C.c_int]),
    "ssdk_finalize": (C.c_int, [VP, VP]),
    "ssdk_spec_step": (C.c_int, [VP, C.c_int, c_i32p, c_i64p, c_i32p, c_i32p, c_f32p, c_f32p, C.c_uint64, C.c_uint64,
                                 c_i64p, c_i32p, c_i64p, VP]),
    "ssdk_spec_step_stage": (C.c_int, [VP, C.c_int, c_i32p, c_i64p, c_i32p, c_i32p, c_f32p, c_f32p, C.c_uint64,
                                       C.c_uint64, VP]),
    "ssdk_spec_step_resident": (C.c_int, [VP, C.c_int, VP]),
    "ssdk_spec_step_fetch": (C.c_int, [VP, C.c_int, c_i64p, c_i32p, c_i64p, VP]),
    "ssdk_spec_step_log": (C.c_int, [VP, C.c_int, c_i64p, C.c_int, VP]),
    "ssdk_forward_tokens": (C.c_int, [VP, C.c_int, C.c_int, C.c_int, c_i64p, c_i32p, c_i32p, C.c_int, c_f32p,
                                      C.c_uint64, C.c_uint64, c_i64p, VP]),
    "ssdk_forward_varlen": (C.c_int, [VP, C.c_int, C.c_int, c_i32p, c_i64p, c_i32p, c_i32p, C.c_int, c_f32p,
                                      C.c_uint64, C.c_uint64, c_i64p, VP]),
    "ssdk_logits_p": (VP, [VP]),
    "ssdk_logits_q": (VP, [VP]),
    "ssdk_logits_last": (VP, [VP]),
    "ssdk_debug_trace": (C.c_int, [VP, C.c_int]),
    "ssdk_launch_count": (C.c_int64, [VP]),
    "ssdk_gemm_small_m": (C.c_int, [VP, VP, VP, VP, C.c_int, C.c_int, C.c_int, C.c_int, C.c_int, VP]),
    "ssdk_gemm_gate_up_silu": (C.c_int, [VP, VP, VP, C.c_int, C.c_int, C.c_int, VP]),
    "ssdk_rmsnorm": (C.c_int, [VP, VP, VP, C.c_float, VP, VP, C.c_int, C.c_int, VP]),
    "ssdk_rope_store_kv": (C.c_int, [VP, VP, VP, VP, VP, VP, C.c_float, VP, VP, VP, C.c_int, C.c_int, C.c_int,
                                     C.c_int, VP]),
    "ssdk_silu_mul": (C.c_int, [VP, VP, C.c_int, C.c_int, VP]),
    "ssdk_paged_attn_scratch_bytes": (C.c_int64, [C.c_int, C.c_int, C.c_int, C.c_int, C.c_int]),
    "ssdk_paged_attn": (C.c_int, [VP, VP, VP, VP, VP, VP, VP, C.c_int, C.c_int, C.c_int, C.c_int, C.c_int, C.c_int,
                                  C.c_int, C.c_float, VP]),
    "ssdk_paged_attn_plan": (C.c_int, [C.c_int, C.c_int, C.c_int, C.c_int, C.c_int, c_i32p]),
    "ssdk_paged_attn_varlen": (C.c_int, [VP, VP, VP, VP, VP, c_i32p, VP, VP, C.c_int, C.c_int, C.c_int, C.c_int, C.c_int,
                                         C.c_int, C.c_float, VP]),
    "ssdk_paged_attn_varlen_plan": (C.c_int, [C.c_int, C.c_int, C.c_int, c_i32p, C.c_int, c_i32p]),
    "ssdk_sample": (C.c_int, [VP, C.c_int64, VP, C.c_int, C.c_int, C.c_uint64, C.c_uint64, VP, VP]),
    "ssdk_verify_scratch_bytes": (C.c_int64, [C.c_int, C.c_int]),
    "ssdk_verify": (C.c_int, [VP, VP, VP, VP, VP, VP, C.c_int, C.c_int, C.c_int, C.c_int, C.c_uint64, C.c_uint64,
                              VP, VP, VP, VP]),
}

_lib = None


def lib_path() -> Path:
    return _LIB_PATH


def load(build_if_missing: bool = True) -> C.CDLL:
    global _lib
    if _lib is not None:
        return _lib
    if build_if_missing:
        from . import build as _build

        try:
            if _build.is_stale():
                _build.build(verbose=False)
        except Exception as exc:
            if not _LIB_PATH.exists():
                raise RuntimeError(f"libssdk.so is missing and could not be built: {exc}") from exc
    if not _LIB_PATH.exists():
        raise RuntimeError(f"{_LIB_PATH} not found — run `python -m ssd_b200.build`; there is no CPU fallback")
    path = os.environ.get("SSDK_LIB") or str(_LIB_PATH)
    lib = C.CDLL(path, mode=os.RTLD_GLOBAL if hasattr(os, "RTLD_GLOBAL") else C.DEFAULT_MODE)
    for name, (res, args) in SIGNATURES.items():
        fn = getattr(lib, name)
        fn.restype = res
        fn.argtypes = args
    if lib.ssdk_abi_version() != 1:
        raise RuntimeError("libssdk.so ABI version mismatch")
    _lib = lib
    return lib


def last_error() -> str:
    return load().ssdk_last_error().decode("utf-8", "replace")


def check(rc: int, what: str = "ssdk call") -> None:
    if rc != 0:
        raise RuntimeError(f"{what} failed: {last_error()}")
```

### ssd_b200/runner.py

```python
from __future__ import annotations

import ctypes as C
from dataclasses import dataclass

import numpy as np
import torch

from . import lib as L


@dataclass
class ModelSpec:
    hidden: int
    layers: int
    heads: int
    kv_heads: int
    head_dim: int
    ffn: int
    vocab: int
    rms_eps: float = 1e-5
    rope_theta: float = 500000.0
    qk_norm: bool = False
    tie_embed: bool = False
    max_pos: int = 8192

    @classmethod
    def from_hf(cls, cfg) -> "ModelSpec":
        hd = getattr(cfg, "head_dim", None) or cfg.hidden_size // cfg.num_attention_heads
        theta = getattr(cfg, "rope_theta", None)
        if theta is None:
            rp = getattr(cfg, "rope_parameters", None) or {}
            theta = rp.get("rope_theta", 1000000.0 if "qwen" in cfg.model_type else 500000.0)
        return cls(hidden=cfg.hidden_size, layers=cfg.num_hidden_layers, heads=cfg.num_attention_heads,
                   kv_heads=cfg.num_key_value_heads, head_dim=hd, ffn=cfg.intermediate_size, vocab=cfg.vocab_size,
                   rms_eps=cfg.rms_norm_eps, rope_theta=float(theta), qk_norm=("qwen3" in cfg.model_type),
                   tie_embed=bool(getattr(cfg, "tie_word_embeddings", False)),
                   max_pos=cfg.max_position_embeddings)


def rope_table(head_dim: int, rows: int, base: float, device) -> torch.Tensor:
    inv_freq = 1.0 / (base ** (torch.arange(0, head_dim, 2, dtype=torch.float, device=device) / head_dim))
    t = torch.arange(rows, dtype=torch.float, device=device)
    freqs = torch.einsum("i,j -> ij", t, inv_freq)
    return torch.cat((freqs.cos(), freqs.sin()), dim=-1).contiguous()


def _i32(a):
    return np.ascontiguousarray(a, dtype=np.int32)


class PairRunner:
    def __init__(self, target: ModelSpec, draft: ModelSpec | None, *, spec_k: int, max_batch: int = 1,
                 block_size: int = 256, max_model_len: int = 4096, num_blocks_target: int | None = None,
                 num_blocks_draft: int | None = None, device: str | torch.device = "cuda:0", use_graph: bool = True,
                 use_pdl: bool = False, jit_speculate: bool = True, tp_size: int = 1, tp_rank: int = 0):
        if not torch.cuda.is_available():
            raise RuntimeError("PairRunner needs a CUDA device: libssdk has no CPU path")
        self.lib = L.load()
        self.device = torch.device(device)
        torch.cuda.set_device(self.device)
        self.spec = {L.TARGET: target, L.DRAFT: draft}
        self.K, self.max_batch, self.block_size = spec_k, max_batch, block_size
        self.max_blocks = (max_model_len + block_size - 1) // block_size
        self.max_model_len = max_model_len
        self.tp_size, self.tp_rank = tp_size, tp_rank
        self._keep: list[torch.Tensor] = []
        self.weights: dict[int, dict] = {}

        def cfg(m: ModelSpec, tp: int, rank: int) -> L.ModelCfg:
            return L.ModelCfg(m.hidden, m.layers, m.heads, m.kv_heads, m.head_dim, m.ffn, m.vocab, int(m.qk_norm),
                              m.rms_eps, self.max_blocks * block_size, tp, rank)

        tcfg = cfg(target, tp_size, tp_rank)
        dcfg = cfg(draft, 1, 0) if draft is not None else None
        rt = L.RuntimeCfg(spec_k, max_batch, block_size, self.max_blocks, int(use_graph),
                          int(use_pdl), int(jit_speculate), 0)
        h = C.c_void_p()
        L.check(self.lib.ssdk_create(C.byref(tcfg), C.byref(dcfg) if dcfg is not None else None, C.byref(rt),
                                     C.byref(h)), "ssdk_create")
        self.h = h
        self.kv = {}
        for which, m, nb, tp in ((L.TARGET, target, num_blocks_target, tp_size), (L.DRAFT, draft, num_blocks_draft, 1)):
            if m is None:
                continue
            nb = nb or max_batch * self.max_blocks
            kv = torch.zeros(2, m.layers, nb, block_size, m.kv_heads // tp, m.head_dim, dtype=torch.bfloat16,
                             device=self.device)
            self.kv[which] = kv
            L.check(self.lib.ssdk_bind_kv_cache(self.h, which, kv.data_ptr(), nb), "ssdk_bind_kv_cache")
            table = rope_table(m.head_dim, self.max_blocks * block_size, m.rope_theta, self.device)
            self._keep.append(table)
            L.check(self.lib.ssdk_bind_weight(self.h, which, L.W_ROPE_TABLE, 0, table.data_ptr(), table.shape[0],
                                              table.shape[1]), "bind rope table")
        nbytes = self.lib.ssdk_workspace_bytes(self.h)
        if nbytes <= 0:
            raise RuntimeError("ssdk_workspace_bytes failed: " + L.last_error())
        self.workspace = torch.zeros(nbytes + 1024, dtype=torch.uint8, device=self.device)
        off = (-self.workspace.data_ptr()) % 1024
        L.check(self.lib.ssdk_bind_workspace(self.h, self.workspace.data_ptr() + off, nbytes), "ssdk_bind_workspace")
        self.finalized = False
        self.step_id = 0

    def bind_weights(self, which: int, w: dict) -> None:
        lib, h = self.lib, self.h

        def bind(kind, layer, t):
            if t.dtype != torch.bfloat16 or not t.is_cuda or not t.is_contiguous():
                raise ValueError("weights must be contiguous bf16 CUDA tensors")
            rows, cols = (t.shape[0], t.shape[1]) if t.dim() == 2 else (t.shape[0], 1)
            L.check(lib.ssdk_bind_weight(h, which, kind, layer, t.data_ptr(), rows, cols), f"bind kind={kind} layer={layer}")

        bind(L.W_EMBED, 0, w["embed"])
        bind(L.W_LM_HEAD, 0, w["lm_head"])
        bind(L.W_FINAL_NORM, 0, w["final_norm"])
        for l, lw in enumerate(w["layers"]):
            bind(L.W_INPUT_NORM, l, lw["input_norm"])
            bind(L.W_QKV, l, lw["qkv"])
            bind(L.W_O, l, lw["o"])
            bind(L.W_POST_NORM, l, lw["post_norm"])
            bind(L.W_GATE_UP, l, lw["gate_up"])
            bind(L.W_DOWN, l, lw["down"])
            if "q_norm" in lw:
                bind(L.W_Q_NORM, l, lw["q_norm"])
                bind(L.W_K_NORM, l, lw["k_norm"])
        self.weights[which] = w

    def set_nccl_comm(self, comm_ptr: int) -> None:
        L.check(self.lib.ssdk_set_nccl_comm(self.h, C.c_void_p(comm_ptr)), "ssdk_set_nccl_comm")

    def finalize(self) -> None:
        L.check(self.lib.ssdk_finalize(self.h, torch.cuda.current_stream().cuda_stream), "ssdk_finalize")
        self.finalized = True

    def _bt(self, block_tables) -> np.ndarray:
        B = len(block_tables)
        out = np.full((B, self.max_blocks), -1, dtype=np.int32)
        for b, t in enumerate(block_tables):
            out[b, :len(t)] = t
        return out

    def forward_tokens(self, which: int, ids: list[list[int]], ctx_len: list[int], block_tables, temps=None,
                       want_sample: bool = True, seed: int = 0) -> list[int] | None:
        if self.spec[which] is None:
            return None
        B, Q = len(ids), len(ids[0])
        assert all(len(x) == Q for x in ids)
        ids_a = np.ascontiguousarray(np.array(ids, dtype=np.int64).reshape(-1))
        ctx_a, bt_a = _i32(ctx_len), self._bt(block_tables)
        temps_a = np.ascontiguousarray(temps if temps is not None else [0.0] * B, dtype=np.float32)
        out = np.zeros(B, dtype=np.int64)
        st = torch.cuda.current_stream().cuda_stream
        L.check(self.lib.ssdk_forward_tokens(self.h, which, B, Q, ids_a.ctypes.data_as(L.c_i64p),
                                             ctx_a.ctypes.data_as(L.c_i32p), bt_a.ctypes.data_as(L.c_i32p),
                                             int(want_sample), temps_a.ctypes.data_as(L.c_f32p), seed, self.step_id,
                                             out.ctypes.data_as(L.c_i64p), st), "ssdk_forward_tokens")
        self.step_id += 1
        return out.tolist() if want_sample else None

    def prefill(self, which: int, tokens: list[int], block_table: list[int], start: int = 0, temp: float = 0.0,
                want_sample: bool = True, chunk: int = 256, seed: int = 0):
        tok = None
        pos = start
        n = len(tokens)
        while pos < n:
            q = min(chunk, n - pos)
            last = pos + q == n
            tok = self.forward_tokens(which, [tokens[pos:pos + q]], [pos], [block_table], [temp],
                                      want_sample=(want_sample and last), seed=seed)
            pos += q
        return tok[0] if tok else None

    @staticmethod
    def plan_prefill_call(remaining: list[int], max_tokens: int, max_batch: int) -> tuple[list[int], int]:
        order = sorted((i for i, r in enumerate(remaining) if r > 0), key=lambda i: (-remaining[i], i))
        best, best_q = [], 0
        for nb in range(1, min(len(order), max_batch) + 1):
            q = min(max_tokens // nb, remaining[order[nb - 1]])
            if q < 1:
                break
            if nb * q > len(best) * best_q:
                best, best_q = order[:nb], q
        return sorted(best), best_q

    def prefill_many(self, which: int, tokens: list[list[int]], block_tables: list[list[int]], starts: list[int],
                     temps: list[float] | None = None, want_sample: bool = True, chunk: int = 256, seed: int = 0):
        n = len(tokens)
        pos = list(starts)
        temps = list(temps) if temps is not None else [0.0] * n
        out: list[int | None] = [None] * n
        packed = [i for i in range(n) if starts[i] == 0]
        while True:
            idx, q = self.plan_prefill_call([len(tokens[i]) - pos[i] if i in packed else 0 for i in range(n)],
                                            min(chunk, 256), self.max_batch)
            if not idx:
                break
            done = [pos[i] + q == len(tokens[i]) for i in idx]
            toks = self.forward_tokens(which, [tokens[i][pos[i]:pos[i] + q] for i in idx], [pos[i] for i in idx],
                                       [block_tables[i] for i in idx], [temps[i] for i in idx],
                                       want_sample=(want_sample and any(done)), seed=seed)
            for j, i in enumerate(idx):
                pos[i] += q
                if done[j] and toks is not None:
                    out[i] = toks[j]
        for i in range(n):
            if starts[i] != 0:
                out[i] = self.prefill(which, tokens[i], block_tables[i], start=starts[i], temp=temps[i],
                                      want_sample=want_sample, chunk=chunk, seed=seed)
        return out if want_sample else None

    def forward_varlen(self, which: int, ids: list[list[int]], ctx_len: list[int], block_tables, temps=None,
                       want_sample: bool = True, seed: int = 0) -> list[int] | None:
        if self.spec[which] is None:
            return None
        B = len(ids)
        q_a = _i32([len(x) for x in ids])
        ids_a = np.ascontiguousarray(np.fromiter((t for x in ids for t in x), dtype=np.int64, count=int(q_a.sum())))
        ctx_a, bt_a = _i32(ctx_len), self._bt(block_tables)
        temps_a = np.ascontiguousarray(temps if temps is not None else [0.0] * B, dtype=np.float32)
        out = np.zeros(B, dtype=np.int64)
        st = torch.cuda.current_stream().cuda_stream
        L.check(self.lib.ssdk_forward_varlen(self.h, which, B, q_a.ctypes.data_as(L.c_i32p), ids_a.ctypes.data_as(L.c_i64p),
                                             ctx_a.ctypes.data_as(L.c_i32p), bt_a.ctypes.data_as(L.c_i32p),
                                             int(want_sample), temps_a.ctypes.data_as(L.c_f32p), seed, self.step_id,
                                             out.ctypes.data_as(L.c_i64p), st), "ssdk_forward_varlen")
        self.step_id += 1
        return out.tolist() if want_sample else None

    @staticmethod
    def plan_varlen_calls(lens: list[int], starts: list[int], block_tables: list[list[int]], block_size: int,
                          max_tokens: int = 256, max_batch: int = 32) -> list[list[tuple[int, int, int]]]:
        n = len(lens)
        done = [min(s, l) for s, l in zip(starts, lens)]
        deps: list[list[tuple[int, int]]] = [[] for _ in range(n)]
        for i in range(n):
            if starts[i] <= 0:
                continue
            pages = set(p for p in block_tables[i][:(starts[i] + block_size - 1) // block_size] if p >= 0)
            for j in range(n):
                if j != i and pages.intersection(block_tables[j]):
                    deps[i].append((j, min(starts[i], lens[j])))
        calls = []
        while any(d < l for d, l in zip(done, lens)):
            call: dict[int, tuple[int, int]] = {}
            budget = max_tokens
            added = True
            while added and budget > 0 and len(call) < max_batch:
                added = False
                for i in range(n):
                    if i in call or done[i] >= lens[i] or budget == 0 or len(call) >= max_batch:
                        continue
                    if any(done[j] < need for j, need in deps[i]):
                        continue
                    q = min(lens[i] - done[i], budget)
                    call[i] = (done[i], q)
                    done[i] += q
                    budget -= q
                    added = True
            assert call, "varlen prefill planner made no progress"
            calls.append([(i, *call[i]) for i in sorted(call)])
        return calls

    def prefill_varlen(self, which: int, tokens: list[list[int]], block_tables: list[list[int]], starts: list[int],
                       temps: list[float] | None = None, want_sample: bool = True, seed: int = 0):
        n = len(tokens)
        temps = list(temps) if temps is not None else [0.0] * n
        out: list[int | None] = [None] * n
        for call in self.plan_varlen_calls([len(t) for t in tokens], starts, block_tables, self.block_size, 256,
                                           self.max_batch):
            ends = [pos + q == len(tokens[i]) for i, pos, q in call]
            toks = self.forward_varlen(which, [tokens[i][pos:pos + q] for i, pos, q in call], [pos for _, pos, _ in call],
                                       [block_tables[i] for i, _, _ in call], [temps[i] for i, _, _ in call],
                                       want_sample=(want_sample and any(ends)), seed=seed)
            for k, (i, _, _) in enumerate(call):
                if ends[k] and toks is not None:
                    out[i] = toks[k]
        return out if want_sample else None

    def spec_step(self, ctx_len: list[int], recovery: list[int], bt_target, bt_draft, temps_t: list[float],
                  temps_q: list[float], seed: int = 0):
        B, K = len(ctx_len), self.K
        ctx_a, rec_a = _i32(ctx_len), np.ascontiguousarray(recovery, dtype=np.int64)
        btt, btd = self._bt(bt_target), self._bt(bt_draft)
        tt, tq = np.ascontiguousarray(temps_t, dtype=np.float32), np.ascontiguousarray(temps_q, dtype=np.float32)
        toks = np.zeros((B, K + 1), dtype=np.int64)
        nacc = np.zeros(B, dtype=np.int32)
        rec = np.zeros(B, dtype=np.int64)
        st = torch.cuda.current_stream().cuda_stream
        L.check(self.lib.ssdk_spec_step(self.h, B, ctx_a.ctypes.data_as(L.c_i32p), rec_a.ctypes.data_as(L.c_i64p),
                                        btt.ctypes.data_as(L.c_i32p), btd.ctypes.data_as(L.c_i32p),
                                        tt.ctypes.data_as(L.c_f32p), tq.ctypes.data_as(L.c_f32p), seed, self.step_id,
                                        toks.ctypes.data_as(L.c_i64p), nacc.ctypes.data_as(L.c_i32p),
                                        rec.ctypes.data_as(L.c_i64p), st), "ssdk_spec_step")
        self.step_id += 1
        return toks, nacc, rec

    def stage(self, ctx_len, recovery, bt_target, bt_draft, temps_t, temps_q, seed: int = 0):
        B = len(ctx_len)
        ctx_a, rec_a = _i32(ctx_len), np.ascontiguousarray(recovery, dtype=np.int64)
        btt, btd = self._bt(bt_target), self._bt(bt_draft)
        tt, tq = np.ascontiguousarray(temps_t, dtype=np.float32), np.ascontiguousarray(temps_q, dtype=np.float32)
        st = torch.cuda.current_stream().cuda_stream
        L.check(self.lib.ssdk_spec_step_stage(self.h, B, ctx_a.ctypes.data_as(L.c_i32p), rec_a.ctypes.data_as(L.c_i64p),
                                              btt.ctypes.data_as(L.c_i32p), btd.ctypes.data_as(L.c_i32p),
                                              tt.ctypes.data_as(L.c_f32p), tq.ctypes.data_as(L.c_f32p), seed,
                                              self.step_id, st), "ssdk_spec_step_stage")

    def step_resident(self, batch: int) -> None:
        L.check(self.lib.ssdk_spec_step_resident(self.h, batch, torch.cuda.current_stream().cuda_stream),
                "ssdk_spec_step_resident")

    def fetch(self, batch: int):
        K = self.K
        toks = np.zeros((batch, K + 1), dtype=np.int64)
        total = np.zeros(batch, dtype=np.int32)
        rec = np.zeros(batch, dtype=np.int64)
        L.check(self.lib.ssdk_spec_step_fetch(self.h, batch, toks.ctypes.data_as(L.c_i64p), total.ctypes.data_as(L.c_i32p),
                                              rec.ctypes.data_as(L.c_i64p), torch.cuda.current_stream().cuda_stream),
                "ssdk_spec_step_fetch")
        return toks, total, rec

    def resident_log(self, seq: int = 0, cap: int = 16384) -> list[int]:
        out = np.zeros(cap, dtype=np.int64)
        n = self.lib.ssdk_spec_step_log(self.h, seq, out.ctypes.data_as(L.c_i64p), cap, torch.cuda.current_stream().cuda_stream)
        if n < 0:
            raise RuntimeError("ssdk_spec_step_log failed: " + L.last_error())
        return out[:n].tolist()

    def logits_p(self, batch: int) -> torch.Tensor:
        return _from_ptr(self.lib.ssdk_logits_p(self.h), (batch, self.K + 1, self.spec[L.TARGET].vocab), self.device)

    def logits_q(self, batch: int) -> torch.Tensor:
        return _from_ptr(self.lib.ssdk_logits_q(self.h), (batch, self.K, self.spec[L.TARGET].vocab), self.device)

    def logits_last(self, batch: int, which: int = L.TARGET) -> torch.Tensor:
        return _from_ptr(self.lib.ssdk_logits_last(self.h), (batch, self.spec[which].vocab), self.device)

    def step_io_bytes(self) -> tuple[int, int]:
        a = lambda n: (n + 15) // 16 * 16
        MB, mbk, K = self.max_batch, self.max_blocks, self.K
        h2d = a(MB * 4) + a(MB * 8) + 2 * a(MB * 4) + 16 + 2 * a(MB * mbk * 4)
        d2h = a(a(MB * (K + 1) * 8) + a(MB * 4) + MB * 8)
        return h2d, d2h

    @property
    def launch_count(self) -> int:
        return int(self.lib.ssdk_launch_count(self.h))

    def close(self) -> None:
        if getattr(self, "h", None):
            self.lib.ssdk_destroy(self.h)
            self.h = None

    def __del__(self):
        try:
            self.close()
        except Exception:
            pass


def _from_ptr(ptr: int, shape, device) -> torch.Tensor:
    n = int(np.prod(shape))

    class _Holder:
        pass

    holder = _Holder()
    holder.__cuda_array_interface__ = {"shape": (n,), "typestr": "<u2", "data": (int(ptr), False), "version": 3}
    t = torch.as_tensor(holder, device=device)
    return t.view(torch.bfloat16).view(*shape).clone()
```

Before: 358.5.

## Fold pending draft KV catch-up token into next step's first draft forward

When all K drafts are accepted, the bonus token's draft KV entry is missing. Instead of running a separate draft forward right away, the runner records it as pending. The next spec step then processes it as a second row inside the streaming draft kernel's first forward, reusing the same weight stream for both rows. This is meant to remove a separate draft forward launch and its weight reads. The cost is extra arithmetic and attention work in the first forward, plus host-side bookkeeping to match pending tokens to sequences.

```diff
diff --git a/include/ssdk.h b/include/ssdk.h
--- a/include/ssdk.h
+++ b/include/ssdk.h
@@ -78,7 +78,7 @@
 
 
 int ssdk_spec_step(ssdk_handle h, int batch,
-                   const int32_t* ctx_len, const int64_t* recovery,
+                   const int32_t* ctx_len, const int64_t* recovery, const int64_t* pending,
                    const int32_t* block_tables_target, const int32_t* block_tables_draft,
                    const float* temp_t, const float* temp_q,
                    uint64_t seed, uint64_t step_id,
@@ -86,7 +86,7 @@
                    void* stream);
 
 int ssdk_spec_step_stage(ssdk_handle h, int batch,
-                         const int32_t* ctx_len, const int64_t* recovery,
+                         const int32_t* ctx_len, const int64_t* recovery, const int64_t* pending,
                          const int32_t* block_tables_target, const int32_t* block_tables_draft,
                          const float* temp_t, const float* temp_q,
                          uint64_t seed, uint64_t step_id, void* stream);
diff --git a/ssd_b200/csrc/draft_stream.cuh b/ssd_b200/csrc/draft_stream.cuh
--- a/ssd_b200/csrc/draft_stream.cuh
+++ b/ssd_b200/csrc/draft_stream.cuh
@@ -45,7 +45,31 @@
   unsigned* attn_ticket;
   int n_slots;
   DsLayer layers[kDsMaxLayers];
-};
+  const int64_t* pend_tok;
+  __nv_bfloat16* vec_row0;
+};
+
+struct DsVecs {
+  __nv_bfloat16 *qkv, *attn, *o, *down, *resid0, *resid1, *act;
+  SSDK_DEVINL __nv_bfloat16* resid(int i) const { return i ? resid1 : resid0; }
+};
+SSDK_DEVINL DsVecs ds_row0_vecs(const DsParams& p, int hd) {
+  DsVecs v{};
+  __nv_bfloat16* b = p.vec_row0;
+  if (!b) return v;
+  v.qkv = b; b += ((p.H + 2 * p.KV) * hd + 7) / 8 * 8;
+  v.attn = b; b += p.H * hd;
+  v.o = b; b += p.d;
+  v.down = b; b += p.d;
+  v.resid0 = b; b += p.d;
+  v.resid1 = b; b += p.d;
+  v.act = b;
+  return v;
+}
+__host__ SSDK_DEVINL int ds_xs_floats(int d, int ffn, int q_width) {
+  const int a = 2 * d > ffn ? 2 * d : ffn;
+  return a > q_width ? a : q_width;
+}
 
 SSDK_DEVINL void ds_sync() {
 #ifdef SSDK_HOST_EMU
@@ -230,16 +254,54 @@
   return logit * s.invT - __logf(e);
 }
 
-template <bool HEAD>
-SSDK_DEVINL void ds_consume_plain(DsRing& ring, const DsGeom& g, const float* xs, __nv_bfloat16* y, DsSample* smp) {
+struct DsRow0 {
+  const float* xs;
+  const __nv_bfloat16* xg;
+  __nv_bfloat16* y;
+};
+SSDK_DEVINL float ds_dot_seg0(const uint8_t* wseg, int steps, int lane, const float* x0) {
+  const uint4* wp = reinterpret_cast<const uint4*>(wseg) + lane;
+  float a0 = 0.f, a1 = 0.f, a2 = 0.f, a3 = 0.f;
+#pragma unroll 2
+  for (int j = 0; j < steps; ++j) {
+    const float4 u = *reinterpret_cast<const float4*>(x0 + j * 256 + lane * 8);
+    const float4 v = *reinterpret_cast<const float4*>(x0 + j * 256 + lane * 8 + 4);
+    const uint4 w = wp[j * 32];
+    float2 f = ds_bf2(w.x);
+    a0 = fmaf(f.x, u.x, a0); a1 = fmaf(f.y, u.y, a1);
+    f = ds_bf2(w.y);
+    a2 = fmaf(f.x, u.z, a2); a3 = fmaf(f.y, u.w, a3);
+    f = ds_bf2(w.z);
+    a0 = fmaf(f.x, v.x, a0); a1 = fmaf(f.y, v.y, a1);
+    f = ds_bf2(w.w);
+    a2 = fmaf(f.x, v.z, a2); a3 = fmaf(f.y, v.w, a3);
+  }
+  return warp_sum((a0 + a1) + (a2 + a3));
+}
+SSDK_DEVINL void ds_load_vec(const __nv_bfloat16* v, int n, float* xs);
+SSDK_DEVINL const float* ds_row0_x(const DsRow0& r, float* xs, int n) {
+  if (r.xs) return r.xs;
+  ds_sync();
+  ds_load_vec(r.xg, n, xs);
+  return xs;
+}
+
+template <bool HEAD, bool TWO = false>
+SSDK_DEVINL void ds_consume_plain(DsRing& ring, const DsGeom& g, float* xs, __nv_bfloat16* y, DsSample* smp,
+                                  const DsRow0& r0 = DsRow0{}) {
+  static_assert(!(HEAD && TWO), "row 0 has no lm_head");
   if ((int)blockIdx.x >= g.nj) return;
   const int warp = threadIdx.x >> 5, lane = threadIdx.x & 31;
   const int steps = g.K >> 8;
   float xr[kDsMaxSteps][8];
   ds_load_x(xs, steps, lane, xr);
+  const float* x0 = nullptr;
+  if constexpr (TWO) x0 = ds_row0_x(r0, xs, g.K);
   for (int s = (int)blockIdx.x; s < g.nj; s += (int)gridDim.x) {
     const uint8_t* st = ds_acquire(ring, 0);
     const float acc = ds_dot_seg(st + (size_t)warp * g.K * 2, steps, lane, xr);
+    float acc0 = 0.f;
+    if constexpr (TWO) acc0 = ds_dot_seg0(st + (size_t)warp * g.K * 2, steps, lane, x0);
     ds_release(ring, 0, lane);
     ring.taken += 1u;
     const int row = s * 8 + warp;
@@ -247,6 +309,7 @@
       const __nv_bfloat16 o = f2bf(acc);
       if (!HEAD) {
         y[row] = o;
+        if constexpr (TWO) r0.y[row] = f2bf(acc0);
       } else {
         if (y) y[row] = o;
         smp->best = argmax_better(smp->best, ArgMax{ds_score(*smp, bf2f(o), row), row});
@@ -254,44 +317,64 @@
     }
   }
 }
-SSDK_DEVINL void ds_consume_pair(DsRing& ring, const DsGeom& g, const float* xs, __nv_bfloat16* act) {
+SSDK_DEVINL float ds_silu_mul(float gate, float up) {
+  gate = bf16_round(gate);
+  up = bf16_round(up);
+  return (gate / (1.0f + __expf(-gate))) * up;
+}
+template <bool TWO>
+SSDK_DEVINL void ds_consume_pair(DsRing& ring, const DsGeom& g, float* xs, __nv_bfloat16* act, const DsRow0& r0) {
   if ((int)blockIdx.x >= g.nj) return;
   const int warp = threadIdx.x >> 5, lane = threadIdx.x & 31;
   const int steps = g.K >> 8;
   float xr[kDsMaxSteps][8];
   ds_load_x(xs, steps, lane, xr);
+  const float* x0 = nullptr;
+  if constexpr (TWO) x0 = ds_row0_x(r0, xs, g.K);
   for (int s = (int)blockIdx.x; s < g.nj; s += (int)gridDim.x) {
+    float gate0 = 0.f, up0 = 0.f;
     const uint8_t* sg = ds_acquire(ring, 0);
-    float gate = ds_dot_seg(sg + (size_t)warp * g.K * 2, steps, lane, xr);
+    const float gate = ds_dot_seg(sg + (size_t)warp * g.K * 2, steps, lane, xr);
+    if constexpr (TWO) gate0 = ds_dot_seg0(sg + (size_t)warp * g.K * 2, steps, lane, x0);
     ds_release(ring, 0, lane);
     const uint8_t* su = ds_acquire(ring, 1);
-    float up = ds_dot_seg(su + (size_t)warp * g.K * 2, steps, lane, xr);
+    const float up = ds_dot_seg(su + (size_t)warp * g.K * 2, steps, lane, xr);
+    if constexpr (TWO) up0 = ds_dot_seg0(su + (size_t)warp * g.K * 2, steps, lane, x0);
     ds_release(ring, 1, lane);
     ring.taken += 2u;
     const int i = s * 8 + warp;
     if (lane == 0 && i < g.rows) {
-      gate = bf16_round(gate);
-      up = bf16_round(up);
-      act[i] = f2bf((gate / (1.0f + __expf(-gate))) * up);
-    }
-  }
-}
-SSDK_DEVINL void ds_consume_split(DsRing& ring, const DsGeom& g, const float* xs, float* res, __nv_bfloat16* y) {
+      act[i] = f2bf(ds_silu_mul(gate, up));
+      if constexpr (TWO) r0.y[i] = f2bf(ds_silu_mul(gate0, up0));
+    }
+  }
+}
+template <bool TWO>
+SSDK_DEVINL void ds_consume_split(DsRing& ring, const DsGeom& g, float* xs, float* res, __nv_bfloat16* y,
+                                  const DsRow0& r0) {
   if ((int)blockIdx.x >= g.nj) return;
   const int warp = threadIdx.x >> 5, lane = threadIdx.x & 31;
   const int row_in_job = warp / g.segs, seg = warp - row_in_job * g.segs;
   const int seg_len = g.K / g.segs, steps = seg_len >> 8;
   float xr[kDsMaxSteps][8];
   ds_load_x(xs + seg * seg_len, steps, lane, xr);
+  const float* x0 = nullptr;
+  if constexpr (TWO) x0 = ds_row0_x(r0, xs, g.K);
   const size_t w_off = ((size_t)row_in_job * g.K + (size_t)seg * seg_len) * 2;
   unsigned it = 0;
   for (int s = (int)blockIdx.x; s < g.nj; s += (int)gridDim.x, ++it) {
     const uint8_t* st = ds_acquire(ring, 0);
     const float acc = ds_dot_seg(st + w_off, steps, lane, xr);
+    float acc0 = 0.f;
+    if constexpr (TWO) acc0 = ds_dot_seg0(st + w_off, steps, lane, x0 + seg * seg_len);
     ds_release(ring, 0, lane);
     ring.taken += 1u;
     float* rb = res + (it & 1u) * kDsWarps;
-    if (lane == 0) rb[warp] = acc;
+    float* rb0 = rb + 2 * kDsWarps;
+    if (lane == 0) {
+      rb[warp] = acc;
+      if constexpr (TWO) rb0[warp] = acc0;
+    }
     ds_sync();
     if ((int)threadIdx.x < g.rpj) {
       const int row = s * g.rpj + (int)threadIdx.x;
@@ -299,13 +382,28 @@
         float v = 0.f;
         for (int q = 0; q < g.segs; ++q) v += rb[(int)threadIdx.x * g.segs + q];
         y[row] = f2bf(v);
-      }
-    }
-  }
-}
-SSDK_DEVINL void ds_consume(DsRing& ring, const DsGeom& g, const float* xs, float* res, __nv_bfloat16* y) {
-  if (g.kind == DS_PLAIN) ds_consume_plain<false>(ring, g, xs, y, nullptr);
-  else ds_consume_split(ring, g, xs, res, y);
+        if constexpr (TWO) {
+          float v0 = 0.f;
+          for (int q = 0; q < g.segs; ++q) v0 += rb0[(int)threadIdx.x * g.segs + q];
+          r0.y[row] = f2bf(v0);
+        }
+      }
+    }
+  }
+}
+SSDK_DEVINL void ds_consume(DsRing& ring, const DsGeom& g, float* xs, float* res, __nv_bfloat16* y, bool two,
+                            const DsRow0& r0) {
+  if (g.kind == DS_PLAIN) {
+    if (two) ds_consume_plain<false, true>(ring, g, xs, y, nullptr, r0);
+    else ds_consume_plain<false>(ring, g, xs, y, nullptr);
+  } else {
+    if (two) ds_consume_split<true>(ring, g, xs, res, y, r0);
+    else ds_consume_split<false>(ring, g, xs, res, y, r0);
+  }
+}
+SSDK_DEVINL void ds_consume_gu(DsRing& ring, const DsGeom& g, float* xs, __nv_bfloat16* act, bool two, const DsRow0& r0) {
+  if (two) ds_consume_pair<true>(ring, g, xs, act, r0);
+  else ds_consume_pair<false>(ring, g, xs, act, r0);
 }
 
 SSDK_DEVINL float ds_block_sum(float v, float* red) {
@@ -407,8 +505,8 @@
   }
 }
 template <int HD, int GMAX, int TB>
-SSDK_DEVINL void ds_attention_unit(const DsParams& p, int layer, int h, int s, int ns, int ctx, float* sm, int* flag,
-                                   const int* bt_s) {
+SSDK_DEVINL void ds_attention_unit(const DsParams& p, const __nv_bfloat16* vqkv, __nv_bfloat16* vattn, int layer, int h,
+                                   int s, int ns, int ctx, float* sm, int* flag, const int* bt_s) {
   constexpr int HALF = HD / 2;
   constexpr int EPL = HD / 32;
   const int warp = threadIdx.x >> 5, lane = threadIdx.x & 31;
@@ -437,8 +535,8 @@
       const int i = lane + 32 * t;
       x1[t] = x2[t] = 0.f;
       if (i < HALF) {
-        const unsigned short a = __ldcg(reinterpret_cast<const unsigned short*>(p.vec_qkv + col0 + i));
-        const unsigned short b = __ldcg(reinterpret_cast<const unsigned short*>(p.vec_qkv + col0 + HALF + i));
+        const unsigned short a = __ldcg(reinterpret_cast<const unsigned short*>(vqkv + col0 + i));
+        const unsigned short b = __ldcg(reinterpret_cast<const unsigned short*>(vqkv + col0 + HALF + i));
         x1[t] = __bfloat162float(__ushort_as_bfloat16(a));
         x2[t] = __bfloat162float(__ushort_as_bfloat16(b));
         ss += x1[t] * x1[t] + x2[t] * x2[t];
@@ -565,7 +663,7 @@
       }
     }
     if (ns == 1) {
-      p.vec_attn[(size_t)(h * G + g) * HD + dim] = f2bf(ll > 0.f ? o / ll : 0.f);
+      vattn[(size_t)(h * G + g) * HD + dim] = f2bf(ll > 0.f ? o / ll : 0.f);
     } else {
       float* out = p.attn_part + ((size_t)(h * G + g) * kDsSplits + s) * LDR;
       out[dim] = o;
@@ -604,7 +702,7 @@
         o += os[q] * wt;
         l += ls[q] * wt;
       }
-      p.vec_attn[(size_t)(h * G + g) * HD + dim] = f2bf(l > 0.f ? o / l : 0.f);
+      vattn[(size_t)(h * G + g) * HD + dim] = f2bf(l > 0.f ? o / l : 0.f);
     }
   }
   ds_sync();
@@ -618,13 +716,13 @@
   SSDK_STATIC_SMEM(uint64_t, empty_bar, kDsMaxSlots);
   SSDK_STATIC_SMEM(DsGeom, geom, 5);
   SSDK_STATIC_SMEM(float, red, 32);
-  SSDK_STATIC_SMEM(float, res, 2 * kDsWarps);
+  SSDK_STATIC_SMEM(float, res, 4 * kDsWarps);
   SSDK_STATIC_SMEM(ArgMax, ared, 32);
   SSDK_SHARED_VAR(int, tok_s);
   SSDK_SHARED_VAR(int, flag_s);
   SSDK_STATIC_SMEM(int, bt_s, kDsBtSmem);
   float* xs = reinterpret_cast<float*>(ds_smem + (size_t)p.n_slots * kDsSlotBytes);
-  float* scratch = xs + max(max(p.d, p.ffn), p.H * HD);
+  float* scratch = xs + ds_xs_floats(p.d, p.ffn, p.H * HD);
   if (threadIdx.x < kDsBtSmem && (int)threadIdx.x < p.max_blocks) bt_s[threadIdx.x] = p.block_table[threadIdx.x];
   if (threadIdx.x == 0) {
     trace_mark(TR_MISC);
@@ -663,23 +761,29 @@
   const uint64_t call0 = p.dyn ? p.dyn[1] * 16ull : p.call_base;
   __nv_bfloat16* resid[2] = {p.resid0, p.resid1};
   long long tok = p.tok_buf[0];
+  const long long tok0 = p.pend_tok ? p.pend_tok[0] : -1;
+  const DsVecs v0 = ds_row0_vecs(p, HD);
 
   for (int f = 0; f < p.n_fwd; ++f) {
     if (threadIdx.x == 0 && f > 0) trace_mark(TR_MISC);
     const int ctx = ctx_base + f + 1;
     const __nv_bfloat16* emb = p.embed + (size_t)tok * p.d;
+    const bool two = f == 0 && tok0 >= 0;
     int cur = 0;
     DsPre pre;
     for (int l = 0; l < p.L; ++l) {
       const DsLayer& lw = p.layers[l];
       if (l == 0) {
+        if (two) ds_norm_prologue(p.embed + (size_t)tok0 * p.d, nullptr, v0.resid(cur ^ 1), lw.in_norm, p.eps, p.d, xs + p.d, red,
+                                  nullptr);
         ds_norm_prologue(emb, nullptr, resid[cur ^ 1], lw.in_norm, p.eps, p.d, xs, red, nullptr);
       } else {
+        if (two) ds_norm_prologue(v0.down, v0.resid(cur), v0.resid(cur ^ 1), lw.in_norm, p.eps, p.d, xs + p.d, red, nullptr);
         ds_norm_prologue(p.vec_down, resid[cur], resid[cur ^ 1], lw.in_norm, p.eps, p.d, xs, red, &pre);
       }
       cur ^= 1;
       ds_mark(f, 0);
-      ds_consume(ring, geom[DS_QKV], xs, res, p.vec_qkv);
+      ds_consume(ring, geom[DS_QKV], xs, res, p.vec_qkv, two, DsRow0{xs + p.d, nullptr, v0.qkv});
       ds_mark(f, 1);
       bar.sync();
       ds_mark(f, 2);
@@ -687,29 +791,40 @@
       bar.sync();
       ds_mark(f, 12);
 #endif
+      if (two) {
+        const int ns0 = ds_num_splits(ctx - 1);
+        for (int u = blockIdx.x; u < p.KV * ns0; u += gridDim.x) {
+          if (ns0 == kDsSplits)
+            ds_attention_unit<HD, GMAX, 8>(p, v0.qkv, v0.attn, l, u / ns0, u % ns0, ns0, ctx - 1, scratch, &flag_s, bt_s);
+          else ds_attention_unit<HD, GMAX, 4>(p, v0.qkv, v0.attn, l, u / ns0, u % ns0, ns0, ctx - 1, scratch, &flag_s, bt_s);
+        }
+        bar.sync();
+      }
       const int ns = ds_num_splits(ctx);
       for (int u = blockIdx.x; u < p.KV * ns; u += gridDim.x) {
-        if (ns == kDsSplits) ds_attention_unit<HD, GMAX, 8>(p, l, u / ns, u % ns, ns, ctx, scratch, &flag_s, bt_s);
-        else ds_attention_unit<HD, GMAX, 4>(p, l, u / ns, u % ns, ns, ctx, scratch, &flag_s, bt_s);
+        if (ns == kDsSplits)
+          ds_attention_unit<HD, GMAX, 8>(p, p.vec_qkv, p.vec_attn, l, u / ns, u % ns, ns, ctx, scratch, &flag_s, bt_s);
+        else ds_attention_unit<HD, GMAX, 4>(p, p.vec_qkv, p.vec_attn, l, u / ns, u % ns, ns, ctx, scratch, &flag_s, bt_s);
       }
       ds_mark(f, 3);
       bar.sync();
       ds_mark(f, 4);
       ds_load_vec(p.vec_attn, p.H * HD, xs);
-      ds_consume(ring, geom[DS_O], xs, res, p.vec_o);
+      ds_consume(ring, geom[DS_O], xs, res, p.vec_o, two, DsRow0{nullptr, v0.attn, v0.o});
       ds_mark(f, 5);
       pre = ds_preload(resid[cur], lw.post_norm, p.d);
       bar.sync();
       ds_mark(f, 6);
+      if (two) ds_norm_prologue(v0.o, v0.resid(cur), v0.resid(cur ^ 1), lw.post_norm, p.eps, p.d, xs + p.d, red, nullptr);
       ds_norm_prologue(p.vec_o, resid[cur], resid[cur ^ 1], lw.post_norm, p.eps, p.d, xs, red, &pre);
       cur ^= 1;
       ds_mark(f, 7);
-      ds_consume_pair(ring, geom[DS_GU], xs, p.vec_act);
+      ds_consume_gu(ring, geom[DS_GU], xs, p.vec_act, two, DsRow0{xs + p.d, nullptr, v0.act});
       ds_mark(f, 8);
       bar.sync();
       ds_mark(f, 9);
       ds_load_vec(p.vec_act, p.ffn, xs);
-      ds_consume(ring, geom[DS_DOWN], xs, res, p.vec_down);
+      ds_consume(ring, geom[DS_DOWN], xs, res, p.vec_down, two, DsRow0{nullptr, v0.act, v0.down});
       ds_mark(f, 10);
       pre = ds_preload(resid[cur], l + 1 < p.L ? p.layers[l + 1].in_norm : p.final_norm, p.d);
       bar.sync();
diff --git a/ssd_b200/csrc/elementwise.cuh b/ssd_b200/csrc/elementwise.cuh
--- a/ssd_b200/csrc/elementwise.cuh
+++ b/ssd_b200/csrc/elementwise.cuh
@@ -89,6 +89,7 @@
 
 __global__ void prep_kernel(const int32_t* __restrict__ ctx0, const int32_t* __restrict__ block_tables,
                             int max_blocks, int block_size, int batch, int q_len, int pos_offset,
+                            const int64_t* __restrict__ pend,
                             int64_t* __restrict__ positions, int32_t* __restrict__ slot_mapping,
                             int32_t* __restrict__ context_lens, unsigned* __restrict__ fwd_seq) {
   pdl_launch_dependents();
@@ -100,7 +101,8 @@
     const int pos = ctx0[b] + pos_offset + j;
     positions[i] = pos;
     const int blk = block_tables[(size_t)b * max_blocks + pos / block_size];
-    slot_mapping[i] = (blk < 0) ? -1 : blk * block_size + pos % block_size;
+    const bool masked = pend && j == 0 && pend[b] < 0;
+    slot_mapping[i] = (blk < 0 || masked) ? -1 : blk * block_size + pos % block_size;
   }
   if (i < batch) context_lens[i] = ctx0[i] + pos_offset + q_len;
   if (fwd_seq && i == 0) *fwd_seq += 1u;
diff --git a/ssd_b200/csrc/engine.cu b/ssd_b200/csrc/engine.cu
--- a/ssd_b200/csrc/engine.cu
+++ b/ssd_b200/csrc/engine.cu
@@ -233,6 +233,7 @@
   int32_t *slot_mapping, *context_lens;
   uint8_t* out_dev;
   int64_t* tok_buf;
+  int64_t* fold_ids;
   int64_t* ids_in;
   int32_t* var_cu_q;
   AttnTile* var_tiles;
@@ -251,6 +252,7 @@
   unsigned* ver_counters;
   size_t partial_floats = 0;
   bf16* ds_vec;
+  bf16* ds_vec0;
   float* ds_attn;
   unsigned* ds_sync;
 };
@@ -282,7 +284,7 @@
   unsigned fw_next = 0;
   size_t step_bytes = 0;
   size_t out_bytes = 0;
-  size_t off_ctx, off_rec, off_tt, off_tq, off_seed, off_btt, off_btd;
+  size_t off_ctx, off_rec, off_pend, off_tt, off_tq, off_seed, off_btt, off_btd;
   size_t off_out_nacc, off_out_rec;
   std::map<int, cudaGraphExec_t> spec_graphs;
   std::map<int, int64_t> spec_graph_launches;
@@ -307,6 +309,8 @@
   m.qkv_dim = (m.H + 2 * m.KV) * m.hd;
   m.vocab_local = c.vocab / c.tp_size;
 }
+
+static size_t ds_vec_elems(int qkv, int d, int ffn, int q_width) { return (size_t)qkv + 4 * d + ffn + q_width + 64; }
 
 static int64_t carve(ssdk_engine* e, uint8_t* base) {
   size_t off = 0;
@@ -378,7 +382,10 @@
   w.ver_rows = (RowPart*)take((size_t)kVerifyMaxRows * kVerifyCtas * sizeof(RowPart));
   w.ver_rec = (RecPart*)take((size_t)kVerifyMaxBatch * kVerifyCtas * sizeof(RecPart));
   w.ver_counters = (unsigned*)take(64);
-  w.ds_vec = (bf16*)take((size_t)(qmax + 4 * dmax + fmax + Hmax * hdmax + 64) * 2);
+  const size_t ds_elems = ds_vec_elems(qmax, dmax, fmax, Hmax * hdmax);
+  w.ds_vec = (bf16*)take(ds_elems * 2);
+  w.ds_vec0 = (bf16*)take(ds_elems * 2);
+  w.fold_ids = (int64_t*)take((size_t)MB * 2 * 8);
   w.ds_attn = (float*)take((size_t)Hmax * kDsSplits * (hdmax + 2) * 4);
   w.ds_sync = (unsigned*)take(256);
   return (int64_t)align_up(off, 1024);
@@ -402,6 +409,7 @@
   bf16* logits_out;
   int64_t logits_ld;
   const VarlenFwd* var = nullptr;
+  const int64_t* pend = nullptr;
 };
 
 static int attn_plan_raw(int H, int KV, int B, int Q, int max_ctx, int* TQ, int* MT, int* nqt, int* nsplit) {
@@ -601,7 +609,7 @@
              w.positions, w.slot_mapping, w.context_lens, fwd_seq));
     TQ = f.var->plan.TQ; MT = f.var->plan.MT; nqt = f.var->plan.n_qtiles; nsplit = f.var->plan.n_split;
   } else {
-    CKI(L.go(prep_kernel, dim3(1), dim3(kMaxTokens), 0, f.ctx0, f.block_tables, mb, bs, f.B, f.Q, f.pos_offset,
+    CKI(L.go(prep_kernel, dim3(1), dim3(kMaxTokens), 0, f.ctx0, f.block_tables, mb, bs, f.B, f.Q, f.pos_offset, f.pend,
              w.positions, w.slot_mapping, w.context_lens, fwd_seq));
     CKI(attn_plan(m, f.B, f.Q, &TQ, &MT, &nqt, &nsplit, e->max_ctx_hint));
   }
@@ -759,6 +767,7 @@
   auto take = [&](size_t n) { size_t o = off; off = align_up(off + n, 16); return o; };
   e->off_ctx = take((size_t)MB * 4);
   e->off_rec = take((size_t)MB * 8);
+  e->off_pend = take((size_t)MB * 8);
   e->off_tt = take((size_t)MB * 4);
   e->off_tq = take((size_t)MB * 4);
   e->off_seed = take(16);
@@ -772,17 +781,22 @@
 
 
 
-__global__ void init_tokens_kernel(const int64_t* __restrict__ recovery, int64_t* __restrict__ tok_buf, int B, int Kp1) {
+__global__ void init_tokens_kernel(const int64_t* __restrict__ recovery, const int64_t* __restrict__ pend,
+                                   int64_t* __restrict__ tok_buf, int64_t* __restrict__ fold_ids, int B, int Kp1) {
   pdl_launch_dependents();
   pdl_wait();
   const int b = threadIdx.x;
-  if (b < B) tok_buf[(size_t)b * Kp1] = recovery[b];
-}
-
-__global__ void advance_kernel(int32_t* __restrict__ ctx, int64_t* __restrict__ recovery_in, uint64_t* __restrict__ seed_step,
-                               const int64_t* __restrict__ tok_buf, const int32_t* __restrict__ n_accept,
-                               const int64_t* __restrict__ recovery_out, int64_t* __restrict__ log_tokens,
-                               int32_t* __restrict__ log_len, int B, int Kp1, int log_cap) {
+  if (b < B) {
+    tok_buf[(size_t)b * Kp1] = recovery[b];
+    fold_ids[2 * b] = pend[b] >= 0 ? pend[b] : recovery[b];
+    fold_ids[2 * b + 1] = recovery[b];
+  }
+}
+
+__global__ void advance_kernel(int32_t* __restrict__ ctx, int64_t* __restrict__ recovery_in, int64_t* __restrict__ pend,
+                               uint64_t* __restrict__ seed_step, const int64_t* __restrict__ tok_buf,
+                               const int32_t* __restrict__ n_accept, const int64_t* __restrict__ recovery_out,
+                               int64_t* __restrict__ log_tokens, int32_t* __restrict__ log_len, int B, int Kp1, int log_cap) {
   pdl_launch_dependents();
   pdl_wait();
   const int b = threadIdx.x;
@@ -793,6 +807,7 @@
     log_len[b] = len;
     ctx[b] += n;
     recovery_in[b] = recovery_out[b];
+    pend[b] = (n == Kp1) ? tok_buf[(size_t)b * Kp1 + Kp1 - 1] : -1;
   }
   if (threadIdx.x == 0) seed_step[1] += 1;
 }
@@ -805,7 +820,7 @@
 constexpr int kMaxDynSmem = 227 * 1024 - 2048;
 static size_t ds_fixed_smem(const Model& m) {
   const int G = m.H / m.KV, gmax = G <= 4 ? 4 : 8;
-  const size_t xs = (size_t)std::max(std::max(m.d, m.ffn), m.H * m.hd);
+  const size_t xs = (size_t)ds_xs_floats(m.d, m.ffn, m.H * m.hd);
   const size_t scratch = (size_t)gmax * m.hd + 2 * m.hd + (size_t)kDsWarps * gmax * (m.hd + 2);
   return (xs + scratch) * 4 + 256;
 }
@@ -856,7 +871,7 @@
   ++L.count;
   return 0;
 }
-static int enqueue_draft_stream(ssdk_engine* e, Launcher& L, int64_t* tok_buf, int n_fwd, bool skip_last_head,
+static int enqueue_draft_stream(ssdk_engine* e, Launcher& L, int64_t* tok_buf, int n_fwd, const int64_t* pend,
                                 const int32_t* ctx0, const int32_t* block_table, const float* temp, const uint64_t* dyn,
                                 bf16* logits, int64_t logits_ld) {
   Model& m = e->model[SSDK_DRAFT];
@@ -870,7 +885,8 @@
   p.k_cache = m.k_cache; p.v_cache = m.v_cache;
   p.cache_layer_stride = (long long)m.num_blocks * e->rt.block_size * m.KV * m.hd;
   p.block_size = e->rt.block_size; p.max_blocks = e->rt.max_blocks_per_seq;
-  p.tok_buf = tok_buf; p.n_fwd = n_fwd; p.skip_last_head = skip_last_head ? 1 : 0;
+  p.tok_buf = tok_buf; p.n_fwd = n_fwd; p.skip_last_head = 0;
+  p.pend_tok = pend; p.vec_row0 = w.ds_vec0;
   p.ctx0 = ctx0; p.block_table = block_table;
   bf16* v = w.ds_vec;
   p.vec_qkv = v; v += align_up((size_t)m.qkv_dim, 8);
@@ -911,6 +927,7 @@
   }
   int32_t* ctx = (int32_t*)(w.step_dev + e->off_ctx);
   int64_t* rec_in = (int64_t*)(w.step_dev + e->off_rec);
+  int64_t* pend = (int64_t*)(w.step_dev + e->off_pend);
   const float* tt = (const float*)(w.step_dev + e->off_tt);
   const float* tq = (const float*)(w.step_dev + e->off_tq);
   uint64_t* seed_step = (uint64_t*)(w.step_dev + e->off_seed);
@@ -920,24 +937,27 @@
   const int tp = tgt.cfg.tp_size, tp_rank = tgt.cfg.tp_rank;
   if (tp > 1 && !e->comm) return fail("tensor parallel spec step without a NCCL communicator");
   if (tp_rank == 0 && !drf.present) return fail("rank 0 needs the draft model");
-  if (drf.present) CKI(L.go(init_tokens_kernel, dim3(1), dim3(64), 0, (const int64_t*)rec_in, w.tok_buf, B, K + 1));
+  if (drf.present)
+    CKI(L.go(init_tokens_kernel, dim3(1), dim3(64), 0, (const int64_t*)rec_in, (const int64_t*)pend, w.tok_buf, w.fold_ids,
+             B, K + 1));
   if (stream_draft)
-    CKI(enqueue_draft_stream(e, L, w.tok_buf, K + 1, true, ctx, btd, tq, seed_step, w.logits_q, (int64_t)V));
-  for (int k = 0; k <= K && drf.present && !stream_draft; ++k) {
+    CKI(enqueue_draft_stream(e, L, w.tok_buf, K, pend, ctx, btd, tq, seed_step, w.logits_q, (int64_t)V));
+  for (int k = 0; k < K && drf.present && !stream_draft; ++k) {
     Fwd f;
     f.which = SSDK_DRAFT; f.B = B; f.Q = 1; f.ids = w.tok_buf + k; f.ids_stride = K + 1;
     f.ctx0 = ctx; f.block_tables = btd; f.pos_offset = k;
-    f.logits_mode = (k < K) ? 1 : 0;
+    f.logits_mode = 1;
+    if (k == 0) {
+      f.Q = 2; f.ids = w.fold_ids; f.ids_stride = 1; f.pos_offset = -1; f.logits_mode = 2; f.pend = pend;
+    }
     f.logits_out = w.logits_q + (size_t)k * V;
     f.logits_ld = (int64_t)K * V;
     CKI(enqueue_forward(e, L, f));
-    if (k < K) {
-      SampleParams sp;
-      sp.logits = w.logits_q + (size_t)k * V; sp.ld = (int64_t)K * V; sp.temps = tq; sp.V = drf.cfg.vocab;
-      sp.seed = 0; sp.call_id = 0; sp.out = w.tok_buf + k + 1; sp.out_stride = K + 1;
-      sp.partial = w.samp_partial; sp.counters = w.samp_counters; sp.dyn = seed_step; sp.sub = k;
-      CKI(L.go(sample_kernel, dim3(kSampleChunks, B), dim3(256), 0, sp));
-    }
+    SampleParams sp;
+    sp.logits = w.logits_q + (size_t)k * V; sp.ld = (int64_t)K * V; sp.temps = tq; sp.V = drf.cfg.vocab;
+    sp.seed = 0; sp.call_id = 0; sp.out = w.tok_buf + k + 1; sp.out_stride = K + 1;
+    sp.partial = w.samp_partial; sp.counters = w.samp_counters; sp.dyn = seed_step; sp.sub = k;
+    CKI(L.go(sample_kernel, dim3(kSampleChunks, B), dim3(256), 0, sp));
   }
   if (tp > 1) {
     CKN(ncclBroadcast(w.tok_buf, w.tok_buf, (size_t)B * (K + 1), ncclInt64, 0, e->comm, L.st));
@@ -964,7 +984,7 @@
     L.barrier_op();
   }
   if (advance) {
-    CKI(L.go(advance_kernel, dim3(1), dim3(64), 0, ctx, rec_in, seed_step, (const int64_t*)w.tok_buf,
+    CKI(L.go(advance_kernel, dim3(1), dim3(64), 0, ctx, rec_in, pend, seed_step, (const int64_t*)w.tok_buf,
              (const int32_t*)w.n_accept, (const int64_t*)w.recovery, w.log_tokens, w.log_len, B, K + 1, kLogCap));
   }
   if (host_io) {
@@ -1241,12 +1261,18 @@
   return 0;
 }
 
-static int fill_step(ssdk_handle h, int batch, const int32_t* ctx_len, const int64_t* recovery, const int32_t* btt,
-                     const int32_t* btd, const float* tt, const float* tq, uint64_t seed, uint64_t step_id) {
+static int fill_step(ssdk_handle h, int batch, const int32_t* ctx_len, const int64_t* recovery, const int64_t* pending,
+                     const int32_t* btt, const int32_t* btd, const float* tt, const float* tq, uint64_t seed,
+                     uint64_t step_id) {
   if (batch < 1 || batch > h->rt.max_batch) return fail("batch %d out of range", batch);
   const int mbk = h->rt.max_blocks_per_seq;
   memcpy(h->pin_in + h->off_ctx, ctx_len, (size_t)batch * 4);
   memcpy(h->pin_in + h->off_rec, recovery, (size_t)batch * 8);
+  int64_t* pend = (int64_t*)(h->pin_in + h->off_pend);
+  for (int b = 0; b < batch; ++b) {
+    pend[b] = pending ? pending[b] : -1;
+    if (pend[b] >= 0 && ctx_len[b] < 1) return fail("spec_step: sequence %d has a pending token but no context", b);
+  }
   memcpy(h->pin_in + h->off_tt, tt, (size_t)batch * 4);
   memcpy(h->pin_in + h->off_tq, tq, (size_t)batch * 4);
   uint64_t ss[2] = {seed, step_id};
@@ -1262,14 +1288,15 @@
   if (out_recovery) memcpy(out_recovery, h->pin_out + h->off_out_rec, (size_t)batch * 8);
 }
 
-int ssdk_spec_step(ssdk_handle h, int batch, const int32_t* ctx_len, const int64_t* recovery,
+int ssdk_spec_step(ssdk_handle h, int batch, const int32_t* ctx_len, const int64_t* recovery, const int64_t* pending,
                    const int32_t* block_tables_target, const int32_t* block_tables_draft, const float* temp_t,
                    const float* temp_q, uint64_t seed, uint64_t step_id, int64_t* out_tokens, int32_t* out_n_accept,
                    int64_t* out_recovery, void* stream) {
   if (!h || !h->finalized) return fail("spec_step: engine not finalized");
   if (h->rt.spec_k < 1) return fail("spec_step: engine built without speculation");
   cudaStream_t st = (cudaStream_t)stream;
-  CKI(fill_step(h, batch, ctx_len, recovery, block_tables_target, block_tables_draft, temp_t, temp_q, seed, step_id));
+  CKI(fill_step(h, batch, ctx_len, recovery, pending, block_tables_target, block_tables_draft, temp_t, temp_q, seed,
+                step_id));
   const bool stream_draft = use_draft_stream(h, batch, *std::max_element(ctx_len, ctx_len + batch));
   if (h->rt.use_graph) {
     cudaGraphExec_t g;
@@ -1289,12 +1316,13 @@
   return 0;
 }
 
-int ssdk_spec_step_stage(ssdk_handle h, int batch, const int32_t* ctx_len, const int64_t* recovery,
+int ssdk_spec_step_stage(ssdk_handle h, int batch, const int32_t* ctx_len, const int64_t* recovery, const int64_t* pending,
                          const int32_t* block_tables_target, const int32_t* block_tables_draft, const float* temp_t,
                          const float* temp_q, uint64_t seed, uint64_t step_id, void* stream) {
   if (!h || !h->finalized) return fail("spec_step_stage: engine not finalized");
   cudaStream_t st = (cudaStream_t)stream;
-  CKI(fill_step(h, batch, ctx_len, recovery, block_tables_target, block_tables_draft, temp_t, temp_q, seed, step_id));
+  CKI(fill_step(h, batch, ctx_len, recovery, pending, block_tables_target, block_tables_draft, temp_t, temp_q, seed,
+                step_id));
   h->resident_ctx_bound = *std::max_element(ctx_len, ctx_len + batch);
   CK(cudaMemcpyAsync(h->ws.step_dev, h->pin_in, h->step_bytes, cudaMemcpyHostToDevice, st));
   CK(cudaMemsetAsync(h->ws.log_len, 0, (size_t)h->rt.max_batch * 4, st));
diff --git a/ssd_b200/lib.py b/ssd_b200/lib.py
--- a/ssd_b200/lib.py
+++ b/ssd_b200/lib.py
@@ -46,9 +46,9 @@
     "ssdk_symm_bytes": (C.c_int64, [VP]),
     "ssdk_bind_symm": (C.c_int, [VP, C.POINTER(VP), C.c_int]),
     "ssdk_finalize": (C.c_int, [VP, VP]),
-    "ssdk_spec_step": (C.c_int, [VP, C.c_int, c_i32p, c_i64p, c_i32p, c_i32p, c_f32p, c_f32p, C.c_uint64, C.c_uint64,
-                                 c_i64p, c_i32p, c_i64p, VP]),
-    "ssdk_spec_step_stage": (C.c_int, [VP, C.c_int, c_i32p, c_i64p, c_i32p, c_i32p, c_f32p, c_f32p, C.c_uint64,
+    "ssdk_spec_step": (C.c_int, [VP, C.c_int, c_i32p, c_i64p, c_i64p, c_i32p, c_i32p, c_f32p, c_f32p, C.c_uint64,
+                                 C.c_uint64, c_i64p, c_i32p, c_i64p, VP]),
+    "ssdk_spec_step_stage": (C.c_int, [VP, C.c_int, c_i32p, c_i64p, c_i64p, c_i32p, c_i32p, c_f32p, c_f32p, C.c_uint64,
                                        C.c_uint64, VP]),
     "ssdk_spec_step_resident": (C.c_int, [VP, C.c_int, VP]),
     "ssdk_spec_step_fetch": (C.c_int, [VP, C.c_int, c_i64p, c_i32p, c_i64p, VP]),
diff --git a/ssd_b200/runner.py b/ssd_b200/runner.py
--- a/ssd_b200/runner.py
+++ b/ssd_b200/runner.py
@@ -100,6 +100,7 @@
         L.check(self.lib.ssdk_bind_workspace(self.h, self.workspace.data_ptr() + off, nbytes), "ssdk_bind_workspace")
         self.finalized = False
         self.step_id = 0
+        self._pending: list[tuple[int, int, tuple[int, ...]]] = []
 
     def bind_weights(self, which: int, w: dict) -> None:
         lib, h = self.lib, self.h
@@ -143,6 +144,8 @@
                        want_sample: bool = True, seed: int = 0) -> list[int] | None:
         if self.spec[which] is None:
             return None
+        if which == L.DRAFT:
+            self.flush_draft()
         B, Q = len(ids), len(ids[0])
         assert all(len(x) == Q for x in ids)
         ids_a = np.ascontiguousarray(np.array(ids, dtype=np.int64).reshape(-1))
@@ -212,6 +215,8 @@
                        want_sample: bool = True, seed: int = 0) -> list[int] | None:
         if self.spec[which] is None:
             return None
+        if which == L.DRAFT:
+            self.flush_draft()
         B = len(ids)
         q_a = _i32([len(x) for x in ids])
         ids_a = np.ascontiguousarray(np.fromiter((t for x in ids for t in x), dtype=np.int64, count=int(q_a.sum())))
@@ -279,6 +284,16 @@
     def spec_step(self, ctx_len: list[int], recovery: list[int], bt_target, bt_draft, temps_t: list[float],
                   temps_q: list[float], seed: int = 0):
         B, K = len(ctx_len), self.K
+        pend = np.full(B, -1, dtype=np.int64)
+        rest = list(self._pending)
+        for b in range(B):
+            for i, (pos, tok, pages) in enumerate(rest):
+                if ctx_len[b] == pos + 1 and tuple(bt_draft[b][:len(pages)]) == pages:
+                    pend[b] = tok
+                    del rest[i]
+                    break
+        self._pending = rest
+        self.flush_draft()
         ctx_a, rec_a = _i32(ctx_len), np.ascontiguousarray(recovery, dtype=np.int64)
         btt, btd = self._bt(bt_target), self._bt(bt_draft)
         tt, tq = np.ascontiguousarray(temps_t, dtype=np.float32), np.ascontiguousarray(temps_q, dtype=np.float32)
@@ -287,21 +302,43 @@
         rec = np.zeros(B, dtype=np.int64)
         st = torch.cuda.current_stream().cuda_stream
         L.check(self.lib.ssdk_spec_step(self.h, B, ctx_a.ctypes.data_as(L.c_i32p), rec_a.ctypes.data_as(L.c_i64p),
-                                        btt.ctypes.data_as(L.c_i32p), btd.ctypes.data_as(L.c_i32p),
-                                        tt.ctypes.data_as(L.c_f32p), tq.ctypes.data_as(L.c_f32p), seed, self.step_id,
-                                        toks.ctypes.data_as(L.c_i64p), nacc.ctypes.data_as(L.c_i32p),
-                                        rec.ctypes.data_as(L.c_i64p), st), "ssdk_spec_step")
+                                        pend.ctypes.data_as(L.c_i64p), btt.ctypes.data_as(L.c_i32p),
+                                        btd.ctypes.data_as(L.c_i32p), tt.ctypes.data_as(L.c_f32p),
+                                        tq.ctypes.data_as(L.c_f32p), seed, self.step_id, toks.ctypes.data_as(L.c_i64p),
+                                        nacc.ctypes.data_as(L.c_i32p), rec.ctypes.data_as(L.c_i64p), st), "ssdk_spec_step")
         self.step_id += 1
+        if self.spec[L.DRAFT] is not None:
+            for b in range(B):
+                if int(nacc[b]) == K:
+                    pos = ctx_len[b] + K
+                    self._pending.append((pos, int(toks[b, K]), tuple(bt_draft[b][:pos // self.block_size + 1])))
         return toks, nacc, rec
 
+    def flush_draft(self) -> None:
+        if not self._pending or self.spec[L.DRAFT] is None:
+            self._pending = []
+            return
+        recs, self._pending = self._pending, []
+        B = len(recs)
+        ids_a = np.ascontiguousarray([tok for _, tok, _ in recs], dtype=np.int64)
+        ctx_a, bt_a = _i32([pos for pos, _, _ in recs]), self._bt([list(pages) for _, _, pages in recs])
+        temps_a = np.zeros(B, dtype=np.float32)
+        out = np.zeros(B, dtype=np.int64)
+        L.check(self.lib.ssdk_forward_tokens(self.h, L.DRAFT, B, 1, ids_a.ctypes.data_as(L.c_i64p),
+                                             ctx_a.ctypes.data_as(L.c_i32p), bt_a.ctypes.data_as(L.c_i32p), 0,
+                                             temps_a.ctypes.data_as(L.c_f32p), 0, self.step_id,
+                                             out.ctypes.data_as(L.c_i64p), torch.cuda.current_stream().cuda_stream),
+                "ssdk_forward_tokens (draft flush)")
+
     def stage(self, ctx_len, recovery, bt_target, bt_draft, temps_t, temps_q, seed: int = 0):
+        self.flush_draft()
         B = len(ctx_len)
         ctx_a, rec_a = _i32(ctx_len), np.ascontiguousarray(recovery, dtype=np.int64)
         btt, btd = self._bt(bt_target), self._bt(bt_draft)
         tt, tq = np.ascontiguousarray(temps_t, dtype=np.float32), np.ascontiguousarray(temps_q, dtype=np.float32)
         st = torch.cuda.current_stream().cuda_stream
         L.check(self.lib.ssdk_spec_step_stage(self.h, B, ctx_a.ctypes.data_as(L.c_i32p), rec_a.ctypes.data_as(L.c_i64p),
-                                              btt.ctypes.data_as(L.c_i32p), btd.ctypes.data_as(L.c_i32p),
+                                              None, btt.ctypes.data_as(L.c_i32p), btd.ctypes.data_as(L.c_i32p),
                                               tt.ctypes.data_as(L.c_f32p), tq.ctypes.data_as(L.c_f32p), seed,
                                               self.step_id, st), "ssdk_spec_step_stage")
 
@@ -338,7 +375,7 @@
     def step_io_bytes(self) -> tuple[int, int]:
         a = lambda n: (n + 15) // 16 * 16
         MB, mbk, K = self.max_batch, self.max_blocks, self.K
-        h2d = a(MB * 4) + a(MB * 8) + 2 * a(MB * 4) + 16 + 2 * a(MB * mbk * 4)
+        h2d = a(MB * 4) + 2 * a(MB * 8) + 2 * a(MB * 4) + 16 + 2 * a(MB * mbk * 4)
         d2h = a(a(MB * (K + 1) * 8) + a(MB * 4) + MB * 8)
         return h2d, d2h
 
```

Result: faster. 376.6 (median of 6 runs) (+5.0%).
